# libxsmm/fpga_ai_nic

Hardware: AMD Instinct MI355X
Metric: MLP training samples/sec (1024-4096-4096-1024, BFP all-reduce + fused SGD) (higher is better)
Workload: dtype bf16; 1 GPU; model=mlp-1024-4096-4096-1024, global_batch=8192, parallelism=dp1, mb_per_gpu=8192, compress=bfp, rounding=rne, algo=mesh, rings=1, transport=none, engine=native, schedule=fixed, gemm_inflight=persistent, hip_graph=False, fused_sgd=True, fused_update_in_gemm=True, epilogue_stream=inline

## Files before the change

### csrc/bindings_ops.cpp

```cpp
#include "bindings_common.h"
#include "bfp/bfp_format.h"
#include "comm/planner.h"
#include "gemm/gemm.h"
#include "gemm/gemm_chain.h"
#include "gemm/gemm_group.h"
#include "nn/nn.h"

namespace fan {

namespace {

int dcode(const at::Tensor& t) {
  if (t.scalar_type() == at::kFloat) return kF32;
  if (t.scalar_type() == at::kBFloat16) return kBF16;
  TORCH_CHECK(false, "expected float32 or bfloat16 tensor");
}

int64_t ld_of(const at::Tensor& t) {
  TORCH_CHECK(t.dim() == 2, "expected a 2-D tensor");
  TORCH_CHECK(t.stride(1) == 1, "expected unit stride in the last dim");
  return t.stride(0);
}

void gemm(const at::Tensor& A, bool a_t, const at::Tensor& B, bool b_t, at::Tensor& C, int64_t epilogue,
          const c10::optional<at::Tensor>& bias, const c10::optional<at::Tensor>& aux, bool accumulate,
          int64_t split_k, const c10::optional<at::Tensor>& workspace, int64_t tile_bm, int64_t tile_bn,
          const c10::optional<at::Tensor>& colsum, int64_t tile_waves, const c10::optional<at::Tensor>& wire,
          int64_t wire_shard, int64_t wire_own, int64_t wire_codec, int64_t wire_period, int64_t wire_off,
          const c10::optional<at::Tensor>& upd_master, const c10::optional<at::Tensor>& upd_lp,
          const c10::optional<at::Tensor>& upd_mom, double upd_lr, double upd_grad_scale, double upd_weight_decay,
          double upd_momentum, bool upd_nesterov, bool defer_colsum, bool defer_reduce) {
  TORCH_CHECK(A.is_cuda() && B.is_cuda() && C.is_cuda(), "gemm operands must be GPU tensors");
  TORCH_CHECK(A.scalar_type() == B.scalar_type(), "A and B dtype mismatch");
  GemmArgs g{};
  g.A = A.data_ptr();
  g.B = B.data_ptr();
  g.C = C.data_ptr();
  g.lda = ld_of(A);
  g.ldb = ld_of(B);
  g.ldc = ld_of(C);
  g.M = (int)(a_t ? A.size(1) : A.size(0));
  g.K = (int)(a_t ? A.size(0) : A.size(1));
  g.N = (int)(b_t ? B.size(0) : B.size(1));
  const int64_t kb = b_t ? B.size(1) : B.size(0);
  TORCH_CHECK(kb == g.K, "gemm: inner dimensions differ (", g.K, " vs ", kb, ")");
  TORCH_CHECK(C.size(0) == g.M && C.size(1) == g.N, "gemm: bad C shape");
  g.a_kcontig = !a_t;
  g.b_kcontig = b_t;
  g.epilogue = (int)epilogue;
  g.c_bf16 = C.scalar_type() == at::kBFloat16;
  g.accumulate = accumulate;
  g.split_k = (int)std::max<int64_t>(0, split_k);
  g.tile_bm = (int)tile_bm;
  g.tile_bn = (int)tile_bn;
  g.tile_waves = (int)tile_waves;
  g.defer_reduce = defer_reduce;
  TORCH_CHECK(!defer_reduce || (epilogue == kEpiBias && C.scalar_type() == at::kFloat && !colsum && !accumulate),
              "defer_reduce: the f32 bias epilogue only (the softmax folds the slabs)");
  if (colsum) {
    TORCH_CHECK(colsum->is_cuda() && colsum->is_contiguous() && colsum->scalar_type() == at::kFloat &&
                    colsum->numel() >= g.N,
                "colsum must be a contiguous f32 GPU tensor of >= N elements");
    g.colsum = colsum->data_ptr<float>();
  }
  if (bias) {
    TORCH_CHECK(bias->is_contiguous() && bias->numel() >= g.N, "bad bias");
    g.bias = bias->data_ptr();
  }
  if (aux) {
    TORCH_CHECK(aux->scalar_type() == C.scalar_type(), "aux dtype must match C");
    g.aux = aux->data_ptr();
    g.ldaux = ld_of(*aux);
  }
  if (workspace) g.workspace = workspace->data_ptr();
  if (epilogue == kEpiWire) {
    TORCH_CHECK(wire && wire->is_cuda() && wire->is_contiguous() && wire->scalar_type() == at::kByte,
                "wire epilogue needs a contiguous uint8 GPU wire buffer");
    TORCH_CHECK(wire_shard > 0 && wire_shard % 256 == 0, "wire_shard must be a positive multiple of 256");
    TORCH_CHECK(wire_off >= 0 && wire_off % 16 == 0, "wire_off must be a non-negative multiple of 16");
    const int64_t last = wire_off + (g.colsum ? (int64_t)g.M * g.ldc + g.N - 1 : (int64_t)(g.M - 1) * g.ldc + g.N - 1);
    const int64_t need = (last / wire_shard + 1) * (int64_t)wire_shard_bytes((int)wire_codec, (size_t)wire_shard);
    TORCH_CHECK(wire->numel() >= need, "wire buffer too small: ", wire->numel(), " < ", need);
    g.wire = wire->data_ptr<uint8_t>();
    g.wire_shard = wire_shard;
    g.wire_own = (int)wire_own;
    g.wire_period = (int)wire_period;
    g.wire_codec = (int)wire_codec;
    g.wire_off = wire_off;
    if (upd_master) {
      auto plane = [&](const at::Tensor& t, at::ScalarType st, const char* what) {
        TORCH_CHECK(t.is_cuda() && t.is_contiguous() && t.scalar_type() == st && t.numel() > last &&
                        t.data_ptr() != nullptr && (reinterpret_cast<uintptr_t>(t.data_ptr()) & 15) == 0,
                    "fused update: ", what, " must be a contiguous, 16-B aligned GPU plane covering the bucket");
      };
      TORCH_CHECK(wire_own == -1, "fused update: no owner shard (single-rank engine)");
      TORCH_CHECK(wire_codec == kBfpRne, "fused update: rne codec only");
      plane(*upd_master, at::kFloat, "master");
      g.upd_master = upd_master->data_ptr<float>();
      if (upd_lp) {
        plane(*upd_lp, at::kBFloat16, "lp");
        g.upd_lp = reinterpret_cast<bf16_t*>(upd_lp->data_ptr());
      }
      if (upd_mom) {
        plane(*upd_mom, at::kFloat, "mom");
        g.upd_mom = upd_mom->data_ptr<float>();
      }
      g.upd = SgdParams{(float)upd_lr, (float)upd_grad_scale, (float)upd_weight_decay, (float)upd_momentum,
                        upd_nesterov ? 1 : 0};
      g.defer_colsum = defer_colsum && g.colsum != nullptr;
    }
  }
  if (A.scalar_type() == at::kBFloat16) {
    TORCH_CHECK(bias ? bias->scalar_type() == at::kBFloat16 : true, "bias must be bf16");
    const GemmPlan p = gemm_bf16_plan(g.M, g.N, g.K, g.split_k, g.tile_bm, g.tile_bn, g.tile_waves);
    const int64_t need = (p.split_k > 1 ? (int64_t)p.split_k * g.M * g.N : 0) +
                         (g.colsum && p.bm > 0 ? (int64_t)p.split_k * ((g.M + p.bm - 1) / p.bm) * g.N : 0);
    if (need > 0 || p.split_k > 1) {
      TORCH_CHECK(workspace && workspace->scalar_type() == at::kFloat && workspace->is_contiguous() &&
                      workspace->numel() >= need,
                  "gemm: split-K ", p.split_k, (g.colsum ? " with colsum" : ""), " needs an f32 workspace of ", need,
                  " elements");
    }
    TORCH_CHECK(gemm_bf16_supported(g), "gemm_bf16: unsupported shape M=", g.M, " N=", g.N, " K=", g.K,
                " split_k=", g.split_k);
    launch_gemm_bf16(g, fan_stream());
  } else {
    TORCH_CHECK(A.scalar_type() == at::kFloat, "gemm: A must be bf16 or f32");
    const int sk = gemm_f32_split(g.M, g.N, g.K, g.split_k);
    if (sk > 1) {
      const int64_t need = (int64_t)sk * g.M * g.N;
      TORCH_CHECK(workspace && workspace->scalar_type() == at::kFloat && workspace->is_contiguous() &&
                      workspace->numel() >= need,
                  "gemm_f32: split-K ", sk, " needs an f32 workspace of ", need, " elements");
    }
    TORCH_CHECK(gemm_f32_supported(g), "gemm_f32: unsupported shape M=", g.M, " N=", g.N, " K=", g.K);
    launch_gemm_f32(g, fan_stream());
  }
}

void gemm_wgrad_group(const std::vector<at::Tensor>& Xs, const std::vector<at::Tensor>& dYs,
                      const std::vector<at::Tensor>& Cs, const std::vector<at::Tensor>& colsums,
                      const std::vector<int64_t>& offs, at::Tensor& workspace, const c10::optional<at::Tensor>& wire,
                      int64_t wire_shard, int64_t wire_own, int64_t wire_codec, int64_t wire_period) {
  const size_t n = Xs.size();
  TORCH_CHECK(n >= 1 && n <= (size_t)kGroupMax && dYs.size() == n && Cs.size() == n && colsums.size() == n &&
                  (offs.empty() || offs.size() == n),
              "gemm_wgrad_group: 1..", kGroupMax, " problems, one X, dY, C, colsum (and wire offset) each");
  TORCH_CHECK(workspace.is_cuda() && workspace.scalar_type() == at::kFloat && workspace.is_contiguous(),
              "gemm_wgrad_group: f32 GPU workspace");
  std::vector<GemmArgs> g(n);
  int64_t ws_off = 0;
  for (size_t i = 0; i < n; ++i) {
    const at::Tensor &X = Xs[i], &dY = dYs[i], &C = Cs[i], &cs = colsums[i];
    TORCH_CHECK(X.is_cuda() && dY.is_cuda() && C.is_cuda() && cs.is_cuda(), "gemm_wgrad_group: GPU tensors");
    TORCH_CHECK(X.scalar_type() == at::kBFloat16 && dY.scalar_type() == at::kBFloat16 &&
                    C.scalar_type() == at::kFloat && cs.scalar_type() == at::kFloat && cs.is_contiguous(),
                "gemm_wgrad_group: bf16 X / dY, f32 C / colsum");
    TORCH_CHECK(X.dim() == 2 && dY.dim() == 2 && X.size(0) == dY.size(0) && C.dim() == 2 && C.size(0) == X.size(1) &&
                    C.size(1) == dY.size(1) && cs.numel() >= dY.size(1),
                "gemm_wgrad_group: shapes (X [K][M], dY [K][N], C [M][N], colsum [N])");
    GemmArgs& a = g[i];
    a.A = X.data_ptr(); a.lda = ld_of(X);
    a.B = dY.data_ptr(); a.ldb = ld_of(dY);
    a.C = C.data_ptr(); a.ldc = ld_of(C);
    a.M = (int)X.size(1); a.N = (int)dY.size(1); a.K = (int)X.size(0);
    a.a_kcontig = false; a.b_kcontig = false; a.c_bf16 = false;
    a.colsum = cs.data_ptr<float>();
    a.epilogue = wire ? kEpiWire : kEpiNone;
    a.workspace = workspace.data_ptr<float>() + ws_off;
    ws_off += (gemm_wgrad_group_ws(a) + 3) / 4 * 4;
    if (wire) {
      TORCH_CHECK(wire->is_cuda() && wire->is_contiguous() && wire->scalar_type() == at::kByte,
                  "wire epilogue needs a contiguous uint8 GPU wire buffer");
      TORCH_CHECK(wire_shard > 0 && wire_shard % 256 == 0, "wire_shard must be a positive multiple of 256");
      const int64_t off = offs.empty() ? 0 : offs[i];
      TORCH_CHECK(off >= 0 && off % 16 == 0, "wire offsets must be non-negative multiples of 16");
      const int64_t last = off + (int64_t)a.M * a.ldc + a.N - 1;
      const int64_t need = (last / wire_shard + 1) * (int64_t)wire_shard_bytes((int)wire_codec, (size_t)wire_shard);
      TORCH_CHECK(wire->numel() >= need, "wire buffer too small: ", wire->numel(), " < ", need);
      a.wire = wire->data_ptr<uint8_t>();
      a.wire_shard = wire_shard;
      a.wire_own = (int)wire_own;
      a.wire_period = (int)wire_period;
      a.wire_codec = (int)wire_codec;
      a.wire_off = off;
    }
  }
  TORCH_CHECK(workspace.numel() >= ws_off, "gemm_wgrad_group: workspace of ", ws_off, " floats needed");
  TORCH_CHECK(gemm_wgrad_group_supported(g.data(), (int)n),
              "gemm_wgrad_group: unsupported (M % 256, N % 128, K % 64, aligned operands, at most ", 64 * kNumCU,
              " workgroups)");
  launch_gemm_wgrad_group(g.data(), (int)n, fan_stream());
}

bool gemm_chain(int64_t kind, const at::Tensor& A0, const std::vector<at::Tensor>& Bs, const std::vector<at::Tensor>& Cs,
                const std::vector<c10::optional<at::Tensor>>& biases,
                const std::vector<c10::optional<at::Tensor>>& auxes, const std::vector<int64_t>& epis,
                at::Tensor& counters, bool dry_run) {
  const int n = (int)Bs.size();
  TORCH_CHECK(n >= 1 && (int)Cs.size() == n && (int)biases.size() == n && (int)auxes.size() == n &&
                  (int)epis.size() == n,
              "gemm_chain: one B, C, bias, aux and epilogue entry per stage");
  if (n > gemm_chain_max_stages()) return false;
  std::vector<GemmArgs> g(n);
  for (int i = 0; i < n; ++i) {
    const at::Tensor& A = i == 0 ? A0 : Cs[i - 1];
    const at::Tensor& B = Bs[i];
    const at::Tensor& C = Cs[i];
    for (const at::Tensor* t : {&A, &B, &C})
      if (!t->is_cuda() || t->dim() != 2 || t->stride(1) != 1) return false;
    if (A.scalar_type() != at::kBFloat16 || B.scalar_type() != at::kBFloat16) return false;
    GemmArgs& a = g[i];
    a.A = A.data_ptr();
    a.B = B.data_ptr();
    a.C = C.data_ptr();
    a.lda = A.stride(0);
    a.ldb = B.stride(0);
    a.ldc = C.stride(0);
    a.M = (int)A.size(0);
    a.K = (int)A.size(1);
    a.N = (int)(kind == kChainBwdData ? B.size(0) : B.size(1));
    if ((kind == kChainBwdData ? B.size(1) : B.size(0)) != a.K || C.size(0) != a.M || C.size(1) != a.N) return false;
    a.a_kcontig = true;
    a.b_kcontig = kind == kChainBwdData;
    a.c_bf16 = C.scalar_type() == at::kBFloat16;
    if (!a.c_bf16 && C.scalar_type() != at::kFloat) return false;
    a.split_k = 1;
    if (kind == kChainFwd) {
      if (!biases[i] || biases[i]->scalar_type() != at::kBFloat16 || biases[i]->numel() < a.N) return false;
      a.bias = biases[i]->data_ptr();
      a.epilogue = (int)epis[i];
    } else {
      if (!auxes[i] || auxes[i]->scalar_type() != at::kBFloat16 || auxes[i]->dim() != 2 ||
          auxes[i]->stride(1) != 1 || auxes[i]->size(0) != a.M || auxes[i]->size(1) != a.N)
        return false;
      a.aux = auxes[i]->data_ptr();
      a.ldaux = auxes[i]->stride(0);
      a.epilogue = (int)epis[i];
    }
  }
  if (!gemm_chain_supported(g.data(), n, (int)kind)) return false;
  TORCH_CHECK(counters.is_cuda() && counters.scalar_type() == at::kInt && counters.is_contiguous() &&
                  counters.numel() >= gemm_chain_counter_words(n, g[0].M),
              "gemm_chain: counters must be a contiguous int32 GPU tensor of gemm_chain_words(n, M) elements");
  if (dry_run) return true;
  launch_gemm_chain(g.data(), n, (int)kind, reinterpret_cast<unsigned*>(counters.data_ptr()), fan_stream());
  return true;
}

int64_t gemm_wgrad_group_ws_floats(const std::vector<std::pair<int64_t, int64_t>>& mn) {
  int64_t w = 0;
  for (const auto& p : mn) w += ((p.first / 256) * p.second + 3) / 4 * 4;
  return w;
}

pybind11::tuple gemm_plan(int64_t M, int64_t N, int64_t K, int64_t split_k, int64_t tile_bm, int64_t tile_bn,
                          int64_t tile_waves) {
  GemmPlan p = gemm_bf16_plan((int)M, (int)N, (int)K, (int)split_k, (int)tile_bm, (int)tile_bn, (int)tile_waves);
  return pybind11::make_tuple(p.bm, p.bn, p.split_k, p.waves);
}

bool gemm_supported(int64_t M, int64_t N, int64_t K, bool bf16, int64_t split_k) {
  GemmArgs g{};
  g.M = (int)M;
  g.N = (int)N;
  g.K = (int)K;
  g.lda = g.ldb = 64;
  g.ldc = N;
  g.split_k = (int)split_k;
  g.workspace = (void*)16;
  return bf16 ? gemm_bf16_supported(g) : gemm_f32_supported(g);
}

void softmax_xent(const at::Tensor& logits, const at::Tensor& labels, at::Tensor& dlogits, at::Tensor& loss_rows,
                  double grad_scale) {
  TORCH_CHECK(logits.is_cuda() && labels.is_cuda() && dlogits.is_cuda() && loss_rows.is_cuda(), "GPU tensors");
  TORCH_CHECK(labels.scalar_type() == at::kInt && labels.is_contiguous(), "labels must be int32");
  TORCH_CHECK(loss_rows.scalar_type() == at::kFloat, "loss_rows must be f32");
  const int M = (int)logits.size(0), Cc = (int)logits.size(1);
  TORCH_CHECK(dlogits.size(0) == M && dlogits.size(1) == Cc, "dlogits shape");
  launch_softmax_xent(dcode(logits), logits.data_ptr(), ld_of(logits), labels.data_ptr<int32_t>(), dcode(dlogits),
                      dlogits.data_ptr(), ld_of(dlogits), loss_rows.data_ptr<float>(), M, Cc, (float)grad_scale,
                      fan_stream());
}

void softmax_xent_slabs(const at::Tensor& ws, int64_t sk, const at::Tensor& bias, at::Tensor& logits,
                        const at::Tensor& labels, at::Tensor& dlogits, at::Tensor& loss_rows, double grad_scale) {
  TORCH_CHECK(ws.is_cuda() && bias.is_cuda() && logits.is_cuda() && labels.is_cuda() && dlogits.is_cuda() &&
                  loss_rows.is_cuda(), "GPU tensors");
  TORCH_CHECK(ws.scalar_type() == at::kFloat && ws.is_contiguous() && logits.scalar_type() == at::kFloat &&
                  bias.scalar_type() == at::kBFloat16 && bias.is_contiguous(), "f32 slabs / logits, bf16 bias");
  TORCH_CHECK(labels.scalar_type() == at::kInt && labels.is_contiguous() && loss_rows.scalar_type() == at::kFloat,
              "int32 labels, f32 loss rows");
  const int M = (int)logits.size(0), Cc = (int)logits.size(1);
  TORCH_CHECK(dlogits.size(0) == M && dlogits.size(1) == Cc && bias.numel() >= Cc, "shapes");
  TORCH_CHECK(sk >= 1 && ws.numel() >= sk * (int64_t)M * Cc, "workspace holds sk slabs of M x C");
  launch_softmax_xent_slabs(ws.data_ptr<float>(), (int)sk, reinterpret_cast<const bf16_t*>(bias.data_ptr()),
                            logits.data_ptr<float>(), ld_of(logits), labels.data_ptr<int32_t>(), dcode(dlogits),
                            dlogits.data_ptr(), ld_of(dlogits), loss_rows.data_ptr<float>(), M, Cc,
                            (float)grad_scale, fan_stream());
}

void col_sum(const at::Tensor& x, at::Tensor& out, double scale, bool accumulate, at::Tensor& workspace) {
  TORCH_CHECK(x.is_cuda() && out.is_cuda() && workspace.is_cuda(), "GPU tensors");
  const int M = (int)x.size(0), N = (int)x.size(1);
  TORCH_CHECK(out.numel() >= N && out.is_contiguous(), "out too small");
  TORCH_CHECK(workspace.scalar_type() == at::kFloat && (size_t)workspace.numel() >= col_sum_workspace_floats(M, N),
              "workspace too small");
  launch_col_sum(dcode(x), x.data_ptr(), ld_of(x), M, N, dcode(out), out.data_ptr(), (float)scale, accumulate,
                 workspace.data_ptr<float>(), fan_stream());
}

}

void register_gemm(pybind11::module_& m) {
  m.def("gemm", &gemm, "MFMA GEMM with fused epilogue", pybind11::arg("A"), pybind11::arg("a_t"), pybind11::arg("B"),
        pybind11::arg("b_t"), pybind11::arg("C"), pybind11::arg("epilogue") = 0, pybind11::arg("bias") = pybind11::none(),
        pybind11::arg("aux") = pybind11::none(), pybind11::arg("accumulate") = false, pybind11::arg("split_k") = 1,
        pybind11::arg("workspace") = pybind11::none(), pybind11::arg("tile_bm") = 0, pybind11::arg("tile_bn") = 0,
        pybind11::arg("colsum") = pybind11::none(), pybind11::arg("tile_waves") = 0,
        pybind11::arg("wire") = pybind11::none(), pybind11::arg("wire_shard") = 0, pybind11::arg("wire_own") = -1,
        pybind11::arg("wire_codec") = 1, pybind11::arg("wire_period") = 0, pybind11::arg("wire_off") = 0,
        pybind11::arg("upd_master") = pybind11::none(), pybind11::arg("upd_lp") = pybind11::none(),
        pybind11::arg("upd_mom") = pybind11::none(), pybind11::arg("upd_lr") = 0.0,
        pybind11::arg("upd_grad_scale") = 1.0, pybind11::arg("upd_weight_decay") = 0.0,
        pybind11::arg("upd_momentum") = 0.0, pybind11::arg("upd_nesterov") = false,
        pybind11::arg("defer_colsum") = false, pybind11::arg("defer_reduce") = false);
  m.def("gemm_supported", &gemm_supported);
  m.def("gemm_flush_colsum", []() { return gemm_flush_colsum(fan_stream()); },
        "launch the bias-gradient reduces queued on the current stream by defer_colsum GEMMs; returns how many");
  m.def("gemm_pending_colsum", []() { return gemm_pending_colsum(fan_stream()); },
        "bias-gradient reduces queued on the current stream");
  m.def("gemm_wgrad_group", &gemm_wgrad_group,
        "up to 8 bwd-weight GEMMs (+ fused bias gradients, f32 or BFP wire epilogue) in one dispatch",
        pybind11::arg("Xs"), pybind11::arg("dYs"), pybind11::arg("Cs"), pybind11::arg("colsums"),
        pybind11::arg("offs"), pybind11::arg("workspace"), pybind11::arg("wire") = pybind11::none(),
        pybind11::arg("wire_shard") = 0, pybind11::arg("wire_own") = -1, pybind11::arg("wire_codec") = 1,
        pybind11::arg("wire_period") = 0);
  m.def("gemm_wgrad_group_ws", &gemm_wgrad_group_ws_floats, "f32 workspace elements for a group of (M, N) problems");
  m.def("gemm_chain", &gemm_chain, "the GEMMs of one MLP pass as one persistent launch (row-panel hand-offs)",
        pybind11::arg("kind"), pybind11::arg("A0"), pybind11::arg("Bs"), pybind11::arg("Cs"), pybind11::arg("biases"),
        pybind11::arg("auxes"), pybind11::arg("epis"), pybind11::arg("counters"), pybind11::arg("dry_run") = false);
  m.def("gemm_chain_words", &gemm_chain_counter_words, "int32 words of a layer-chain counter block",
        pybind11::arg("n"), pybind11::arg("M"));
  m.def("gemm_set_prio", [](int on) { gemm_prio_flag().store(on); },
        "4-wave pipelined GEMM waves at s_setprio 2 (another stream's kernels issue in their stalls)");
  m.def("gemm_prio", []() { return gemm_prio_flag().load(); });
  m.def("gemm_set_ovl", [](int on) { gemm_ovl_flag().store(on); },
        "256x256 bf16 plans on the persistent loop with overlapped tile transitions (pl4_run OVL)");
  m.def("gemm_ovl", []() { return gemm_ovl_flag().load(); });
  m.def("gemm_set_reduce4", [](int on) { gemm_reduce4_flag().store(on); },
        "split-K wire / fused-update reduce: 4 values per lane (1) or one 16-value group per lane (0)");
  m.def("gemm_reduce4", []() { return gemm_reduce4_flag().load(); });
  m.def("gemm_f32_split", &gemm_f32_split, "f32 GEMM split-K factor (split_k <= 0: automatic)", pybind11::arg("M"),
        pybind11::arg("N"), pybind11::arg("K"), pybind11::arg("split_k") = 0);
  m.def("gemm_set_main_loop", [](int mode) { gemm_main_loop_flag().store(mode); },
        "256x256 GEMM tiles: 0 one-role, 2 pipelined (4 or 8 waves by layout / K), 3 pipelined 4-wave, "
        "5 pipelined 8-wave");
  m.def("gemm_main_loop", []() { return gemm_main_loop_flag().load(); });
  m.def("gemm_set_persist", [](int cap) { gemm_persist_flag().store(cap); },
        "grid cap of the persistent 4-wave GEMM kernel (<= 0: one workgroup per tile)");
  m.def("gemm_persist", []() { return gemm_persist_flag().load(); });
  m.def("gemm_set_stamp_buffer", [](const c10::optional<at::Tensor>& t) {
          gemm_set_stamp_buffer(t ? t->data_ptr() : nullptr);
        },
        "diagnostic builds only: int64 GPU buffer [8 wg][8 waves][64 K-tiles][5] for the GEMM loop's s_memtime stamps");
  m.def("gemm_plan", &gemm_plan, "bf16 GEMM tile/split-K plan (bm, bn, split_k, waves); bm == 0: unsupported",
        pybind11::arg("M"), pybind11::arg("N"), pybind11::arg("K"), pybind11::arg("split_k") = 0,
        pybind11::arg("tile_bm") = 0, pybind11::arg("tile_bn") = 0, pybind11::arg("tile_waves") = 0);
  m.attr("EPI_NONE") = (int)kEpiNone;
  m.attr("EPI_BIAS") = (int)kEpiBias;
  m.attr("EPI_BIAS_RELU") = (int)kEpiBiasRelu;
  m.attr("EPI_RELU_MASK") = (int)kEpiReluMask;
  m.attr("EPI_WIRE") = (int)kEpiWire;
}

void register_nn(pybind11::module_& m) {
  m.def("softmax_xent", &softmax_xent, "fused softmax + cross-entropy fwd/bwd");
  m.def("softmax_xent_slabs", &softmax_xent_slabs,
        "softmax + cross-entropy over the classifier GEMM's unreduced split-K slabs (+ bias; logits written)");
  m.def("col_sum", &col_sum, "bias-gradient column sum");
  m.def("col_sum_workspace_floats", [](int64_t M, int64_t N) { return (int64_t)col_sum_workspace_floats((int)M, (int)N); });
}

void register_planner(pybind11::module_& m) {
  m.def("ring_geometry", [](int64_t n, int world, int64_t max_slice) {
    auto g = ring_geometry(n, world, max_slice);
    return pybind11::make_tuple(g.n, g.slice_elems, g.blocks, g.n_pad);
  });
  m.def("ring_plan", [](int world, int position, int64_t blocks) {
    auto rounds = ring_plan(world, position, blocks);
    std::vector<std::vector<int32_t>> out;
    out.reserve(rounds.size());
    for (auto& r : rounds) out.push_back({r.send_slice, r.send_src, r.recv_slice, r.recv_full, r.owned});
    return out;
  });
  m.def(
      "ring_orders",
      [](int world, int max_rings, c10::optional<std::vector<std::vector<int>>> links) {
        if (!links) return ring_orders(world, max_rings);
        std::vector<char> l((size_t)world * world, 0);
        TORCH_CHECK((int)links->size() == world, "links: world rows expected");
        for (int a = 0; a < world; ++a) {
          TORCH_CHECK((int)(*links)[a].size() == world, "links: world columns expected");
          for (int b = 0; b < world; ++b) l[(size_t)a * world + b] = (*links)[a][b] != 0;
        }
        return ring_orders(world, max_rings, &l);
      },
      pybind11::arg("world"), pybind11::arg("max_rings"), pybind11::arg("links") = pybind11::none(),
      "arc-disjoint directed Hamiltonian rings over the (optional) link matrix links[a][b]: a can send to b");
}

}
```

### csrc/gemm/gemm.h

```cpp
#pragma once
#include <atomic>

#include "bfp/bfp_format.h"
#include "common/hip_common.h"

namespace fan {

enum GemmEpilogue : int {
  kEpiNone = 0,
  kEpiBias = 1,
  kEpiBiasRelu = 2,
  kEpiReluMask = 3,
  kEpiWire = 4,
  kEpiWireUpd = 5,
};
constexpr bool is_wire_epi(int e) { return e == kEpiWire || e == kEpiWireUpd; }

constexpr int kWireOwnAll = -2;

struct GemmArgs {
  const void* A;
  const void* B;
  void* C;
  const void* bias;
  const void* aux;
  int64_t lda, ldb, ldc, ldaux;
  int M, N, K;
  bool a_kcontig, b_kcontig;
  int epilogue;
  bool c_bf16;
  bool accumulate;
  int split_k;
  void* workspace;
  int tile_bm = 0;
  int tile_bn = 0;
  int tile_waves = 0;
  float* colsum = nullptr;
  uint8_t* wire = nullptr;
  int64_t wire_shard = 0;
  int wire_own = -1;
  int wire_period = 0;
  int wire_codec = 1;
  int64_t wire_off = 0;
  float* upd_master = nullptr;
  bf16_t* upd_lp = nullptr;
  float* upd_mom = nullptr;
  SgdParams upd{};
  bool defer_colsum = false;
  bool defer_reduce = false;
};

struct GemmPlan {
  int bm, bn, split_k, waves;
};

GemmPlan gemm_bf16_plan(int M, int N, int K, int split_k, int tile_bm = 0, int tile_bn = 0, int tile_waves = 0);

bool gemm_bf16_supported(const GemmArgs& a);
void launch_gemm_bf16(const GemmArgs& a, hipStream_t stream);
int gemm_flush_colsum(hipStream_t stream);
int gemm_pending_colsum(hipStream_t stream);

std::atomic<int>& gemm_main_loop_flag();
std::atomic<int>& gemm_persist_flag();
std::atomic<int>& gemm_prio_flag();
std::atomic<int>& gemm_ovl_flag();
std::atomic<int>& gemm_reduce4_flag();
void gemm_set_stamp_buffer(void* p);
void* gemm_stamp_buffer();

int gemm_f32_split(int M, int N, int K, int split_k);
bool gemm_f32_supported(const GemmArgs& a);
void launch_gemm_f32(const GemmArgs& a, hipStream_t stream);

}
```

### csrc/gemm/gemm_bf16_kernel.h

```cpp
#pragma once
#include <cstdlib>
#include <type_traits>
#include <utility>

#include "bfp/bfp_format.h"
#include "gemm/gemm.h"
#include "gemm/glds.h"

namespace fan {
namespace gemm_detail {

typedef short s16x8 __attribute__((ext_vector_type(8)));
typedef short s16x4 __attribute__((ext_vector_type(4)));
typedef __bf16 bf16x8 __attribute__((ext_vector_type(8)));
typedef float f32x4 __attribute__((ext_vector_type(4)));
typedef __attribute__((address_space(3))) void lds_void_t;
typedef __attribute__((address_space(3))) s16x4 lds_s16x4_t;

constexpr int BK = 64;
constexpr int kDefaultWaves = 8;

#ifdef FAN_GEMM_STAMPS
constexpr int kStampWG = 8, kStampKT = 64, kStampPts = 5;
#define FAN_STAMP(pt)                                                                                        \
  if (wo.stamps && blockIdx.x < kStampWG && kt < kStampKT && lane == 0)                                       \
  wo.stamps[(((size_t)blockIdx.x * 8 + wave) * kStampKT + kt) * kStampPts + (pt)] = __builtin_amdgcn_s_memtime()
#else
#define FAN_STAMP(pt)
#endif

__device__ __forceinline__ int mn_swz(int k) { return (k & 3) | (((k >> 3) & 1) << 2); }

static __device__ __attribute__((aligned(256))) uint4 g_gemm_zero16[16];

__host__ __device__ constexpr int cdiv_i(int a, int b) { return (a + b - 1) / b; }

template <int OUTER, int NT>
struct OpTile {
  static constexpr int BYTES = OUTER * BK * 2;
  static constexpr int IB = NT * 16;
  static constexpr int GLDS = BYTES / IB;
  static constexpr int PER_HALF = (64 * 256) / IB;
};

template <bool KCONTIG, int OUTER, int NT, bool EDGE = false>
__device__ __forceinline__ void stage_one(const bf16_t* __restrict__ g, int64_t ld, int o0, int k0, char* lds,
                                          int wave, int lane, int i, int o_lim = 0, int k_lim = 0) {
  using T = OpTile<OUTER, NT>;
  const int t = wave * 64 + lane;
  const bf16_t* src;
  bool out = false;
  if (KCONTIG) {
    const int row = i * (T::IB / 128) + (t >> 3);
    const int c = (t & 7) ^ ((row >> 1) & 7);
    src = g + (int64_t)(o0 + row) * ld + k0 + c * 8;
    if (EDGE) out = o0 + row >= o_lim || k0 + c * 8 >= k_lim;
  } else {
    const int half = i / T::PER_HALF;
    const int krow = (i % T::PER_HALF) * (T::IB / 256) + (t >> 4);
    const int cs = t & 15;
    const int blk = (cs >> 1) ^ mn_swz(krow);
    const int col = o0 + half * 128 + blk * 16 + (cs & 1) * 8;
    src = g + (int64_t)(k0 + krow) * ld + col;
    if (EDGE) out = k0 + krow >= k_lim || col >= o_lim;
  }
  if (EDGE && out) src = reinterpret_cast<const bf16_t*>(g_gemm_zero16);
  glds16((const void*)src, __builtin_amdgcn_readfirstlane(lds_addr_of(lds + i * T::IB + wave * 1024)));
}

template <bool KCONTIG, int OUTER, int NT, bool EDGE = false>
__device__ __forceinline__ void stage_tile(const bf16_t* __restrict__ g, int64_t ld, int o0, int k0, char* lds,
                                           int wave, int lane, int o_lim = 0, int k_lim = 0) {
#pragma unroll
  for (int i = 0; i < OpTile<OUTER, NT>::GLDS; ++i)
    stage_one<KCONTIG, OUTER, NT, EDGE>(g, ld, o0, k0, lds, wave, lane, i, o_lim, k_lim);
}

template <bool KCONTIG>
__device__ __forceinline__ s16x8 read_frag(const char* lds, int o, int ks, int lane) {
  if (KCONTIG) {
    const int row = o + (lane & 15);
    const int chunk = ks * 4 + (lane >> 4);
    return *reinterpret_cast<const s16x8*>(lds + row * 128 + ((chunk ^ ((row >> 1) & 7)) << 4));
  } else {
    const char* h = lds + (o >> 7) * (64 * 256);
    const int oo = o & 127;
    const int q = (lane & 15) >> 2, p = lane & 3;
    const int kb = ks * 32 + 8 * (lane >> 4) + q;
    const int blk = oo >> 4;
    const int off0 = kb * 256 + ((blk ^ mn_swz(kb)) << 5) + 8 * p;
    const int off1 = (kb + 4) * 256 + ((blk ^ mn_swz(kb + 4)) << 5) + 8 * p;
    s16x4 lo = __builtin_amdgcn_ds_read_tr16_b64_v4i16((lds_s16x4_t*)(h + off0));
    s16x4 hi = __builtin_amdgcn_ds_read_tr16_b64_v4i16((lds_s16x4_t*)(h + off1));
    s16x8 r;
    r[0] = lo[0]; r[1] = lo[1]; r[2] = lo[2]; r[3] = lo[3];
    r[4] = hi[0]; r[5] = hi[1]; r[6] = hi[2]; r[7] = hi[3];
    return r;
  }
}

__device__ __forceinline__ float frag_sum(const s16x8& f) {
  typedef __bf16 bf16x2 __attribute__((ext_vector_type(2)));
  typedef short s16x2 __attribute__((ext_vector_type(2)));
  const bf16x2 one = {(__bf16)1.0f, (__bf16)1.0f};
  float s = 0.f;
#pragma unroll
  for (int e = 0; e < 4; ++e) {
    const s16x2 p = {f[2 * e], f[2 * e + 1]};
    s = __builtin_amdgcn_fdot2_f32_bf16(__builtin_bit_cast(bf16x2, p), one, s, false);
  }
  return s;
}

__device__ __forceinline__ int xcd_remap(int bid, int nwg) {
  const int xcd = bid % kNumXCD;
  const int q = nwg / kNumXCD, r = nwg % kNumXCD;
  const int base = xcd < r ? xcd * (q + 1) : r * (q + 1) + (xcd - r) * q;
  return base + bid / kNumXCD;
}

template <typename TC>
struct Out;
template <>
struct Out<float> {
  __device__ static __forceinline__ void load4(const float* p, float v[4]) {
    const float4 x = *reinterpret_cast<const float4*>(p);
    v[0] = x.x; v[1] = x.y; v[2] = x.z; v[3] = x.w;
  }
  __device__ static __forceinline__ void store4(float* p, const float v[4]) {
    *reinterpret_cast<float4*>(p) = make_float4(v[0], v[1], v[2], v[3]);
  }
};
template <>
struct Out<bf16_t> {
  __device__ static __forceinline__ void load4(const bf16_t* p, float v[4]) {
    const uint2 u = *reinterpret_cast<const uint2*>(p);
    v[0] = __uint_as_float(u.x << 16); v[1] = __uint_as_float(u.x & 0xFFFF0000u);
    v[2] = __uint_as_float(u.y << 16); v[3] = __uint_as_float(u.y & 0xFFFF0000u);
  }
  __device__ static __forceinline__ void store4(bf16_t* p, const float v[4]) {
    *reinterpret_cast<uint2*>(p) = make_uint2(pack_bf16x2(v[0], v[1]), pack_bf16x2(v[2], v[3]));
  }
};

template <int EPI, typename TC, bool ACCUM>
__device__ __forceinline__ void epi4(float v[4], TC* __restrict__ C, int64_t ldc, const bf16_t* __restrict__ bias,
                                     const TC* __restrict__ aux, int64_t ldaux, int row, int col) {
  if (EPI == kEpiBias || EPI == kEpiBiasRelu) {
    const uint2 u = *reinterpret_cast<const uint2*>(bias + col);
    v[0] += __uint_as_float(u.x << 16); v[1] += __uint_as_float(u.x & 0xFFFF0000u);
    v[2] += __uint_as_float(u.y << 16); v[3] += __uint_as_float(u.y & 0xFFFF0000u);
  }
  if (EPI == kEpiBiasRelu) {
#pragma unroll
    for (int u = 0; u < 4; ++u) v[u] = fmaxf(v[u], 0.f);
  }
  if (EPI == kEpiReluMask) {
    float m[4];
    Out<TC>::load4(aux + (int64_t)row * ldaux + col, m);
#pragma unroll
    for (int u = 0; u < 4; ++u) v[u] = m[u] > 0.f ? v[u] : 0.f;
  }
  TC* p = C + (int64_t)row * ldc + col;
  if (ACCUM) {
    float o[4];
    Out<TC>::load4(p, o);
#pragma unroll
    for (int u = 0; u < 4; ++u) v[u] += o[u];
  }
  Out<TC>::store4(p, v);
}

typedef uint32_t u32x4_t __attribute__((ext_vector_type(4)));
__device__ __forceinline__ void store_wt16(void* p, const uint4& o) {
  const u32x4_t v = {o.x, o.y, o.z, o.w};
  asm volatile("global_store_dwordx4 %0, %1, off sc1\n\ts_nop 1" ::"v"(p), "v"(v) : "memory");
}

template <int EPI, bool ACCUM, bool WT = false>
__device__ __forceinline__ void epi8_bf16(float v[8], bf16_t* __restrict__ C, int64_t ldc,
                                          const bf16_t* __restrict__ bias, const uint4* mask, int row, int col) {
  auto lo = [](uint32_t u) { return __uint_as_float(u << 16); };
  auto hi = [](uint32_t u) { return __uint_as_float(u & 0xFFFF0000u); };
  if (EPI == kEpiBias || EPI == kEpiBiasRelu) {
    const uint4 u = *reinterpret_cast<const uint4*>(bias + col);
    v[0] += lo(u.x); v[1] += hi(u.x); v[2] += lo(u.y); v[3] += hi(u.y);
    v[4] += lo(u.z); v[5] += hi(u.z); v[6] += lo(u.w); v[7] += hi(u.w);
  }
  if (EPI == kEpiBiasRelu) {
#pragma unroll
    for (int u = 0; u < 8; ++u) v[u] = fmaxf(v[u], 0.f);
  }
  if (EPI == kEpiReluMask) {
    const uint4 m = *mask;
    const float mv[8] = {lo(m.x), hi(m.x), lo(m.y), hi(m.y), lo(m.z), hi(m.z), lo(m.w), hi(m.w)};
#pragma unroll
    for (int u = 0; u < 8; ++u) v[u] = mv[u] > 0.f ? v[u] : 0.f;
  }
  bf16_t* p = C + (int64_t)row * ldc + col;
  if (ACCUM) {
    const uint4 o = *reinterpret_cast<const uint4*>(p);
    v[0] += lo(o.x); v[1] += hi(o.x); v[2] += lo(o.y); v[3] += hi(o.y);
    v[4] += lo(o.z); v[5] += hi(o.z); v[6] += lo(o.w); v[7] += hi(o.w);
  }
  const uint4 o = make_uint4(pack_bf16x2(v[0], v[1]), pack_bf16x2(v[2], v[3]), pack_bf16x2(v[4], v[5]),
                             pack_bf16x2(v[6], v[7]));
  if constexpr (WT) store_wt16(p, o);
  else *reinterpret_cast<uint4*>(p) = o;
}

struct WireOut {
  uint8_t* p;
  int64_t shard;
  int own;
  int period;
  int codec;
  float inv_shard;
  int bias_off;
  float* um;
  bf16_t* ulp;
  float* umom;
  SgdParams up;
#ifdef FAN_GEMM_STAMPS
  unsigned long long* stamps;
#endif
  uint32_t off;
  int prio;
};

__device__ __forceinline__ int wire_shard_of(uint32_t f, const WireOut& wo) {
  int sh = (int)((float)f * wo.inv_shard);
  const uint32_t sz = (uint32_t)wo.shard;
  if ((uint32_t)sh * sz > f) --sh;
  else if ((uint32_t)(sh + 1) * sz <= f) ++sh;
  return sh;
}

__device__ __forceinline__ uint8_t* wire_shard_base(int sh, const WireOut& wo) {
  return wo.p + (int64_t)sh * (wo.shard + wo.shard / 16);
}

__device__ __forceinline__ int32_t wire_encode(float x, uint32_t E, int codec) {
  return codec == kBfpTrunc ? bfp_encode_trunc(__float_as_uint(x), E) : bfp_encode_rne(x, E);
}

__device__ __forceinline__ float wire_roundtrip_rne(float x, uint32_t E) {
  return bfp_decode_rne(bfp_encode_rne(x, E), E);
}

__device__ __forceinline__ float sgd_apply(float g, float& w, float& m, bool has_mom, const SgdParams& p) {
  float gj = g * p.grad_scale;
  if (p.weight_decay != 0.0f) gj = fmaf(p.weight_decay, w, gj);
  if (has_mom) {
    m = fmaf(p.momentum, m, gj);
    gj = p.nesterov ? fmaf(p.momentum, m, gj) : m;
  }
  w = fmaf(-p.lr, gj, w);
  return w;
}

template <bool PRE = false>
__device__ __forceinline__ void local_update16(const float v[16], uint32_t E, uint32_t f, const WireOut& wo,
                                               float (&w)[16]) {
  float m[16];
  if constexpr (!PRE) {
#pragma unroll
    for (int u = 0; u < 16; u += 4) {
      const float4 a = *reinterpret_cast<const float4*>(wo.um + f + u);
      w[u] = a.x; w[u + 1] = a.y; w[u + 2] = a.z; w[u + 3] = a.w;
    }
  }
  const bool hm = wo.umom != nullptr;
  if (hm) {
#pragma unroll
    for (int u = 0; u < 16; u += 4) {
      const float4 a = *reinterpret_cast<const float4*>(wo.umom + f + u);
      m[u] = a.x; m[u + 1] = a.y; m[u + 2] = a.z; m[u + 3] = a.w;
    }
  }
#pragma unroll
  for (int u = 0; u < 16; ++u) sgd_apply(wire_roundtrip_rne(v[u], E), w[u], m[u], hm, wo.up);
#pragma unroll
  for (int u = 0; u < 16; u += 4) {
    *reinterpret_cast<float4*>(wo.um + f + u) = make_float4(w[u], w[u + 1], w[u + 2], w[u + 3]);
    if (hm) *reinterpret_cast<float4*>(wo.umom + f + u) = make_float4(m[u], m[u + 1], m[u + 2], m[u + 3]);
  }
  if (wo.ulp) {
    uint4* d = reinterpret_cast<uint4*>(wo.ulp + f);
    d[0] = make_uint4(pack_bf16x2(w[0], w[1]), pack_bf16x2(w[2], w[3]), pack_bf16x2(w[4], w[5]),
                      pack_bf16x2(w[6], w[7]));
    d[1] = make_uint4(pack_bf16x2(w[8], w[9]), pack_bf16x2(w[10], w[11]), pack_bf16x2(w[12], w[13]),
                      pack_bf16x2(w[14], w[15]));
  }
}

template <bool UPD = false, bool PRE = false>
__device__ __forceinline__ int wire_store16(const float v[16], uint32_t f, const WireOut& wo, float (&wm)[16]) {
  uint32_t mx = 0;
#pragma unroll
  for (int u = 0; u < 16; ++u) mx = max(mx, __float_as_uint(v[u]) & 0x7FFFFFFFu);
  const uint32_t E = mx >> 23;
  if constexpr (UPD) {
    local_update16<PRE>(v, E, f, wo, wm);
    return -1;
  }
  const int sh = wire_shard_of(f, wo);
  const uint32_t pos = f - (uint32_t)sh * (uint32_t)wo.shard;
  uint32_t w[4] = {0u, 0u, 0u, 0u};
#pragma unroll
  for (int u = 0; u < 16; ++u) w[u >> 2] |= ((uint32_t)wire_encode(v[u], E, wo.codec) & 0xFFu) << (8 * (u & 3));
  uint8_t* base = wire_shard_base(sh, wo);
  *reinterpret_cast<uint4*>(base + pos) = make_uint4(w[0], w[1], w[2], w[3]);
  base[wo.shard + pos / 16] = (uint8_t)E;
  return sh;
}

template <bool UPD = false>
__device__ __forceinline__ int wire_store16(const float v[16], uint32_t f, const WireOut& wo) {
  float wm[16];
  return wire_store16<UPD, false>(v, f, wo, wm);
}

template <bool UPD = false, bool PRE = false>
__device__ __forceinline__ void wire_epi16(const float v[16], float* __restrict__ C, int64_t ldc, const WireOut& wo,
                                           int row, int col, float (&w)[16]) {
  const uint32_t loc = (uint32_t)row * (uint32_t)ldc + (uint32_t)col;
  const int sh = wire_store16<UPD, PRE>(v, wo.off + loc, wo, w);
  if (sh >= 0 && (wo.own == kWireOwnAll || (wo.period > 0 ? sh % wo.period : sh) == wo.own)) {
#pragma unroll
    for (int u = 0; u < 16; u += 4)
      *reinterpret_cast<float4*>(C + loc + u) = make_float4(v[u], v[u + 1], v[u + 2], v[u + 3]);
  }
}

template <bool UPD = false>
__device__ __forceinline__ void wire_epi16(const float v[16], float* __restrict__ C, int64_t ldc, const WireOut& wo,
                                           int row, int col) {
  float w[16];
  wire_epi16<UPD, false>(v, C, ldc, wo, row, col, w);
}

template <int NJ, int WTN, int EPI, bool SPLIT>
__device__ __forceinline__ void colsum_finish(float (&cs)[NJ], int lane, int col0, float* __restrict__ out,
                                              const WireOut& wo, int N) {
#pragma unroll
  for (int j = 0; j < NJ; ++j) {
    float v = cs[j];
    v += __shfl_xor(v, 16);
    v += __shfl_xor(v, 32);
    const int col = col0 + j * 16 + (lane & 15);
    if (lane < 16 && col < N) out[col] = v;
    if constexpr (is_wire_epi(EPI) && !SPLIT) {
      if (wo.bias_off > 0 && col0 + j * 16 < N) {
        uint32_t mx = __float_as_uint(v) & 0x7FFFFFFFu;
#pragma unroll
        for (int o = 1; o < 16; o <<= 1) mx = max(mx, (uint32_t)__shfl_xor((int)mx, o));
        const uint32_t E = mx >> 23;
        const uint32_t f = (uint32_t)wo.bias_off + (uint32_t)col;
        if constexpr (EPI == kEpiWireUpd) {
          if (lane < 16) {
            float w = wo.um[f], m = wo.umom ? wo.umom[f] : 0.f;
            sgd_apply(wire_roundtrip_rne(v, E), w, m, wo.umom != nullptr, wo.up);
            wo.um[f] = w;
            if (wo.umom) wo.umom[f] = m;
            if (wo.ulp) wo.ulp[f] = f32_to_bf16(w);
          }
          continue;
        }
        const int sh = wire_shard_of(f, wo);
        const uint32_t pos = f - (uint32_t)sh * (uint32_t)wo.shard;
        uint8_t* base = wire_shard_base(sh, wo);
        if (lane < 16) base[pos] = (uint8_t)(wire_encode(v, E, wo.codec) & 0xFF);
        if (lane == 0) base[wo.shard + pos / 16] = (uint8_t)E;
      }
    }
  }
}

template <int MI, int NJ, int WTN, int EPI, typename TC, bool ACCUM, bool SPLIT, int SW = WTN, bool WT = false>
__device__ __forceinline__ void store_tile(const f32x4 (&acc)[MI][NJ], char* smem, int wave, int lane, int row0,
                                           int col0, TC* __restrict__ C, int64_t ldc, const bf16_t* __restrict__ bias,
                                           const TC* __restrict__ aux, int64_t ldaux, int M, int N, int ksplit,
                                           float* __restrict__ ws, const WireOut& wo, bool mn_edge = false) {
  static_assert(SW == WTN || (SW == 64 && WTN % 64 == 0 && sizeof(TC) == 2 && !SPLIT && !is_wire_epi(EPI)),
                "64-column staging: bf16 8-column path only");
  static_assert(!WT || (sizeof(TC) == 2 && !SPLIT && !is_wire_epi(EPI)), "write-through stores: the bf16 8-column path");
  constexpr int EW = SW + 4;
  float* stg = reinterpret_cast<float*>(smem) + wave * (16 * EW);
  const int col_l = lane & 15, row_l = (lane >> 4) * 4;
  constexpr int C4 = WTN / 4;
  constexpr int RPI = 64 / C4;
  if constexpr (sizeof(TC) == 2 && !SPLIT && !is_wire_epi(EPI)) {
    {
      constexpr int C8 = SW / 8;
      constexpr int RP8 = 64 / C8;
      constexpr int NP8 = 16 / RP8;
      constexpr int HV = WTN / SW;
      static_assert(WTN % 8 == 0 && RP8 <= 16 && 16 % RP8 == 0, "8-column chunks of whole 16-row blocks");
      constexpr bool kPf8 = EPI == kEpiReluMask;
      constexpr int kPfd = 2;
      uint4 aq8[kPf8 ? MI : 1][kPf8 ? HV * NP8 : 1];
      auto aux_load8 = [&](int i) __attribute__((always_inline)) {
#pragma unroll
        for (int hv = 0; hv < HV; ++hv)
#pragma unroll
          for (int pass = 0; pass < NP8; ++pass) {
            const int row = row0 + i * 16 + pass * RP8 + lane / C8;
            const int col = col0 + hv * SW + (lane % C8) * 8;
            if (!mn_edge || (row < M && col < N))
              aq8[i][hv * NP8 + pass] = *reinterpret_cast<const uint4*>(aux + (int64_t)row * ldaux + col);
          }
      };
      if constexpr (kPf8) {
#pragma unroll
        for (int i = 0; i < kPfd && i < MI; ++i) aux_load8(i);
      }
#pragma unroll
      for (int i = 0; i < MI; ++i) {
        if constexpr (kPf8) {
          if (i + kPfd < MI) aux_load8(i + kPfd);
        }
#pragma unroll
        for (int hv = 0; hv < HV; ++hv) {
#pragma unroll
        for (int j = 0; j < SW / 16; ++j)
#pragma unroll
          for (int r = 0; r < 4; ++r) stg[(row_l + r) * EW + j * 16 + col_l] = acc[i][hv * (SW / 16) + j][r];
        __builtin_amdgcn_s_waitcnt(0xC07F);
#pragma unroll
        for (int pass = 0; pass < NP8; ++pass) {
          const int rr = pass * RP8 + lane / C8;
          const int cc = (lane % C8) * 8;
          const float4 q0 = *reinterpret_cast<const float4*>(stg + rr * EW + cc);
          const float4 q1 = *reinterpret_cast<const float4*>(stg + rr * EW + cc + 4);
          float v[8] = {q0.x, q0.y, q0.z, q0.w, q1.x, q1.y, q1.z, q1.w};
          const int row = row0 + i * 16 + rr;
          const int col = col0 + hv * SW + cc;
          if (mn_edge && (row >= M || col >= N)) continue;
          const uint4* mk = nullptr;
          if constexpr (kPf8) mk = &aq8[i][hv * NP8 + pass];
          epi8_bf16<EPI, ACCUM, WT>(v, reinterpret_cast<bf16_t*>(C), ldc, bias, mk, row, col);
        }
        __builtin_amdgcn_s_waitcnt(0xC07F);
        }
      }
      return;
    }
  }
  constexpr bool kPfAux = EPI == kEpiReluMask && !SPLIT && sizeof(TC) == 2;
  constexpr int kPf = 2;
  constexpr int NP = 16 / RPI;
  using AuxV = typename std::conditional<sizeof(TC) == 2, uint2, uint4>::type;
  AuxV aq[kPfAux ? MI : 1][kPfAux ? NP : 1];
  auto aux_load = [&](int i) __attribute__((always_inline)) {
#pragma unroll
    for (int pass = 0; pass < NP; ++pass) {
      const int row = row0 + i * 16 + pass * RPI + lane / C4;
      const int col = col0 + (lane % C4) * 4;
      if (!mn_edge || (row < M && col < N))
        aq[i][pass] = *reinterpret_cast<const AuxV*>(aux + (int64_t)row * ldaux + col);
    }
  };
  if constexpr (kPfAux) {
#pragma unroll
    for (int i = 0; i < kPf && i < MI; ++i) aux_load(i);
  }
  constexpr bool kPfUpd = EPI == kEpiWireUpd && !SPLIT;
  constexpr int UG16 = WTN / 16, URPG = 64 / UG16, UPASS = URPG >= 16 ? 1 : 16 / URPG;
#ifndef FAN_GEMM_UPD_PF
#define FAN_GEMM_UPD_PF 2
#endif
  constexpr int kUpf = FAN_GEMM_UPD_PF, US = kPfUpd ? kUpf + 1 : 1;
  float um_pf[US][kPfUpd ? UPASS : 1][16];
  auto upd_load = [&](int i, int slot) __attribute__((always_inline)) {
    if constexpr (kPfUpd) {
#pragma unroll
      for (int pass = 0; pass < UPASS; ++pass) {
        const int rr = pass * URPG + lane / UG16;
        const int row = row0 + i * 16 + rr, col = col0 + (lane % UG16) * 16;
        if ((URPG <= 16 || rr < 16) && (!mn_edge || (row < M && col < N))) {
          const float* q = wo.um + wo.off + (uint32_t)row * (uint32_t)ldc + (uint32_t)col;
#pragma unroll
          for (int u = 0; u < 16; u += 4) {
            const float4 a = *reinterpret_cast<const float4*>(q + u);
            um_pf[slot][pass][u] = a.x; um_pf[slot][pass][u + 1] = a.y;
            um_pf[slot][pass][u + 2] = a.z; um_pf[slot][pass][u + 3] = a.w;
          }
        }
      }
    }
  };
  if constexpr (kPfUpd) {
#pragma unroll
    for (int d = 0; d < kUpf && d < MI; ++d) upd_load(d, d % US);
  }
#pragma unroll
  for (int i = 0; i < MI; ++i) {
    if constexpr (kPfAux) {
      if (i + kPf < MI) aux_load(i + kPf);
    }
    if constexpr (kPfUpd) {
      if (i + kUpf < MI) upd_load(i + kUpf, (i + kUpf) % US);
    }
#pragma unroll
    for (int j = 0; j < NJ; ++j)
#pragma unroll
      for (int r = 0; r < 4; ++r) stg[(row_l + r) * EW + j * 16 + col_l] = acc[i][j][r];
    __builtin_amdgcn_s_waitcnt(0xC07F);
    if constexpr (is_wire_epi(EPI) && !SPLIT) {
      constexpr int G16 = WTN / 16;
      constexpr int RPG = 64 / G16;
      constexpr int PASSES = RPG >= 16 ? 1 : 16 / RPG;
#pragma unroll
      for (int pass = 0; pass < PASSES; ++pass) {
        const int rr = pass * RPG + lane / G16;
        if (RPG <= 16 || rr < 16) {
          const int cc = (lane % G16) * 16;
          float v[16];
#pragma unroll
          for (int u = 0; u < 16; u += 4) {
            const float4 q = *reinterpret_cast<const float4*>(stg + rr * EW + cc + u);
            v[u] = q.x; v[u + 1] = q.y; v[u + 2] = q.z; v[u + 3] = q.w;
          }
          if (!mn_edge || (row0 + i * 16 + rr < M && col0 + cc < N))
            wire_epi16<EPI == kEpiWireUpd, kPfUpd>(v, reinterpret_cast<float*>(C), ldc, wo, row0 + i * 16 + rr,
                                                   col0 + cc, um_pf[kPfUpd ? i % US : 0][kPfUpd ? pass : 0]);
        }
      }
      __builtin_amdgcn_s_waitcnt(0xC07F);
      continue;
    }
#pragma unroll
    for (int pass = 0; pass < 16 / RPI; ++pass) {
      const int rr = pass * RPI + lane / C4;
      const int cc = (lane % C4) * 4;
      const float4 q = *reinterpret_cast<const float4*>(stg + rr * EW + cc);
      float v[4] = {q.x, q.y, q.z, q.w};
      const int row = row0 + i * 16 + rr;
      const int col = col0 + cc;
      if (mn_edge && (row >= M || col >= N)) continue;
      if (SPLIT) {
        float* slab = ws + (int64_t)ksplit * M * N;
        *reinterpret_cast<float4*>(slab + (int64_t)row * N + col) = q;
      } else if constexpr (kPfAux) {
        float m[4];
        if constexpr (sizeof(TC) == 2) {
          const uint2 u = aq[i][pass];
          m[0] = __uint_as_float(u.x << 16); m[1] = __uint_as_float(u.x & 0xFFFF0000u);
          m[2] = __uint_as_float(u.y << 16); m[3] = __uint_as_float(u.y & 0xFFFF0000u);
        } else {
          const uint4 u = aq[i][pass];
          m[0] = __uint_as_float(u.x); m[1] = __uint_as_float(u.y);
          m[2] = __uint_as_float(u.z); m[3] = __uint_as_float(u.w);
        }
#pragma unroll
        for (int u = 0; u < 4; ++u) v[u] = m[u] > 0.f ? v[u] : 0.f;
        epi4<kEpiNone, TC, ACCUM>(v, C, ldc, bias, aux, ldaux, row, col);
      } else {
        epi4<EPI, TC, ACCUM>(v, C, ldc, bias, aux, ldaux, row, col);
      }
    }
    __builtin_amdgcn_s_waitcnt(0xC07F);
  }
}

template <int BM, int BN, int WM, int WN, bool AK, bool BKC, int EPI, typename TC, bool ACCUM, bool SPLIT,
          bool DMA1 = false, bool RAGGED = false>
__global__ void __launch_bounds__(WM * WN * 64, WM * WN / 4)
    gemm_bf16_kernel(const bf16_t* __restrict__ A, int64_t lda, const bf16_t* __restrict__ B, int64_t ldb,
                     TC* __restrict__ C, int64_t ldc, const bf16_t* __restrict__ bias, const TC* __restrict__ aux,
                     int64_t ldaux, int M, int N, int K, int split_k, float* __restrict__ ws,
                     float* __restrict__ colsum, WireOut wo) {
  constexpr int NT = WM * WN * 64;
  constexpr int A_BYTES = OpTile<BM, NT>::BYTES, B_BYTES = OpTile<BN, NT>::BYTES;
  constexpr int STAGE = A_BYTES + B_BYTES;
  constexpr int S = (3 * STAGE <= 160 * 1024) ? 3 : 2;
  constexpr int G = OpTile<BM, NT>::GLDS + OpTile<BN, NT>::GLDS;
  constexpr int WTM = BM / WM, WTN = BN / WN;
  constexpr int MI = WTM / 16, NJ = WTN / 16;
  static_assert(WM * WN == 8 || WM * WN == 4, "4 or 8 waves");
  extern __shared__ __attribute__((aligned(16))) char smem[];

  const int tiles_n = cdiv_i(N, BN);
  const int tiles_m = cdiv_i(M, BM);
  const int tiles = tiles_m * tiles_n;
  const int nwg = tiles * split_k;
  const int wg = xcd_remap(blockIdx.x, nwg);
  const int tile = wg % tiles;
  const int ksplit = wg / tiles;
  const int GM = tiles_m >= 4 ? 4 : tiles_m;
  const int grp = tile / (GM * tiles_n);
  const int gm = (tiles_m - grp * GM) < GM ? (tiles_m - grp * GM) : GM;
  const int in_grp = tile % (GM * tiles_n);
  const int m0 = (grp * GM + in_grp % gm) * BM;
  const int n0 = (in_grp / gm) * BN;
  const int nkt = cdiv_i(K, BK);
  const int kt_per = cdiv_i(nkt, split_k);
  const int kt0 = ksplit * kt_per;
  const int nk = max(0, min(nkt, kt0 + kt_per) - kt0);
  const int kbeg = kt0 * BK;
  const bool mn_edge = RAGGED && (m0 + BM > M || n0 + BN > N);
  const bool edge = RAGGED && (mn_edge || (kt0 + nk) * BK > K);

  const int lane = threadIdx.x & 63;
  const int wave = __builtin_amdgcn_readfirstlane(threadIdx.x >> 6);
  const int wm = wave / WN, wn = wave % WN;
  const bool do_colsum = !BKC && colsum != nullptr && m0 == 0 && wm == 0;
  float cs[NJ];
#pragma unroll
  for (int j = 0; j < NJ; ++j) cs[j] = 0.f;

  f32x4 acc[MI][NJ];
#pragma unroll
  for (int i = 0; i < MI; ++i)
#pragma unroll
    for (int j = 0; j < NJ; ++j) acc[i][j] = f32x4{0.f, 0.f, 0.f, 0.f};

  auto issue_stage = [&](int kt_stage, int buf) {
    char* st = smem + buf * STAGE;
    if (edge) {
      stage_tile<AK, BM, NT, true>(A, lda, m0, kbeg + kt_stage * BK, st, wave, lane, M, K);
      stage_tile<BKC, BN, NT, true>(B, ldb, n0, kbeg + kt_stage * BK, st + A_BYTES, wave, lane, N, K);
    } else {
      stage_tile<AK, BM, NT>(A, lda, m0, kbeg + kt_stage * BK, st, wave, lane);
      stage_tile<BKC, BN, NT>(B, ldb, n0, kbeg + kt_stage * BK, st + A_BYTES, wave, lane);
    }
  };

  constexpr int REG_BUDGET = NT == 256 ? 480 : 232;
  constexpr int ACC_R = MI * NJ * 4, FRAG_R = (MI + NJ) * 4;
  constexpr bool DBL = ACC_R + 2 * FRAG_R <= REG_BUDGET;
#pragma unroll
  for (int s = 0; s < S - 1; ++s) {
    if (s < nk) issue_stage(s, s);
  }

  for (int kt = 0; kt < nk; ++kt) {
    FAN_STAMP(0);
    if (S == 3 && kt + 1 < nk) {
      asm volatile("s_waitcnt vmcnt(%0)" ::"n"(G) : "memory");
    } else {
      asm volatile("s_waitcnt vmcnt(0)" ::: "memory");
    }
    FAN_STAMP(1);
    __builtin_amdgcn_s_barrier();
    FAN_STAMP(2);
    const bool pf = kt + S - 1 < nk;
    char* pst = smem + ((kt + S - 1) % S) * STAGE;
    const int pk = kbeg + (kt + S - 1) * BK;
    if constexpr (DMA1 && S == 2 && NT == 512) {
      if (pf && wave < 4) {
        if (edge) {
          stage_tile<AK, BM, 256, true>(A, lda, m0, pk, pst, wave, lane, M, K);
          stage_tile<BKC, BN, 256, true>(B, ldb, n0, pk, pst + A_BYTES, wave, lane, N, K);
        } else {
          stage_tile<AK, BM, 256>(A, lda, m0, pk, pst, wave, lane);
          stage_tile<BKC, BN, 256>(B, ldb, n0, pk, pst + A_BYTES, wave, lane);
        }
      }
    } else if (pf) {
      if (edge) {
        stage_tile<AK, BM, NT, true>(A, lda, m0, pk, pst, wave, lane, M, K);
        stage_tile<BKC, BN, NT, true>(B, ldb, n0, pk, pst + A_BYTES, wave, lane, N, K);
      } else {
        stage_tile<AK, BM, NT>(A, lda, m0, pk, pst, wave, lane);
        stage_tile<BKC, BN, NT>(B, ldb, n0, pk, pst + A_BYTES, wave, lane);
      }
    }
    FAN_STAMP(3);
    const char* sa = smem + (kt % S) * STAGE;
    const char* sb = sa + A_BYTES;
    if constexpr (DBL) {
      s16x8 af[2][MI], bfr[2][NJ];
#pragma unroll
      for (int ks = 0; ks < 2; ++ks) {
#pragma unroll
        for (int i = 0; i < MI; ++i) af[ks][i] = read_frag<AK>(sa, wm * WTM + i * 16, ks, lane);
#pragma unroll
        for (int j = 0; j < NJ; ++j) bfr[ks][j] = read_frag<BKC>(sb, wn * WTN + j * 16, ks, lane);
        if (do_colsum) {
#pragma unroll
          for (int j = 0; j < NJ; ++j) cs[j] += frag_sum(bfr[ks][j]);
        }
      }
      FAN_STAMP(4);
#pragma unroll
      for (int ks = 0; ks < 2; ++ks) {
        __builtin_amdgcn_s_setprio(1);
#pragma unroll
        for (int i = 0; i < MI; ++i)
#pragma unroll
          for (int j = 0; j < NJ; ++j)
            acc[i][j] = __builtin_amdgcn_mfma_f32_16x16x32_bf16(__builtin_bit_cast(bf16x8, af[ks][i]),
                                                                __builtin_bit_cast(bf16x8, bfr[ks][j]), acc[i][j],
                                                                0, 0, 0);
        __builtin_amdgcn_s_setprio(0);
      }
    } else {
#pragma unroll
      for (int ks = 0; ks < 2; ++ks) {
        s16x8 af[MI], bfr[NJ];
#pragma unroll
        for (int i = 0; i < MI; ++i) af[i] = read_frag<AK>(sa, wm * WTM + i * 16, ks, lane);
#pragma unroll
        for (int j = 0; j < NJ; ++j) bfr[j] = read_frag<BKC>(sb, wn * WTN + j * 16, ks, lane);
        if (do_colsum) {
#pragma unroll
          for (int j = 0; j < NJ; ++j) cs[j] += frag_sum(bfr[j]);
        }
        __builtin_amdgcn_s_setprio(1);
#pragma unroll
        for (int i = 0; i < MI; ++i)
#pragma unroll
          for (int j = 0; j < NJ; ++j)
            acc[i][j] = __builtin_amdgcn_mfma_f32_16x16x32_bf16(__builtin_bit_cast(bf16x8, af[i]),
                                                                __builtin_bit_cast(bf16x8, bfr[j]), acc[i][j], 0,
                                                                0, 0);
        __builtin_amdgcn_s_setprio(0);
      }
    }
  }

  if (do_colsum)
    colsum_finish<NJ, WTN, EPI, SPLIT>(cs, lane, n0 + wn * WTN, SPLIT ? ws + (int64_t)split_k * M * N + (int64_t)ksplit * N
                                                                      : colsum, wo, N);
  __syncthreads();
  store_tile<MI, NJ, WTN, EPI, TC, ACCUM, SPLIT>(acc, smem, wave, lane, m0 + wm * WTM, n0 + wn * WTN, C, ldc, bias,
                                                 aux, ldaux, M, N, ksplit, ws, wo, mn_edge);
}

__device__ __forceinline__ void glds16_s(const void* sbase, uint32_t voff, uint32_t lds_addr) {
  asm volatile("s_mov_b32 m0, %2\n\ts_nop 0\n\tglobal_load_lds_dwordx4 %0, %1" ::"v"(voff), "s"(sbase), "s"(lds_addr)
               : "memory");
}

template <uint32_t OFF, bool SC1 = false>
__device__ __forceinline__ void glds16_si(const void* sbase, uint32_t voff, uint32_t lds_base) {
  if constexpr (SC1)
    asm volatile("s_add_u32 m0, %2, %3\n\ts_nop 0\n\tglobal_load_lds_dwordx4 %0, %1 sc1" ::"v"(voff), "s"(sbase),
                 "s"(lds_base), "i"(OFF)
                 : "memory", "scc");
  else
    asm volatile("s_add_u32 m0, %2, %3\n\ts_nop 0\n\tglobal_load_lds_dwordx4 %0, %1" ::"v"(voff), "s"(sbase),
                 "s"(lds_base), "i"(OFF)
                 : "memory", "scc");
}

template <int VM, int LGKM>
__device__ __forceinline__ void waitcnt_known() {
  static_assert(VM >= 0 && VM <= 63 && LGKM >= 0 && LGKM <= 15, "s_waitcnt field ranges");
#ifdef FAN_GEMM_ASM_WAITS
  asm volatile("s_waitcnt vmcnt(%0) lgkmcnt(%1)" ::"n"(VM), "n"(LGKM) : "memory");
#else
  __builtin_amdgcn_s_waitcnt((VM & 15) | (7 << 4) | (LGKM << 8) | ((VM >> 4) << 14));
  asm volatile("" ::: "memory");
#endif
}

template <bool KCONTIG, int OUTER, int NT>
__device__ __forceinline__ uint32_t piece_off(int64_t ld, int o0, int wave, int lane, int i) {
  using T = OpTile<OUTER, NT>;
  const int t = wave * 64 + lane;
  if (KCONTIG) {
    const int row = i * (T::IB / 128) + (t >> 3);
    const int c = (t & 7) ^ ((row >> 1) & 7);
    return (uint32_t)(((int64_t)(o0 + row) * ld + c * 8) * 2);
  } else {
    const int half = i / T::PER_HALF;
    const int krow = (i % T::PER_HALF) * (T::IB / 256) + (t >> 4);
    const int cs = t & 15;
    const int blk = (cs >> 1) ^ mn_swz(krow);
    return (uint32_t)(((int64_t)krow * ld + o0 + half * 128 + blk * 16 + (cs & 1) * 8) * 2);
  }
}

template <bool AK, bool BKC, int EPI, typename TC, bool ACCUM, bool SPLIT, bool COLSUM = false>
__global__ void __launch_bounds__(512, 2)
    gemm_pl_kernel(const bf16_t* __restrict__ A, int64_t lda, const bf16_t* __restrict__ B, int64_t ldb,
                   TC* __restrict__ C, int64_t ldc, const bf16_t* __restrict__ bias, const TC* __restrict__ aux,
                   int64_t ldaux, int M, int N, int K, int split_k, float* __restrict__ ws,
                   float* __restrict__ colsum, WireOut wo) {
  constexpr int BM = 256, BN = 256, NT = 512;
  constexpr int A_BYTES = OpTile<BM, NT>::BYTES;
  constexpr int STAGE = A_BYTES + OpTile<BN, NT>::BYTES;
  constexpr int GA = OpTile<BM, NT>::GLDS, G = GA + OpTile<BN, NT>::GLDS;
  constexpr int WTM = 128, WTN = 64, MI = 8, NJ = 4;
  static_assert(G == 8, "8 glds pieces per wave and K-tile");
  extern __shared__ __attribute__((aligned(16))) char smem[];

  const int tiles_n = N / BN, tiles_m = M / BM, tiles = tiles_m * tiles_n;
  const int wg = xcd_remap(blockIdx.x, tiles * split_k);
  const int tile = wg % tiles, ksplit = wg / tiles;
  const int GM = tiles_m >= 4 ? 4 : tiles_m;
  const int grp = tile / (GM * tiles_n);
  const int gm = (tiles_m - grp * GM) < GM ? (tiles_m - grp * GM) : GM;
  const int in_grp = tile % (GM * tiles_n);
  const int m0 = (grp * GM + in_grp % gm) * BM;
  const int n0 = (in_grp / gm) * BN;
  const int k_per = K / split_k;
  const int kbeg = ksplit * k_per;
  const int nk = k_per / BK;

  const int lane = threadIdx.x & 63;
  const int wave = __builtin_amdgcn_readfirstlane(threadIdx.x >> 6);
  const int wm = wave / 4, wn = wave % 4;
  const int im = SPLIT ? 0 : m0 / BM;
  const int cs0 = SPLIT ? (m0 == 0 ? 0 : nk) : im * nk / tiles_m;
  const int cs1 = SPLIT ? nk : (im + 1) * nk / tiles_m;
  const bool do_colsum = COLSUM && wm == 0;
  float cs[NJ];
#pragma unroll
  for (int j = 0; j < NJ; ++j) cs[j] = 0.f;

  f32x4 acc[MI][NJ];
#pragma unroll
  for (int i = 0; i < MI; ++i)
#pragma unroll
    for (int j = 0; j < NJ; ++j) acc[i][j] = f32x4{0.f, 0.f, 0.f, 0.f};
  s16x8 fa[MI], fb[2][NJ];

  uint32_t off[G];
#pragma unroll
  for (int p = 0; p < GA; ++p) off[p] = piece_off<AK, BM, NT>(lda, m0, wave, lane, p);
#pragma unroll
  for (int p = GA; p < G; ++p) off[p] = piece_off<BKC, BN, NT>(ldb, n0, wave, lane, p - GA);
  const int64_t a_step = AK ? (int64_t)BK * 2 : (int64_t)BK * lda * 2;
  const int64_t b_step = BKC ? (int64_t)BK * 2 : (int64_t)BK * ldb * 2;
  const char* a_k0 = reinterpret_cast<const char*>(A) + (AK ? (int64_t)kbeg * 2 : (int64_t)kbeg * lda * 2);
  const char* b_k0 = reinterpret_cast<const char*>(B) + (BKC ? (int64_t)kbeg * 2 : (int64_t)kbeg * ldb * 2);
  const uint32_t lds0 = lds_addr_of(smem);

  auto piece = [&](int kt, int p) {
    const uint32_t st = lds0 + (kt & 1) * STAGE + wave * 1024;
    if (p < GA) glds16_s(a_k0 + kt * a_step, off[p], st + p * OpTile<BM, NT>::IB);
    else glds16_s(b_k0 + kt * b_step, off[p], st + A_BYTES + (p - GA) * OpTile<BN, NT>::IB);
  };
  auto read_a = [&](const char* st, int ks, int i) { fa[i] = read_frag<AK>(st, wm * WTM + i * 16, ks, lane); };
  auto read_b = [&](const char* st, int ks, int set, int j) {
    fb[set][j] = read_frag<BKC>(st + A_BYTES, wn * WTN + j * 16, ks, lane);
  };
  auto block = [&](auto cur_c, auto read_c, auto dma_c, const char* rd_st, int rd_ks, int dma_kt, bool csk) {
    constexpr int cur = decltype(cur_c)::value;
    constexpr bool READ = decltype(read_c)::value, DMA = decltype(dma_c)::value;
    if (COLSUM && csk) {
#pragma unroll
      for (int j = 0; j < NJ; ++j) cs[j] += frag_sum(fb[cur][j]);
    }
#pragma unroll
    for (int i = 0; i < MI; ++i) {
#pragma unroll
      for (int j = 0; j < NJ; ++j) {
        if (READ && i < 2 && (j & 1) == 0) read_b(rd_st, rd_ks, cur ^ 1, i * 2 + (j >> 1));
        if (DMA && j == 2) piece(dma_kt, i);
        acc[i][j] = __builtin_amdgcn_mfma_f32_16x16x32_bf16(__builtin_bit_cast(bf16x8, fa[i]),
                                                            __builtin_bit_cast(bf16x8, fb[cur][j]), acc[i][j], 0, 0, 0);
      }
      if (READ) read_a(rd_st, rd_ks, i);
    }
    if constexpr (READ) {
#pragma unroll
      for (int i = 0; i < MI; ++i) {
        if (i < 2) {
          __builtin_amdgcn_sched_group_barrier(0x100, 1, 0);
          __builtin_amdgcn_sched_group_barrier(0x008, 2, 0);
          __builtin_amdgcn_sched_group_barrier(0x100, 1, 0);
          __builtin_amdgcn_sched_group_barrier(0x008, 2, 0);
        } else {
          __builtin_amdgcn_sched_group_barrier(0x008, 4, 0);
        }
        __builtin_amdgcn_sched_group_barrier(0x100, 1, 0);
      }
    }
  };
  using I0 = std::integral_constant<int, 0>;
  using I1 = std::integral_constant<int, 1>;
  using T_ = std::true_type;
  using F_ = std::false_type;

#pragma unroll
  for (int p = 0; p < G; ++p) piece(0, p);
  if (nk > 1) {
#pragma unroll
    for (int p = 0; p < G; ++p) piece(1, p);
    asm volatile("s_waitcnt vmcnt(%0)" ::"n"(G) : "memory");
  } else {
    asm volatile("s_waitcnt vmcnt(0)" ::: "memory");
  }
  __builtin_amdgcn_s_barrier();
#pragma unroll
  for (int j = 0; j < NJ; ++j) read_b(smem, 0, 0, j);
#pragma unroll
  for (int i = 0; i < MI; ++i) read_a(smem, 0, i);

  auto ktile = [&](int kt, auto more_c, auto more2_c) {
    const char* st = smem + (kt & 1) * STAGE;
    const bool csk = do_colsum && kt >= cs0 && kt < cs1;
    FAN_STAMP(0);
    __builtin_amdgcn_s_setprio(1);
    block(I0{}, T_{}, F_{}, st, 1, 0, csk);
    __builtin_amdgcn_s_setprio(0);
    FAN_STAMP(1);
    asm volatile("s_waitcnt vmcnt(0) lgkmcnt(0)" ::: "memory");
    FAN_STAMP(2);
    __builtin_amdgcn_s_barrier();
    FAN_STAMP(3);
    __builtin_amdgcn_s_setprio(1);
    block(I1{}, more_c, more2_c, smem + ((kt + 1) & 1) * STAGE, 0, kt + 2, csk);
    __builtin_amdgcn_s_setprio(0);
    FAN_STAMP(4);
  };
  int kt = 0;
  for (; kt + 2 < nk; ++kt) ktile(kt, T_{}, T_{});
  if (kt + 1 < nk) ktile(kt++, T_{}, F_{});
  if (kt < nk) ktile(kt, F_{}, F_{});

  if (COLSUM && do_colsum && (!SPLIT || m0 == 0))
    colsum_finish<NJ, WTN, kEpiNone, true>(
        cs, lane, n0 + wn * WTN, ws + (SPLIT ? (int64_t)split_k * M * N + (int64_t)ksplit * N : (int64_t)im * N), wo,
        N);
  asm volatile("s_waitcnt vmcnt(0)" ::: "memory");
  __syncthreads();
  store_tile<MI, NJ, WTN, EPI, TC, ACCUM, SPLIT>(acc, smem, wave, lane, m0 + wm * WTM, n0 + wn * WTN, C, ldc, bias,
                                                 aux, ldaux, M, N, ksplit, ws, wo);
}


template <typename F, int... I>
__device__ __forceinline__ void static_for_impl(F&& f, std::integer_sequence<int, I...>) {
  (f(std::integral_constant<int, I>{}), ...);
}
template <int N, typename F>
__device__ __forceinline__ void static_for(F&& f) {
  static_for_impl(f, std::make_integer_sequence<int, N>{});
}

__device__ __forceinline__ void mfma_acc(f32x4& acc, const s16x8& a, const s16x8& b) {
#ifdef FAN_GEMM_NOMFMA
  asm volatile("" : "+a"(acc) : "v"(a), "v"(b));
#else
  asm volatile("v_mfma_f32_16x16x32_bf16 %0, %1, %2, %0" : "+a"(acc) : "v"(a), "v"(b));
#endif
}

constexpr int kChainMaxStages = 8;
constexpr int kChainLdsCtl = 2 * (256 + 256) * BK * 2 + 4 * 16 * (64 + 4) * 4;
constexpr int kChainLds = kChainLdsCtl + 64;
constexpr uint32_t kChainSpinLimit = 1u << 22;

struct ChainStageArgs {
  const bf16_t* A;
  const bf16_t* B;
  void* C;
  const bf16_t* bias;
  const void* aux;
  int64_t lda, ldb, ldc, ldaux;
  int M, N, K;
  int tn;
  int first;
  int dep;
  int signal;
  int cfg;
};

struct ChainArgs {
  ChainStageArgs st[kChainMaxStages];
  int nstages;
  int total;
  int ppg;
  int panels;
  unsigned* ctr;
  int prio;
  int flags;
};
constexpr int kChainNoAcquire = 1;
constexpr int kChainRowsFastest = 2;

__host__ __device__ constexpr int chain_ctr_words(int nstages, int panels) { return (10 + nstages * panels) * 16; }
__device__ __forceinline__ int chain_ready_word(const ChainArgs& ca, int s, int panel) {
  return (10 + s * ca.panels + panel) * 16;
}
__device__ __forceinline__ int chain_stage_of(const ChainArgs& ca, int t) {
  int s = 0;
  while (s + 1 < ca.nstages && t >= ca.st[s + 1].first) ++s;
  return s;
}

struct ChainState {
  int ticket;
  int ready;
  int pending;
};

struct ChainRun {
  unsigned* ctr;
  int group, ppg, wpg;
  int first, end, tn;
  int dep;
  int dep_word0;
  int sig_word0;
  int nx_end, nx_tn;
  int flags;
};
__device__ __forceinline__ void chain_rc(const ChainRun& cr, int tn, int k, int& r, int& c) {
  if (cr.flags & kChainRowsFastest) {
    r = k % cr.ppg;
    c = k / cr.ppg;
  } else {
    r = k / tn;
    c = k % tn;
  }
}

__device__ __forceinline__ void chain_add(unsigned* ctr, int word) {
  __hip_atomic_fetch_add(ctr + word, 1u, __ATOMIC_RELAXED, __HIP_MEMORY_SCOPE_AGENT);
}
__device__ __forceinline__ unsigned chain_poll(const unsigned* ctr, int word) {
  return __hip_atomic_load(ctr + word, __ATOMIC_RELAXED, __HIP_MEMORY_SCOPE_AGENT);
}
__device__ __forceinline__ void chain_acquire(int flags = 0) {
  if (!(flags & kChainNoAcquire)) asm volatile("buffer_inv sc1" ::: "memory");
}
__device__ __forceinline__ void chain_tile_rc(const ChainArgs& ca, int tn, int k, int& r, int& c) {
  if (ca.flags & kChainRowsFastest) {
    r = k % ca.ppg;
    c = k / ca.ppg;
  } else {
    r = k / tn;
    c = k % tn;
  }
}

__device__ __forceinline__ void chain_dep_of(const ChainArgs& ca, int t, int& word, unsigned& target) {
  word = -1;
  target = 0;
  if (t >= ca.total) return;
  const int s = chain_stage_of(ca, t);
  const ChainStageArgs& S = ca.st[s];
  if (S.dep <= 0) return;
  int r, c;
  chain_tile_rc(ca, S.tn, t - S.first, r, c);
  word = chain_ready_word(ca, s - 1, (int)(blockIdx.x & 7) * ca.ppg + r);
  target = (unsigned)S.dep;
}

template <bool AK, bool BKC, int EPI, typename TC, bool ACCUM, bool SPLIT, bool COLSUM = false, int BN_ = 256,
          int BM_ = 256, bool OVL = false, bool CHAIN = false, bool WT = false, bool ASC1 = false>
__device__ __forceinline__ void pl4_run(const bf16_t* __restrict__ A, int64_t lda, const bf16_t* __restrict__ B,
                                        int64_t ldb, TC* __restrict__ C, int64_t ldc, const bf16_t* __restrict__ bias,
                                        const TC* __restrict__ aux, int64_t ldaux, int M, int N, int K, int split_k,
                                        float* __restrict__ ws, float* __restrict__ colsum, const WireOut& wo, int v0,
                                        int vstep, ChainRun cr = ChainRun{}, ChainState* chs = nullptr) {
  constexpr int BM = BM_, BN = BN_, NT = 256;
  constexpr int A_BYTES = OpTile<BM, NT>::BYTES;
  constexpr int STAGE = A_BYTES + OpTile<BN, NT>::BYTES;
  constexpr int GA = OpTile<BM, NT>::GLDS, G = GA + OpTile<BN, NT>::GLDS;
  constexpr int WTM = BM / 2, WTN = BN / 2, MI = WTM / 16, NJ = WTN / 16;
  constexpr int Q = MI * NJ, R = MI + NJ;
#ifndef FAN_GEMM_RSP_Q4
#define FAN_GEMM_RSP_Q4 3
#endif
  constexpr int RSP = (Q * FAN_GEMM_RSP_Q4 / 4) / R, DSP = Q / G;
  static_assert(BN == 256 || BN == 128, "256x256 or 256x128 tiles");
  static_assert(BM == 256 || (BM == 224 && BN == 128 && AK && !COLSUM) || (BM == 128 && BN == 128),
                "256-row tiles; 224-row tiles (K-contiguous A, BN 128); 128x128 tiles");
  static_assert(OpTile<BM, NT>::BYTES % OpTile<BM, NT>::IB == 0, "whole glds pieces");
  constexpr int STAGES = BN == 128 ? 3 : 2;
  static_assert(RSP >= 1 && DSP >= 1 && G * DSP <= Q, "schedule");
  static_assert(!OVL || (BM == 256 && BN == 256 && !COLSUM && !SPLIT && !ACCUM && sizeof(TC) == 2 &&
                         !is_wire_epi(EPI)),
                "overlapped transitions: 256x256 bf16 tiles without split-K or bias gradient");
  constexpr int kSW = OVL ? 64 : WTN;
  constexpr int kS = MI * (WTN / kSW) * (16 / (64 / (kSW / 8)));
  constexpr int DSP2 = Q / (2 * G);
  static_assert(!OVL || (G + kS <= 63 && DSP2 >= 1), "vmcnt range / schedule");
  extern __shared__ __attribute__((aligned(16))) char smem[];

  const int tiles_n = N / BN, tiles_m = M / BM, tiles = tiles_m * tiles_n;
  const int lane = threadIdx.x & 63;
  const int wave = __builtin_amdgcn_readfirstlane(threadIdx.x >> 6);
  const int wm = wave / 2, wn = wave % 2;
  const uint32_t lds0 = lds_addr_of(smem);
  if (wo.prio > 0) __builtin_amdgcn_s_setprio(2);
  static_assert(!CHAIN || (!SPLIT && !COLSUM && !ACCUM && BM == 256), "layer chain: unsplit 256-row tiles");
  const int GM = tiles_m >= 4 ? 4 : tiles_m;
  auto tile_origin = [&](int v, int& m, int& n) __attribute__((always_inline)) {
    if constexpr (CHAIN) {
      int r, c;
      chain_rc(cr, cr.tn, v - cr.first, r, c);
      m = (cr.group * cr.ppg + r) * BM;
      n = c * BN;
    } else {
      const int t1 = xcd_remap(v, tiles * split_k) % tiles;
      const int g1 = t1 / (GM * tiles_n);
      const int gm1 = (tiles_m - g1 * GM) < GM ? (tiles_m - g1 * GM) : GM;
      const int i1 = t1 % (GM * tiles_n);
      m = (g1 * GM + i1 % gm1) * BM;
      n = (i1 / gm1) * BN;
    }
  };
  int ch_next = 0, ch_rdy = 0;
  bool ch_cont = false;
  auto tile_body = [&](int v, bool first, int vn) __attribute__((always_inline)) {
  const int ksplit = CHAIN ? 0 : xcd_remap(v, tiles * split_k) / tiles;
  int m0, n0;
  tile_origin(v, m0, n0);
  const int k_per = K / split_k;
  const int kbeg = ksplit * k_per;
  const int nk = k_per / BK;

  const int im = SPLIT ? 0 : m0 / BM;
  const int cs0 = SPLIT ? (m0 == 0 ? 0 : nk) : im * nk / tiles_m;
  const int cs1 = SPLIT ? nk : (im + 1) * nk / tiles_m;
  const bool do_colsum = COLSUM && wm == 0;
  float cs[NJ];
#pragma unroll
  for (int j = 0; j < NJ; ++j) cs[j] = 0.f;

  f32x4 acc[MI][NJ];
#pragma unroll
  for (int i = 0; i < MI; ++i)
#pragma unroll
    for (int j = 0; j < NJ; ++j) acc[i][j] = f32x4{0.f, 0.f, 0.f, 0.f};
  s16x8 fa[2][MI], fb[2][NJ];

  uint32_t off[G];
#pragma unroll
  for (int p = 0; p < GA; ++p) off[p] = piece_off<AK, BM, NT>(lda, m0, wave, lane, p);
#pragma unroll
  for (int p = GA; p < G; ++p) off[p] = piece_off<BKC, BN, NT>(ldb, n0, wave, lane, p - GA);
  const int64_t a_step = AK ? (int64_t)BK * 2 : (int64_t)BK * lda * 2;
  const int64_t b_step = BKC ? (int64_t)BK * 2 : (int64_t)BK * ldb * 2;
  const char* a_k0 = reinterpret_cast<const char*>(A) + (AK ? (int64_t)kbeg * 2 : (int64_t)kbeg * lda * 2);
  const char* b_k0 = reinterpret_cast<const char*>(B) + (BKC ? (int64_t)kbeg * 2 : (int64_t)kbeg * ldb * 2);

  auto piece = [&](int kt, auto pc) __attribute__((always_inline)) {
    constexpr int p = decltype(pc)::value;
    const uint32_t st = lds0 + (STAGES == 2 ? kt & 1 : kt % 3) * STAGE + wave * 1024;
    if constexpr (p < GA) glds16_si<p * OpTile<BM, NT>::IB, ASC1>(a_k0 + kt * a_step, off[p], st);
    else glds16_si<A_BYTES + (p - GA) * OpTile<BN, NT>::IB>(b_k0 + kt * b_step, off[p], st);
  };
  auto read_next = [&](const char* st, int ks, int set, int r) __attribute__((always_inline)) {
    if (r < MI) fa[set][r] = read_frag<AK>(st, wm * WTM + r * 16, ks, lane);
    else fb[set][r - MI] = read_frag<BKC>(st + A_BYTES, wn * WTN + (r - MI) * 16, ks, lane);
  };
  auto block = [&](auto cur_c, auto read_c, auto dma_c, const char* rd_st, int rd_ks, int dma_kt,
                   bool csk, auto next_c, bool next_on = false) __attribute__((always_inline)) {
    constexpr int cur = decltype(cur_c)::value;
    constexpr bool READ = decltype(read_c)::value, DMA = decltype(dma_c)::value, NEXT = decltype(next_c)::value;
    if (COLSUM && csk)
      static_for<NJ>([&](auto jc) __attribute__((always_inline)) { cs[jc.value] += frag_sum(fb[cur][jc.value]); });
    static_for<MI * NJ>([&](auto qc) __attribute__((always_inline)) {
      constexpr int q = decltype(qc)::value;
      if constexpr (READ && q % RSP == 0 && q / RSP < R) read_next(rd_st, rd_ks, cur ^ 1, q / RSP);
#ifndef FAN_GEMM_NODMA
      if constexpr (DMA && q % DSP == DSP / 2 && q / DSP < G) piece(dma_kt, std::integral_constant<int, q / DSP>{});
      if constexpr (NEXT && q % DSP2 == 0 && q / DSP2 < 2 * G) {
        if (next_on) piece(q / DSP2 / G, std::integral_constant<int, q / DSP2 % G>{});
      }
#endif
      mfma_acc(acc[q / NJ][q % NJ], fa[cur][q / NJ], fb[cur][q % NJ]);
    });
  };
  using I0 = std::integral_constant<int, 0>;
  using I1 = std::integral_constant<int, 1>;
  using T_ = std::true_type;
  using F_ = std::false_type;

  if (!OVL || first) static_for<G>([&](auto pc) __attribute__((always_inline)) { piece(0, pc); });
  if (nk > 1) {
    if (!OVL || first) {
      static_for<G>([&](auto pc) __attribute__((always_inline)) { piece(1, pc); });
      asm volatile("s_waitcnt vmcnt(%0)" ::"n"(G) : "memory");
    } else {
      asm volatile("s_waitcnt vmcnt(%0)" ::"n"(G + kS) : "memory");
    }
  } else {
    asm volatile("s_waitcnt vmcnt(0)" ::: "memory");
  }
  __builtin_amdgcn_s_barrier();
#pragma unroll
  for (int r = 0; r < R; ++r) read_next(smem, 0, 0, r);

  unsigned ch_poll = 0;
  int* const ch_ctl = reinterpret_cast<int*>(smem + kChainLdsCtl);
  auto chain_hook = [&](int kt) __attribute__((always_inline)) {
    if constexpr (CHAIN) {
      if (kt == 1) {
        if (wave == 0 && lane == 0) {
          if (chs->pending >= 0) chain_add(cr.ctr, chs->pending);
          ch_ctl[0] = cr.wpg + (int)__hip_atomic_fetch_add(cr.ctr + cr.group * 16, 1u, __ATOMIC_RELAXED,
                                                            __HIP_MEMORY_SCOPE_AGENT);
        }
        chs->pending = -1;
      } else if (kt == nk - 3) {
        if (wave == 0 && lane == 0) {
          const int t = ch_ctl[0];
          int r, c, word = -1, tgt = 0;
          if (t < cr.end) {
            if (cr.dep > 0) {
              chain_rc(cr, cr.tn, t - cr.first, r, c);
              word = cr.dep_word0 + r * 16;
              tgt = cr.dep;
            }
          } else if (t < cr.nx_end && cr.sig_word0 >= 0) {
            chain_rc(cr, cr.nx_tn, t - cr.end, r, c);
            word = cr.sig_word0 + r * 16;
            tgt = cr.tn;
          } else {
            word = -2;
          }
          ch_ctl[2] = word;
          ch_ctl[3] = tgt;
          if (word >= 0) ch_poll = chain_poll(cr.ctr, word);
        }
      } else if (kt == nk - 2) {
        if (wave == 0 && lane == 0) {
          const int word = ch_ctl[2];
          ch_ctl[1] = word == -1 || (word >= 0 && ch_poll >= (unsigned)ch_ctl[3]);
        }
      }
    }
  };
  auto chain_decide = [&]() __attribute__((always_inline)) {
    if constexpr (CHAIN) {
      ch_next = __builtin_amdgcn_readfirstlane(ch_ctl[0]);
      ch_rdy = __builtin_amdgcn_readfirstlane(ch_ctl[1]);
      ch_cont = OVL && ch_rdy && ch_next < cr.end;
      if (ch_cont && cr.dep > 0) chain_acquire(cr.flags);
    }
  };
  auto ktile = [&](int kt, auto more_c, auto more2_c) __attribute__((always_inline)) {
    const char* st = smem + (STAGES == 2 ? kt & 1 : kt % 3) * STAGE;
    const bool csk = do_colsum && kt >= cs0 && kt < cs1;
    FAN_STAMP(0);
    if constexpr (STAGES == 2) {
      constexpr bool kLast = OVL && !decltype(more_c)::value && !decltype(more2_c)::value;
      auto next_offsets = [&](int vnn) __attribute__((always_inline)) {
        int m1, n1;
        tile_origin(vnn, m1, n1);
#pragma unroll
        for (int p = 0; p < GA; ++p) off[p] = piece_off<AK, BM, NT>(lda, m1, wave, lane, p);
#pragma unroll
        for (int p = GA; p < G; ++p) off[p] = piece_off<BKC, BN, NT>(ldb, n1, wave, lane, p - GA);
      };
      if constexpr (kLast && !CHAIN) {
        if (vn >= 0) next_offsets(vn);
      }
      block(I0{}, T_{}, F_{}, st, 1, 0, csk, F_{});
      FAN_STAMP(1);
      if (OVL && kt == 0 && !first) waitcnt_known<kS, 0>();
      else waitcnt_known<0, 0>();
      FAN_STAMP(2);
      __builtin_amdgcn_s_barrier();
      FAN_STAMP(3);
      if constexpr (kLast) {
        int vnn = vn;
        if constexpr (CHAIN) {
          chain_decide();
          vnn = ch_cont ? ch_next : -1;
          if (vnn >= 0) next_offsets(vnn);
        }
        block(I1{}, F_{}, F_{}, smem, 0, 0, csk, T_{}, vnn >= 0);
      } else {
        if constexpr (!decltype(more_c)::value && !decltype(more2_c)::value) chain_decide();
        else chain_hook(kt);
        block(I1{}, more_c, more2_c, smem + ((kt + 1) & 1) * STAGE, 0, kt + 2, csk, F_{});
        if constexpr (decltype(more_c)::value) waitcnt_known<63, 0>();
      }
    } else {
      block(I0{}, T_{}, more2_c, st, 1, kt + 2, csk, F_{});
      FAN_STAMP(1);
      if constexpr (decltype(more2_c)::value) waitcnt_known<G, 0>();
      else waitcnt_known<0, 0>();
      FAN_STAMP(2);
      __builtin_amdgcn_s_barrier();
      FAN_STAMP(3);
      if constexpr (!decltype(more_c)::value && !decltype(more2_c)::value) chain_decide();
      else chain_hook(kt);
      block(I1{}, more_c, F_{}, smem + ((kt + 1) % 3) * STAGE, 0, 0, csk, F_{});
      if constexpr (decltype(more_c)::value) waitcnt_known<63, 0>();
    }
    FAN_STAMP(4);
  };
  int kt = 0;
  for (; kt + 2 < nk; ++kt) ktile(kt, T_{}, T_{});
  if (kt + 1 < nk) ktile(kt++, T_{}, F_{});
  if (kt < nk) ktile(kt, F_{}, F_{});

  asm volatile("s_nop 7\n\ts_nop 7\n\ts_nop 7" ::: "memory");
#pragma unroll
  for (int i = 0; i < MI; ++i)
#pragma unroll
    for (int j = 0; j < NJ; ++j) asm volatile("" : "+a"(acc[i][j]));
  if (COLSUM && do_colsum && (!SPLIT || m0 == 0))
    colsum_finish<NJ, WTN, kEpiNone, true>(
        cs, lane, n0 + wn * WTN, ws + (SPLIT ? (int64_t)split_k * M * N + (int64_t)ksplit * N : (int64_t)im * N), wo,
        N);
  if constexpr (OVL) {
    store_tile<MI, NJ, WTN, EPI, TC, ACCUM, SPLIT, kSW, WT>(acc, smem + 2 * STAGE, wave, lane, m0 + wm * WTM,
                                                            n0 + wn * WTN, C, ldc, bias, aux, ldaux, M, N, ksplit, ws,
                                                            wo);
  } else {
    asm volatile("s_waitcnt vmcnt(0)" ::: "memory");
    __syncthreads();
    store_tile<MI, NJ, WTN, EPI, TC, ACCUM, SPLIT, WTN, WT>(acc, smem, wave, lane, m0 + wm * WTM, n0 + wn * WTN, C,
                                                            ldc, bias, aux, ldaux, M, N, ksplit, ws, wo);
  }
  };
  if constexpr (CHAIN) {
    int v = chs->ticket;
    for (bool first = true;; first = false) {
      tile_body(v, first, -1);
      if (cr.sig_word0 >= 0) {
        int r, c;
        chain_rc(cr, cr.tn, v - cr.first, r, c);
        chs->pending = cr.sig_word0 + r * 16;
      }
      chs->ticket = ch_next;
      chs->ready = ch_rdy;
      if constexpr (!OVL) __syncthreads();
      if (!ch_cont) break;
      v = ch_next;
    }
  } else if constexpr (COLSUM) {
    if (v0 < tiles * split_k) tile_body(v0, true, -1);
  } else {
    for (int v = v0; v < tiles * split_k; v += vstep) {
      tile_body(v, v == v0, v + vstep < tiles * split_k ? v + vstep : -1);
      if constexpr (!OVL) __syncthreads();
    }
  }
}

template <bool AK, bool BKC, int EPI, typename TC, bool ACCUM, bool SPLIT, bool COLSUM = false, int BN_ = 256,
          int BM_ = 256, bool OVL = false>
__global__ void __launch_bounds__(256, 1)
    gemm_pl4_kernel(const bf16_t* __restrict__ A, int64_t lda, const bf16_t* __restrict__ B, int64_t ldb,
                    TC* __restrict__ C, int64_t ldc, const bf16_t* __restrict__ bias, const TC* __restrict__ aux,
                    int64_t ldaux, int M, int N, int K, int split_k, float* __restrict__ ws,
                    float* __restrict__ colsum, WireOut wo) {
  pl4_run<AK, BKC, EPI, TC, ACCUM, SPLIT, COLSUM, BN_, BM_, OVL>(A, lda, B, ldb, C, ldc, bias, aux, ldaux, M,
                                                                           N, K, split_k, ws, colsum, wo,
                                                                           (int)blockIdx.x, (int)gridDim.x);
}

template <typename TC>
struct PlProblem {
  const bf16_t* A;
  int64_t lda;
  const bf16_t* B;
  int64_t ldb;
  TC* C;
  int64_t ldc;
  const bf16_t* bias;
  const TC* aux;
  int64_t ldaux;
  int M, N, K, split_k;
  float* ws;
  float* colsum;
  WireOut wo;
};

template <bool AK, bool BKC, int EPI, typename TC_, bool ACCUM, bool SPLIT, bool COLSUM, int BN_, int BM_ = 256>
struct PlCfg {
  using TC = TC_;
  static constexpr int kLds = (BN_ == 128 ? 3 : 2) * (BM_ + BN_) * BK * 2;
  static constexpr int kBM = BM_, kBN = BN_;
  __device__ static __forceinline__ void run(const PlProblem<TC>& p, int v0, int vstep) {
    pl4_run<AK, BKC, EPI, TC, ACCUM, SPLIT, COLSUM, BN_, BM_>(p.A, p.lda, p.B, p.ldb, p.C, p.ldc, p.bias, p.aux,
                                                             p.ldaux, p.M, p.N, p.K, p.split_k, p.ws, p.colsum, p.wo,
                                                             v0, vstep);
  }
};

constexpr int kMaxGroup = 8;
template <typename TC>
struct PlGroup {
  PlProblem<TC> p[kMaxGroup];
  int first[kMaxGroup + 1];
  int n;
};

template <class P>
__global__ void __launch_bounds__(256, 1) gemm_groupn_kernel(PlGroup<typename P::TC> g) {
  const int b = (int)blockIdx.x;
  int i = 0;
  while (i + 1 < g.n && b >= g.first[i + 1]) ++i;
  P::run(g.p[i], b - g.first[i], g.first[i + 1] - g.first[i]);
}

template <int EPI, typename TC, bool ACCUM, int SK = 0>
__global__ void __launch_bounds__(256)
    splitk_reduce_kernel(const float* __restrict__ ws, int split_k, TC* __restrict__ C, int64_t ldc,
                         const bf16_t* __restrict__ bias, const TC* __restrict__ aux, int64_t ldaux, int M, int N) {
  const int64_t total4 = (int64_t)M * N / 4;
  const int sk = SK > 0 ? SK : split_k;
  for (int64_t i = blockIdx.x * (int64_t)blockDim.x + threadIdx.x; i < total4; i += (int64_t)gridDim.x * blockDim.x) {
    const int64_t e = i * 4;
    const int row = (int)(e / N), col = (int)(e % N);
    float4 s = reinterpret_cast<const float4*>(ws)[i];
#pragma unroll
    for (int k = 1; k < (SK > 0 ? SK : sk); ++k) {
      const float4 t = reinterpret_cast<const float4*>(ws + (int64_t)k * M * N)[i];
      s.x += t.x; s.y += t.y; s.z += t.z; s.w += t.w;
    }
    float v[4] = {s.x, s.y, s.z, s.w};
    epi4<EPI, TC, ACCUM>(v, C, ldc, bias, aux, ldaux, row, col);
  }
}

template <bool UPD, int SK = 0>
__global__ void __launch_bounds__(256)
    splitk_reduce_wire_kernel(const float* __restrict__ ws, int split_k, float* __restrict__ C, int64_t ldc, int M,
                              int N, float* __restrict__ colsum, WireOut wo) {
  if constexpr (SK > 0) split_k = SK;
  const int gpr = N / 16;
  const int64_t groups = (int64_t)M * gpr;
  const int64_t total = groups + (colsum ? gpr : 0);
  const int64_t slab = (int64_t)M * N;
  for (int64_t g = blockIdx.x * (int64_t)blockDim.x + threadIdx.x; g < total; g += (int64_t)gridDim.x * blockDim.x) {
    const bool bias = g >= groups;
    const int row = bias ? -1 : (int)(g / gpr);
    const int col = (int)((bias ? g - groups : g % gpr) * 16);
    const float* p = bias ? ws + (int64_t)split_k * slab + col : ws + (int64_t)row * N + col;
    const int64_t stride = bias ? N : slab;
    float v[16];
#pragma unroll
    for (int u = 0; u < 16; u += 4) {
      const float4 q = *reinterpret_cast<const float4*>(p + u);
      v[u] = q.x; v[u + 1] = q.y; v[u + 2] = q.z; v[u + 3] = q.w;
    }
#pragma unroll
    for (int k = 1; k < (SK > 0 ? SK : split_k); ++k) {
#pragma unroll
      for (int u = 0; u < 16; u += 4) {
        const float4 q = *reinterpret_cast<const float4*>(p + k * stride + u);
        v[u] += q.x; v[u + 1] += q.y; v[u + 2] += q.z; v[u + 3] += q.w;
      }
    }
    if (!bias) {
      wire_epi16<UPD>(v, C, ldc, wo, row, col);
    } else {
#pragma unroll
      for (int u = 0; u < 16; ++u) colsum[col + u] = v[u];
      if (wo.bias_off > 0) wire_store16<UPD>(v, (uint32_t)wo.bias_off + (uint32_t)col, wo);
    }
  }
}

struct ColsumGroup {
  const float* part[kMaxGroup];
  float* colsum[kMaxGroup];
  WireOut wo[kMaxGroup];
  int parts[kMaxGroup];
  int N[kMaxGroup];
  int first[kMaxGroup + 1];
  int n;
};
template <bool WIRE, bool UPD>
__device__ __forceinline__ void colsum_reduce_block(const float* __restrict__ part, int parts,
                                                    float* __restrict__ colsum, int N, const WireOut& wo, int blk);

__device__ __forceinline__ void local_update4(float v[4], uint32_t E, uint32_t f, const WireOut& wo) {
  float4 a = *reinterpret_cast<const float4*>(wo.um + f);
  float w[4] = {a.x, a.y, a.z, a.w}, m[4] = {0.f, 0.f, 0.f, 0.f};
  const bool hm = wo.umom != nullptr;
  if (hm) {
    const float4 b = *reinterpret_cast<const float4*>(wo.umom + f);
    m[0] = b.x; m[1] = b.y; m[2] = b.z; m[3] = b.w;
  }
#pragma unroll
  for (int u = 0; u < 4; ++u) sgd_apply(wire_roundtrip_rne(v[u], E), w[u], m[u], hm, wo.up);
  *reinterpret_cast<float4*>(wo.um + f) = make_float4(w[0], w[1], w[2], w[3]);
  if (hm) *reinterpret_cast<float4*>(wo.umom + f) = make_float4(m[0], m[1], m[2], m[3]);
  if (wo.ulp) *reinterpret_cast<uint2*>(wo.ulp + f) = make_uint2(pack_bf16x2(w[0], w[1]), pack_bf16x2(w[2], w[3]));
}

template <bool UPD, int SK = 0, bool QCS = false>
__global__ void __launch_bounds__(256)
    splitk_reduce_wire4_kernel(const float* __restrict__ ws, int split_k, float* __restrict__ C, int64_t ldc, int M,
                               int N, float* __restrict__ colsum, WireOut wo, ColsumGroup qcs) {
  int bid = (int)blockIdx.x, nb = (int)gridDim.x;
  if constexpr (QCS) {
    const int nq = qcs.first[qcs.n];
    if (bid < nq) {
      int i = 0;
      while (i + 1 < qcs.n && bid >= qcs.first[i + 1]) ++i;
      colsum_reduce_block<true, true>(qcs.part[i], qcs.parts[i], qcs.colsum[i], qcs.N[i], qcs.wo[i],
                                      bid - qcs.first[i]);
      return;
    }
    bid -= nq;
    nb -= nq;
  }
  if constexpr (SK > 0) split_k = SK;
  const int64_t slab = (int64_t)M * N, quads = slab / 4;
  const int64_t t0 = bid * (int64_t)blockDim.x + threadIdx.x, step = (int64_t)nb * blockDim.x;
  for (int64_t q = t0; q < quads; q += step) {
    const int64_t e = q * 4;
    const int row = (int)(e / N), col = (int)(e % N);
    float4 a = *reinterpret_cast<const float4*>(ws + e);
#pragma unroll
    for (int k = 1; k < (SK > 0 ? SK : split_k); ++k) {
      const float4 b = *reinterpret_cast<const float4*>(ws + k * slab + e);
      a.x += b.x; a.y += b.y; a.z += b.z; a.w += b.w;
    }
    float v[4] = {a.x, a.y, a.z, a.w};
    uint32_t mx = 0;
#pragma unroll
    for (int u = 0; u < 4; ++u) mx = max(mx, __float_as_uint(v[u]) & 0x7FFFFFFFu);
    mx = max(mx, (uint32_t)__shfl_xor((int)mx, 1));
    mx = max(mx, (uint32_t)__shfl_xor((int)mx, 2));
    const uint32_t E = mx >> 23;
    const uint32_t loc = (uint32_t)row * (uint32_t)ldc + (uint32_t)col;
    if constexpr (UPD) {
      local_update4(v, E, wo.off + loc, wo);
    } else {
      const int sub = (col & 15) >> 2;
      const uint32_t fg = wo.off + loc - 4u * (uint32_t)sub;
      const int sh = wire_shard_of(fg, wo);
      const uint32_t pos = fg - (uint32_t)sh * (uint32_t)wo.shard;
      uint32_t w = 0;
#pragma unroll
      for (int u = 0; u < 4; ++u) w |= ((uint32_t)wire_encode(v[u], E, wo.codec) & 0xFFu) << (8 * u);
      uint8_t* base = wire_shard_base(sh, wo);
      *reinterpret_cast<uint32_t*>(base + pos + 4 * sub) = w;
      if (sub == 0) base[wo.shard + pos / 16] = (uint8_t)E;
      if (wo.own == kWireOwnAll || (wo.period > 0 ? sh % wo.period : sh) == wo.own)
        *reinterpret_cast<float4*>(C + loc) = a;
    }
  }
  if (colsum) {
    for (int64_t g = t0; g < N / 16; g += step) {
      const int col = (int)g * 16;
      const float* p = ws + (int64_t)split_k * slab + col;
      float v[16];
#pragma unroll
      for (int u = 0; u < 16; u += 4) {
        const float4 b = *reinterpret_cast<const float4*>(p + u);
        v[u] = b.x; v[u + 1] = b.y; v[u + 2] = b.z; v[u + 3] = b.w;
      }
      for (int k = 1; k < split_k; ++k) {
#pragma unroll
        for (int u = 0; u < 16; u += 4) {
          const float4 b = *reinterpret_cast<const float4*>(p + (int64_t)k * N + u);
          v[u] += b.x; v[u + 1] += b.y; v[u + 2] += b.z; v[u + 3] += b.w;
        }
      }
#pragma unroll
      for (int u = 0; u < 16; ++u) colsum[col + u] = v[u];
      if (wo.bias_off > 0) wire_store16<UPD>(v, (uint32_t)wo.bias_off + (uint32_t)col, wo);
    }
  }
}

template <bool WIRE, bool UPD>
__device__ __forceinline__ void colsum_reduce_block(const float* __restrict__ part, int parts,
                                                    float* __restrict__ colsum, int N, const WireOut& wo, int blk) {
  __shared__ float4 red[16][16];
  __shared__ float fin[64];
  const int t = threadIdx.x, cg = t & 15, pc = t >> 4;
  const int col = blk * 64 + cg * 4;
  float4 acc = make_float4(0.f, 0.f, 0.f, 0.f);
  if (col < N) {
    for (int p = pc; p < parts; p += 16) {
      const float4 q = *reinterpret_cast<const float4*>(part + (int64_t)p * N + col);
      acc.x += q.x; acc.y += q.y; acc.z += q.z; acc.w += q.w;
    }
  }
  red[pc][cg] = acc;
  __syncthreads();
  if (t < 16) {
    float4 s = red[0][t];
    for (int c = 1; c < 16; ++c) {
      const float4 q = red[c][t];
      s.x += q.x; s.y += q.y; s.z += q.z; s.w += q.w;
    }
    fin[t * 4] = s.x; fin[t * 4 + 1] = s.y; fin[t * 4 + 2] = s.z; fin[t * 4 + 3] = s.w;
    if (col < N) *reinterpret_cast<float4*>(colsum + col) = s;
  }
  if constexpr (WIRE) {
    __syncthreads();
    const int c16 = blk * 64 + t * 16;
    if (t < 4 && c16 < N && wo.bias_off > 0) {
      float v[16];
#pragma unroll
      for (int u = 0; u < 16; ++u) v[u] = fin[t * 16 + u];
      wire_store16<UPD>(v, (uint32_t)wo.bias_off + (uint32_t)c16, wo);
    }
  }
}

template <bool WIRE, bool UPD = false>
__global__ void __launch_bounds__(256)
    colsum_reduce_kernel(const float* __restrict__ part, int parts, float* __restrict__ colsum, int N, WireOut wo) {
  colsum_reduce_block<WIRE, UPD>(part, parts, colsum, N, wo, (int)blockIdx.x);
}

template <bool WIRE, bool UPD = false>
__global__ void __launch_bounds__(256) colsum_reduce_group_kernel(ColsumGroup g) {
  const int b = (int)blockIdx.x;
  int i = 0;
  while (i + 1 < g.n && b >= g.first[i + 1]) ++i;
  colsum_reduce_block<WIRE, UPD>(g.part[i], g.parts[i], g.colsum[i], g.N[i], g.wo[i], b - g.first[i]);
}

}
}
```

### csrc/gemm/gemm_bf16_plan.hip

```cpp
#include "gemm/gemm_bf16_launch.h"

#include <algorithm>
#include <cstdio>
#include <map>
#include <mutex>
#include <vector>

namespace fan {

static std::atomic<void*> g_stamp_buffer{nullptr};
void* gemm_stamp_buffer() { return g_stamp_buffer.load(std::memory_order_relaxed); }
void gemm_set_stamp_buffer(void* p) {
#ifdef FAN_GEMM_STAMPS
  g_stamp_buffer.store(p);
#else
  (void)p;
  FAN_CHECK(false, "built without FAN_GEMM_STAMPS");
#endif
}

using gemm_detail::BK;
using gemm_detail::kDefaultWaves;
using gemm_detail::launch_tile;

namespace gemm_detail {
extern template void launch_tile<false, false>(const GemmArgs&, int, int, int, int, hipStream_t);
extern template void launch_tile<false, true>(const GemmArgs&, int, int, int, int, hipStream_t);
extern template void launch_tile<true, false>(const GemmArgs&, int, int, int, int, hipStream_t);
extern template void launch_tile<true, true>(const GemmArgs&, int, int, int, int, hipStream_t);
}

namespace gemm_detail {
namespace {
std::mutex g_pend_mu;
std::map<hipStream_t, std::vector<PendingColsum>>& pend_map() {
  static std::map<hipStream_t, std::vector<PendingColsum>> m;
  return m;
}
}

void push_pending_colsum(hipStream_t s, const PendingColsum& p) {
  std::lock_guard<std::mutex> g(g_pend_mu);
  pend_map()[s].push_back(p);
}

ColsumGroup take_pending_colsum(hipStream_t s) {
  ColsumGroup g{};
  std::lock_guard<std::mutex> lk(g_pend_mu);
  auto it = pend_map().find(s);
  if (it == pend_map().end() || it->second.empty()) return g;
  auto& v = it->second;
  const int n = (int)std::min<size_t>(v.size(), kMaxGroup);
  int blocks = 0;
  for (int i = 0; i < n; ++i) {
    g.part[i] = v[i].part;
    g.parts[i] = v[i].parts;
    g.colsum[i] = v[i].colsum;
    g.N[i] = v[i].N;
    g.wo[i] = v[i].wo;
    g.first[i] = blocks;
    blocks += cdiv_i(v[i].N, 64);
  }
  g.first[n] = blocks;
  g.n = n;
  v.erase(v.begin(), v.begin() + n);
  return g;
}
}

int gemm_flush_colsum(hipStream_t s) {
  int ran = 0;
  for (;;) {
    const gemm_detail::ColsumGroup g = gemm_detail::take_pending_colsum(s);
    if (g.n == 0) return ran;
    hipLaunchKernelGGL((gemm_detail::colsum_reduce_group_kernel<true, true>), g.first[g.n], 256, 0, s, g);
    ran += g.n;
  }
}

int gemm_pending_colsum(hipStream_t s) {
  std::lock_guard<std::mutex> g(gemm_detail::g_pend_mu);
  auto it = gemm_detail::pend_map().find(s);
  return it == gemm_detail::pend_map().end() ? 0 : (int)it->second.size();
}

std::atomic<int>& gemm_prio_flag() {
  static std::atomic<int> flag{[] {
    const char* e = getenv("FAN_GEMM_PRIO");
    return e && e[0] == '0' ? 0 : 1;
  }()};
  return flag;
}

std::atomic<int>& gemm_ovl_flag() {
  static std::atomic<int> flag{[] {
    const char* e = getenv("FAN_GEMM_OVL");
    return e && e[0] == '0' ? 0 : 1;
  }()};
  return flag;
}

std::atomic<int>& gemm_reduce4_flag() {
  static std::atomic<int> flag{[] {
    const char* e = getenv("FAN_GEMM_REDUCE4");
    return e && e[0] == '0' ? 0 : 1;
  }()};
  return flag;
}

std::atomic<int>& gemm_main_loop_flag() {
  static std::atomic<int> flag{[] {
    const char* pl = getenv("FAN_GEMM_PL");
    const int m = pl && pl[0] >= '0' && pl[0] <= '5' ? pl[0] - '0' : 2;
    return m == 1 || m == 4 ? 2 : m;
  }()};
  return flag;
}

std::atomic<int>& gemm_persist_flag() {
  static std::atomic<int> flag{[] {
    const char* e = getenv("FAN_GEMM_PERSIST");
    return e ? atoi(e) : kNumCU;
  }()};
  return flag;
}

struct TunedPlan {
  int M, N, K, bm, bn, sk;
};
static constexpr TunedPlan kTuned[] = {
    {4096, 3072, 768, 256, 256, 1},
    {3072, 768, 4096, 256, 256, 4},
    {768, 3072, 4096, 256, 256, 4},
    {768, 768, 4096, 128, 128, 4},
    {768, 2304, 4096, 128, 256, 4},
};

struct EnvPlans {
  std::vector<TunedPlan> plans;
  bool bad = false;
};
static const EnvPlans& env_plans() {
  static const EnvPlans ep = [] {
    EnvPlans r;
    const char* e = getenv("FAN_GEMM_PLAN");
    for (const char* q = e; q && *q;) {
      TunedPlan t{};
      int used = 0;
      if (sscanf(q, "%dx%dx%d=%d,%d,%d%n", &t.M, &t.N, &t.K, &t.bm, &t.bn, &t.sk, &used) != 6 ||
          (t.bm != 128 && t.bm != 256 && t.bm != 224) || (t.bn != 128 && t.bn != 256) ||
          (t.bm == 224 && t.bn != 128) || t.sk < 1) {
        r.bad = true;
        break;
      }
      r.plans.push_back(t);
      q += used;
      if (*q == ';') ++q;
    }
    return r;
  }();
  FAN_CHECK(!ep.bad, "FAN_GEMM_PLAN: expected MxNxK=bm,bn,sk[;...] with bm, bn in {128, 256} (or 224x128)");
  return ep;
}

static GemmPlan plan_ragged(int M, int N, int K, int split_k, int tile_bm, int tile_bn) {
  GemmPlan p{0, 0, 1, kDefaultWaves};
  const int cand[4][2] = {{256, 256}, {128, 256}, {256, 128}, {128, 128}};
  auto pad_ok = [](int x, int b) { return (int64_t)((x + b - 1) / b) * b * 100 <= (int64_t)x * 115; };
  int best = 3;
  for (int c = 0; c < 4; ++c) {
    const int bm = cand[c][0], bn = cand[c][1];
    if (tile_bm > 0) {
      if (bm == tile_bm && bn == tile_bn) best = c;
      continue;
    }
    const int tiles = ((M + bm - 1) / bm) * ((N + bn - 1) / bn);
    if (tiles >= kNumCU && pad_ok(M, bm) && pad_ok(N, bn)) {
      best = c;
      break;
    }
  }
  p.bm = cand[best][0];
  p.bn = cand[best][1];
  const int tiles = ((M + p.bm - 1) / p.bm) * ((N + p.bn - 1) / p.bn);
  const int nkt = (K + BK - 1) / BK;
  int sk = 1;
  if (split_k > 0) {
    sk = split_k;
    if (sk > nkt) return GemmPlan{0, 0, 1, kDefaultWaves};
  } else if (tiles * 2 <= kNumCU) {
    while (tiles * sk < kNumCU && sk < 8 && nkt / (sk * 2) >= 8) sk *= 2;
  }
  p.split_k = sk;
  return p;
}

GemmPlan gemm_bf16_plan(int M, int N, int K, int split_k, int tile_bm, int tile_bn, int tile_waves) {
  GemmPlan p{0, 0, 1, 8};
  if (M <= 0 || N <= 0 || K <= 0 || M % 8 || N % 8 || K % 8) return p;
  if (tile_bm == 224) {
    const int sk = split_k > 0 ? split_k : 1;
    if (tile_bn != 128 || M % 224 || N % 128 || K % (BK * sk)) return p;
    return GemmPlan{224, 128, sk, kDefaultWaves};
  }
  if (tile_bm != 0 && ((tile_bm != 128 && tile_bm != 256) || (tile_bn != 128 && tile_bn != 256))) return p;
  if (tile_bm == 0 && split_k <= 0) {
    for (const TunedPlan& t : env_plans().plans)
      if (t.bm == 224 && t.M == M && t.N == N && t.K == K) return gemm_bf16_plan(M, N, K, t.sk, 224, 128, 0);
  }
  if (M % 128 || N % 128 || K % BK ||
      (tile_bm > 0 && (M % tile_bm || N % tile_bn)) || (split_k > 1 && K % (BK * split_k)))
    return plan_ragged(M, N, K, split_k, tile_bm, tile_bn);
  if (tile_bm == 0 && split_k <= 0) {
    for (const TunedPlan& t : env_plans().plans) {
      if (t.M == M && t.N == N && t.K == K && M % t.bm == 0 && N % t.bn == 0 && K % (BK * t.sk) == 0) {
        p.bm = t.bm;
        p.bn = t.bn;
        p.split_k = t.sk;
        p.waves = kDefaultWaves;
        return p;
      }
    }
    for (const TunedPlan& t : kTuned) {
      if (t.M == M && t.N == N && t.K == K && K % (BK * t.sk) == 0) {
        p.bm = t.bm;
        p.bn = t.bn;
        p.split_k = t.sk;
        p.waves = kDefaultWaves;
        return p;
      }
    }
  }
  const int cand[4][2] = {{256, 256}, {256, 128}, {128, 256}, {128, 128}};
  int best = -1;
  for (int c = 0; c < 4 && best < 0; ++c) {
    const int bm = cand[c][0], bn = cand[c][1];
    if (M % bm || N % bn) continue;
    if (tile_bm > 0 && (bm != tile_bm || bn != tile_bn)) continue;
    if (tile_bm > 0 || (M / bm) * (N / bn) >= kNumCU) best = c;
  }
  if (best < 0) {
    for (int c = 3; c >= 0 && best < 0; --c) {
      const int bm = cand[c][0], bn = cand[c][1];
      if (M % bm || N % bn) continue;
      if (tile_bm > 0 && (bm != tile_bm || bn != tile_bn)) continue;
      best = c;
    }
  }
  if (best < 0) return p;
  int sk = 1;
  if (tile_bm == 0 && split_k <= 0 && best == 3 && M % 256 == 0 && N % 256 == 0) {
    const int t256 = (M / 256) * (N / 256);
    int s = 1;
    while (t256 * s < kNumCU && K % (BK * s * 2) == 0 && K / (s * 2) >= 1024) s *= 2;
    if (t256 * s >= kNumCU) {
      best = 0;
      sk = s;
    }
  }
  const int tiles = (M / cand[best][0]) * (N / cand[best][1]);
  if (sk > 1) {
  } else if (split_k > 0) {
    sk = split_k;
    if (K % (BK * sk)) return p;
  } else if (tiles * 2 <= kNumCU) {
    while (tiles * sk < kNumCU && sk < 8 && K % (BK * sk * 2) == 0 && K / (sk * 2) >= 512) sk *= 2;
  }
  p.bm = cand[best][0];
  p.bn = cand[best][1];
  p.split_k = sk;
#ifdef FAN_GEMM_4WAVE
  p.waves = tile_waves == 4 || tile_waves == 8 ? tile_waves : kDefaultWaves;
#else
  p.waves = kDefaultWaves;
  (void)tile_waves;
#endif
  return p;
}

bool gemm_bf16_supported(const GemmArgs& a) {
  const GemmPlan p = gemm_bf16_plan(a.M, a.N, a.K, a.split_k, a.tile_bm, a.tile_bn, a.tile_waves);
  if (p.bm == 0) return false;
  if (a.lda % 8 || a.ldb % 8 || a.ldc % 4 || (a.aux && a.ldaux % 4)) return false;
  if (((uintptr_t)a.A | (uintptr_t)a.B) & 15) return false;
  if (((uintptr_t)a.C) & (a.c_bf16 ? 7 : 15)) return false;
  if (a.accumulate && a.c_bf16) return false;
  if (p.split_k > 1 && a.workspace == nullptr) return false;
  if (a.colsum && a.b_kcontig) return false;
  if (p.bm == 224 && (!a.a_kcontig || a.colsum)) return false;
  if (a.epilogue == kEpiWire) {
    if (a.a_kcontig || a.b_kcontig || a.c_bf16 || a.accumulate || !a.wire || a.N % 16) return false;
    if (a.wire_shard <= 0 || a.wire_shard % 256 || a.ldc % 16) return false;
    if (a.wire_codec != kBfpTrunc && a.wire_codec != kBfpRne) return false;
    if (a.wire_off < 0 || a.wire_off % 16 || a.wire_off + (int64_t)a.M * a.ldc + a.N >= (int64_t(1) << 31))
      return false;
  }
  return true;
}

void launch_gemm_bf16(const GemmArgs& a, hipStream_t s) {
  FAN_CHECK(gemm_bf16_supported(a), "gemm_bf16: unsupported shape/layout (need M, N, K % 8 == 0)");
  const GemmPlan p = gemm_bf16_plan(a.M, a.N, a.K, a.split_k, a.tile_bm, a.tile_bn, a.tile_waves);
  if (a.c_bf16 && !a.wire) {
    const bool mask = a.epilogue == kEpiReluMask;
    const bool bias = a.epilogue == kEpiBias || a.epilogue == kEpiBiasRelu;
    FAN_CHECK(((uintptr_t)a.C & 15) == 0 && a.ldc % 8 == 0 && (!bias || ((uintptr_t)a.bias & 15) == 0) &&
                  (!mask || (((uintptr_t)a.aux & 15) == 0 && a.ldaux % 8 == 0)),
              "gemm_bf16: bf16 output, bias and activation must be 16-B aligned with ldc, ldaux % 8 == 0");
  }
  if (a.a_kcontig && a.b_kcontig) launch_tile<true, true>(a, p.bm, p.bn, p.waves, p.split_k, s);
  else if (a.a_kcontig && !a.b_kcontig) launch_tile<true, false>(a, p.bm, p.bn, p.waves, p.split_k, s);
  else if (!a.a_kcontig && a.b_kcontig) launch_tile<false, true>(a, p.bm, p.bn, p.waves, p.split_k, s);
  else launch_tile<false, false>(a, p.bm, p.bn, p.waves, p.split_k, s);
  FAN_HIP_CHECK(hipGetLastError());
}

}
```

### csrc/gemm/gemm_group.h

```cpp
#pragma once
#include "gemm/gemm.h"

namespace fan {

constexpr int kGroupMax = 8;
bool gemm_wgrad_group_supported(const GemmArgs* a, int n);
int64_t gemm_wgrad_group_ws(const GemmArgs& a);
void launch_gemm_wgrad_group(const GemmArgs* a, int n, hipStream_t stream);

}
```

### csrc/gemm/gemm_group.hip

```cpp
#include "gemm/gemm_bf16_kernel.h"
#include "gemm/gemm_group.h"

namespace fan {

using namespace gemm_detail;

namespace {

template <typename TC>
PlProblem<TC> problem_of(const GemmArgs& a, const WireOut& wo) {
  return PlProblem<TC>{(const bf16_t*)a.A, a.lda, (const bf16_t*)a.B, a.ldb, (TC*)a.C, a.ldc, (const bf16_t*)a.bias,
                       (const TC*)a.aux, a.ldaux, a.M, a.N, a.K, 1, (float*)a.workspace, a.colsum, wo};
}

WireOut wire_of(const GemmArgs& a) {
  WireOut wo{};
  wo.prio = gemm_prio_flag().load(std::memory_order_relaxed);
  if (a.wire) {
    wo.p = a.wire;
    wo.shard = a.wire_shard;
    wo.own = a.wire_own;
    wo.period = a.wire_period;
    wo.codec = a.wire_codec;
    wo.inv_shard = a.wire_shard > 0 ? 1.0f / (float)a.wire_shard : 0.f;
    wo.bias_off = a.colsum ? (int)(a.wire_off + (int64_t)a.M * a.ldc) : 0;
    wo.off = (uint32_t)a.wire_off;
  }
  return wo;
}

template <int EPI>
void launch_wgrad_group(const GemmArgs* a, int n, hipStream_t s) {
  using P = PlCfg<false, false, EPI, float, false, false, true, 128, 256>;
  PlGroup<float> g{};
  ColsumGroup cg{};
  g.n = cg.n = n;
  int wg = 0, cb = 0;
  for (int i = 0; i < n; ++i) {
    const WireOut wo = wire_of(a[i]);
    g.p[i] = problem_of<float>(a[i], wo);
    g.first[i] = wg;
    const int tiles = (a[i].M / 256) * (a[i].N / 128);
    wg += (tiles + kNumXCD - 1) / kNumXCD * kNumXCD;
    cg.part[i] = (const float*)a[i].workspace;
    cg.parts[i] = a[i].M / 256;
    cg.colsum[i] = a[i].colsum;
    cg.wo[i] = wo;
    cg.N[i] = a[i].N;
    cg.first[i] = cb;
    cb += (a[i].N + 63) / 64;
  }
  g.first[n] = wg;
  cg.first[n] = cb;
  auto k = gemm_groupn_kernel<P>;
  FAN_HIP_CHECK(hipFuncSetAttribute((const void*)k, hipFuncAttributeMaxDynamicSharedMemorySize, P::kLds));
  hipLaunchKernelGGL(k, wg, 256, P::kLds, s, g);
  FAN_HIP_CHECK(hipGetLastError());
  hipLaunchKernelGGL((colsum_reduce_group_kernel<is_wire_epi(EPI)>), cb, 256, 0, s, cg);
  FAN_HIP_CHECK(hipGetLastError());
}

}

int64_t gemm_wgrad_group_ws(const GemmArgs& a) { return (int64_t)(a.M / 256) * a.N; }

bool gemm_wgrad_group_supported(const GemmArgs* a, int n) {
  static_assert(kGroupMax == kMaxGroup, "group capacity");
  if (n < 1 || n > kGroupMax) return false;
  int64_t wg = 0;
  for (int i = 0; i < n; ++i) {
    const GemmArgs& g = a[i];
    if (g.a_kcontig || g.b_kcontig || g.c_bf16 || g.accumulate || !g.colsum || !g.workspace) return false;
    if (g.epilogue != a[0].epilogue || (g.epilogue != kEpiNone && g.epilogue != kEpiWire)) return false;
    if (g.M <= 0 || g.N <= 0 || g.M % 256 || g.N % 128 || g.K <= 0 || g.K % 64 || g.ldc < g.N) return false;
    if (g.lda % 8 || g.ldb % 8 || g.ldc % 4 || ((uintptr_t)g.C & 15) || ((uintptr_t)g.colsum & 15)) return false;
    if (g.epilogue == kEpiWire) {
      if (!g.wire || g.wire_shard <= 0 || g.wire_shard % 256 || g.wire_off < 0 || g.wire_off % 16 || g.upd_master)
        return false;
      if (g.wire_off + (int64_t)g.M * g.ldc + g.N >= (1ll << 31)) return false;
    }
    wg += ((int64_t)(g.M / 256) * (g.N / 128) + kNumXCD - 1) / kNumXCD * kNumXCD;
  }
  return wg <= 64 * kNumCU;
}

void launch_gemm_wgrad_group(const GemmArgs* a, int n, hipStream_t s) {
  FAN_CHECK(gemm_wgrad_group_supported(a, n), "gemm_wgrad_group: unsupported shapes / layouts / epilogues");
  if (a[0].epilogue == kEpiWire) launch_wgrad_group<kEpiWire>(a, n, s);
  else launch_wgrad_group<kEpiNone>(a, n, s);
}

}
```

### fpga_ai_nic_amd/models/mlp.py

```python
from __future__ import annotations


import math
from dataclasses import dataclass

import torch

from ..ops import gemm as G
from ..ops import nn as NN


@dataclass
class LayerBucket:
    cin: int
    cout: int
    n: int
    n_pad: int
    master: torch.Tensor
    grad: torch.Tensor
    lp: torch.Tensor | None
    mom: torch.Tensor | None

    @property
    def w_master(self):
        return self.master[: self.cin * self.cout].view(self.cin, self.cout)

    @property
    def b_master(self):
        return self.master[self.cin * self.cout: self.n]

    @property
    def w(self):
        src = self.lp if self.lp is not None else self.master
        return src[: self.cin * self.cout].view(self.cin, self.cout)

    @property
    def b(self):
        src = self.lp if self.lp is not None else self.master
        return src[self.cin * self.cout: self.n]

    @property
    def gw(self):
        return self.grad[: self.cin * self.cout].view(self.cin, self.cout)

    @property
    def gb(self):
        return self.grad[self.cin * self.cout: self.n]


class MLP:

    def __init__(self, sizes, *, dtype=torch.bfloat16, device="cpu", pad_fn=None, seed: int = 1,
                 momentum: bool = False, init_scale: float | None = None, bias: bool = True,
                 relu: str = "hidden"):
        if len(sizes) < 2:
            raise ValueError("need at least one layer")
        if relu not in ("hidden", "all", "none"):
            raise ValueError(f"relu must be hidden|all|none, got {relu!r}")
        self.bias, self.relu = bias, relu
        self.sizes = list(sizes)
        self.L = len(sizes) - 1
        self.dtype = dtype
        self.device = torch.device(device)
        pad_fn = pad_fn or (lambda n: (n + 255) // 256 * 256)
        gen = torch.Generator().manual_seed(seed)
        self.layers: list[LayerBucket] = []
        for i in range(self.L):
            cin, cout = sizes[i], sizes[i + 1]
            n = cin * cout + cout
            n_pad = pad_fn(n)
            master = torch.zeros(n_pad, dtype=torch.float32)
            bound = init_scale if init_scale is not None else 1.0 / math.sqrt(cin)
            master[: cin * cout] = (torch.rand(cin * cout, generator=gen) * 2 - 1) * bound
            b0 = (torch.rand(cout, generator=gen) * 2 - 1) * bound
            master[cin * cout: n] = b0 if bias else 0.0
            master = master.to(self.device)
            lp = master.to(torch.bfloat16) if dtype == torch.bfloat16 else None
            grad = torch.zeros(n_pad, dtype=torch.float32, device=self.device)
            mom = torch.zeros(n_pad, dtype=torch.float32, device=self.device) if momentum else None
            self.layers.append(LayerBucket(cin, cout, n, n_pad, master, grad, lp, mom))
        self._act_mb = None
        self._zero_b: dict[int, torch.Tensor] = {}

    def _relu_at(self, i: int) -> bool:
        return self.relu == "all" or (self.relu == "hidden" and i + 1 < self.L)

    def _bias_of(self, l: LayerBucket):
        if self.bias:
            return l.b
        z = self._zero_b.get(l.cout)
        if z is None:
            z = self._zero_b[l.cout] = torch.zeros(l.cout, dtype=l.b.dtype, device=self.device)
        return z

    def num_params(self) -> int:
        return sum(l.n for l in self.layers)

    def flops_per_sample(self) -> int:
        f = 0
        for i, l in enumerate(self.layers):
            f += (6 if i > 0 else 4) * l.cin * l.cout
        return f

    def sync_lp(self):
        for l in self.layers:
            if l.lp is not None:
                l.lp.copy_(l.master.to(torch.bfloat16))

    def state_dict(self):
        out = {}
        for i, l in enumerate(self.layers):
            out[f"fc{i}.weight"] = l.w_master.detach().clone()
            out[f"fc{i}.bias"] = l.b_master.detach().clone()
        return out

    def load_state_dict(self, sd):
        for i, l in enumerate(self.layers):
            l.w_master.copy_(sd[f"fc{i}.weight"].to(l.master.dtype))
            l.b_master.copy_(sd[f"fc{i}.bias"].to(l.master.dtype))
        self.sync_lp()

    def repad(self, i: int, n_pad: int):
        l = self.layers[i]
        if n_pad <= l.n_pad:
            return

        def grow(t):
            if t is None:
                return None
            u = torch.zeros(n_pad, dtype=t.dtype, device=t.device)
            u[: l.n_pad] = t
            return u

        l.master, l.grad, l.lp, l.mom = grow(l.master), grow(l.grad), grow(l.lp), grow(l.mom)
        l.n_pad = n_pad

    def alloc_activations(self, mb: int):
        if self._act_mb == mb:
            return
        adt = self.dtype
        dev = self.device
        self.act = [torch.empty(mb, c, dtype=adt, device=dev) for c in self.sizes[:-1]]
        self.logits = torch.empty(mb, self.sizes[-1], dtype=torch.float32, device=dev)
        self.dz = [None] + [torch.empty(mb, c, dtype=adt, device=dev) for c in self.sizes[1:]]
        self.loss_rows = torch.empty(mb, dtype=torch.float32, device=dev)
        self._act_mb = mb

    def forward_layer(self, i: int, fold_logits: bool = False):
        l = self.layers[i]
        out = self.act[i + 1] if i + 1 < self.L else self.logits
        self._slabs = None
        if fold_logits and i + 1 == self.L and out.is_cuda and self.dtype == torch.bfloat16 and not self._relu_at(i):
            self._slabs = {}
        G.linear_fwd(self.act[i], l.w, self._bias_of(l), out, relu=self._relu_at(i), defer_reduce=self._slabs)

    def forward_chain(self) -> bool:
        if not (self.device.type == "cuda" and self.dtype == torch.bfloat16 and self.L >= 2):
            return False
        outs = [self.act[i + 1] for i in range(self.L - 1)] + [self.logits]
        epis = [G.EPI_BIAS_RELU if self._relu_at(i) else G.EPI_BIAS for i in range(self.L)]
        return G.linear_chain(G.CHAIN_FWD, self.act[0], [l.w for l in self.layers], outs,
                              biases=[self._bias_of(l) for l in self.layers], epis=epis, key=("fwd", id(self)))

    def backward_data_chain(self) -> bool:
        if not (self.device.type == "cuda" and self.dtype == torch.bfloat16 and self.L >= 3):
            return False
        if not all(self._relu_at(i - 1) for i in range(1, self.L)):
            return False
        idx = list(range(self.L - 1, 0, -1))
        return G.linear_chain(G.CHAIN_BWD_DATA, self.dz[self.L], [self.layers[i].w for i in idx],
                              [self.dz[i] for i in idx], auxes=[self.act[i] for i in idx], key=("bwd", id(self)))

    def loss_backward(self, labels, grad_scale: float):
        slabs, self._slabs = getattr(self, "_slabs", None), None
        if slabs:
            NN.softmax_xent_slabs(slabs, self._bias_of(self.layers[-1]), self.logits, labels, self.dz[self.L],
                                  self.loss_rows, grad_scale)
        else:
            NN.softmax_xent(self.logits, labels, self.dz[self.L], self.loss_rows, grad_scale)
        if self._relu_at(self.L - 1):
            self.dz[self.L].mul_(self.logits > 0)

    def backward_weight(self, i: int, wire=None, update=None, defer_colsum=False):
        l = self.layers[i]
        if wire is not None:
            G.linear_bwd_weight(self.act[i], self.dz[i + 1], l.gw, bias_grad=l.gb if self.bias else None, wire=wire,
                                update=update, defer_colsum=defer_colsum)
        elif not self.bias:
            G.linear_bwd_weight(self.act[i], self.dz[i + 1], l.gw)
        elif l.gw.is_cuda and self.dtype == torch.bfloat16:
            G.linear_bwd_weight(self.act[i], self.dz[i + 1], l.gw, bias_grad=l.gb)
        else:
            G.linear_bwd_weight(self.act[i], self.dz[i + 1], l.gw)
            NN.col_sum(self.dz[i + 1], l.gb)

    def backward_data(self, i: int):
        if i == 0:
            return
        l = self.layers[i]
        G.linear_bwd_data(self.dz[i + 1], l.w, self.dz[i], relu_input=self.act[i] if self._relu_at(i - 1) else None)

    def forward(self, x):
        self.alloc_activations(x.shape[0])
        self.act[0].copy_(x)
        for i in range(self.L):
            self.forward_layer(i)
        return self.logits
```

### fpga_ai_nic_amd/ops/gemm.py

```python
from __future__ import annotations

import torch

from .. import _ext

EPI_NONE, EPI_BIAS, EPI_BIAS_RELU, EPI_RELU_MASK, EPI_WIRE = 0, 1, 2, 3, 4

_ws: dict = {}


def _workspace(device, numel):
    key = (device, torch.cuda.current_stream(device).cuda_stream if device.type == "cuda" else 0)
    t = _ws.get(key)
    if t is None or t.numel() < numel:
        t = torch.empty(max(numel, 1 << 20), dtype=torch.float32, device=device)
        _ws[key] = t
    return t


def _bf16_ws_floats(M: int, N: int, sk: int, bm: int, colsum) -> int:
    return (sk * M * N if sk > 1 else 0) + (sk * (-(-M // bm)) * N if colsum is not None else 0)


def choose_split_k(M: int, N: int, K: int, target_wg: int = 256) -> int:
    tiles = (M // 128) * (N // 128)
    if tiles == 0:
        return 1
    best = 1
    for s in (2, 3, 4, 6, 8):
        if tiles * best >= target_wg:
            break
        if K % (64 * s) == 0 and K // s >= 256:
            best = s
    return best


def gemm(A, a_t: bool, B, b_t: bool, C, epilogue: int = EPI_NONE, bias=None, aux=None, accumulate=False,
         split_k: int | None = None, tile: tuple | None = None, colsum=None, wire=None, update=None,
         defer_colsum: bool = False, defer_reduce: dict | None = None):
    if wire is not None:
        if not C.is_cuda or A.dtype != torch.bfloat16 or not a_t or b_t:
            raise ValueError("wire epilogue: bf16 GPU bwd-weight layout only")
        _bf16(_ext.require(), A, a_t, B, b_t, C, EPI_WIRE, None, None, False, split_k, tile, colsum, wire, update,
              defer_colsum=defer_colsum)
        return C
    if update is not None:
        raise ValueError("update needs the wire epilogue")
    if C.is_cuda:
        Cx = _ext.require()
        if colsum is not None and (A.dtype != torch.bfloat16 or b_t):
            from . import nn as _nn

            gemm(A, a_t, B, b_t, C, epilogue, bias, aux, accumulate, split_k, tile)
            _nn.col_sum(B.t() if b_t else B, colsum)
            return C
        if A.dtype == torch.bfloat16:
            if C.dtype == torch.bfloat16 and not _aligned16(C, bias, aux if epilogue == EPI_RELU_MASK else None):
                Ct = torch.empty(C.shape, dtype=C.dtype, device=C.device)
                if accumulate:
                    Ct.copy_(C)
                _bf16(Cx, A, a_t, B, b_t, Ct, epilogue, None if bias is None else bias.clone(),
                      aux if aux is None or epilogue != EPI_RELU_MASK else aux.contiguous().clone(), accumulate,
                      split_k, tile, colsum, None)
                C.copy_(Ct)
                return C
            _bf16(Cx, A, a_t, B, b_t, C, epilogue, bias, aux, accumulate, split_k, tile, colsum, None,
                  defer_reduce=defer_reduce)
            return C
        M = A.shape[1] if a_t else A.shape[0]
        K = A.shape[0] if a_t else A.shape[1]
        N = B.shape[0] if b_t else B.shape[1]
        ws = None
        tbm, tbn, tw = (tuple(tile) + (0,))[:3] if tile is not None else (0, 0, 0)
        sk = Cx.gemm_f32_split(M, N, K, 0 if split_k is None else int(split_k))
        if sk > 1:
            ws = _workspace(C.device, sk * M * N)
        Cx.gemm(A, a_t, B, b_t, C, epilogue, bias, aux, accumulate, sk, ws, tbm, tbn, colsum, tw)
        return C
    a = (A.t() if a_t else A).float()
    b = (B.t() if b_t else B).float()
    r = a @ b
    if epilogue in (EPI_BIAS, EPI_BIAS_RELU):
        r = r + bias.float()
    if epilogue == EPI_BIAS_RELU:
        r = torch.relu(r)
    if epilogue == EPI_RELU_MASK:
        r = r * (aux.float() > 0)
    if accumulate:
        r = r + C.float()
    C.copy_(r.to(C.dtype))
    if colsum is not None:
        colsum.copy_(b.sum(0).to(colsum.dtype))
    return C


def wgrad_group_supported(problems) -> bool:
    if not 1 <= len(problems) <= 8:
        return False
    for p in problems:
        X, dY = p[0], p[1]
        K, M, N = X.shape[0], X.shape[1], dY.shape[1]
        if M % 256 or N % 128 or K % 64 or dY.shape[0] != K or X.dtype != torch.bfloat16 or not X.is_cuda:
            return False
    return True


def gemm_wgrad_group(problems, wire=None):
    Cx = _ext.require()
    Xs = [p[0] for p in problems]
    dYs = [p[1] for p in problems]
    Cs = [p[2] for p in problems]
    css = [p[3] for p in problems]
    offs = [int(p[4]) if len(p) > 4 else 0 for p in problems]
    ws = _workspace(Cs[0].device, Cx.gemm_wgrad_group_ws([(x.shape[1], y.shape[1]) for x, y in zip(Xs, dYs)]))
    if wire is None:
        Cx.gemm_wgrad_group(Xs, dYs, Cs, css, offs, ws)
    else:
        buf, shard, own, codec = wire[:4]
        period = wire[4] if len(wire) > 4 else 0
        Cx.gemm_wgrad_group(Xs, dYs, Cs, css, offs, ws, buf, int(shard), int(own), int(codec), int(period))


def _aligned16(C, bias, aux) -> bool:
    ok = C.data_ptr() % 16 == 0 and C.stride(0) % 8 == 0
    if bias is not None:
        ok = ok and bias.data_ptr() % 16 == 0
    if aux is not None:
        ok = ok and aux.data_ptr() % 16 == 0 and aux.stride(0) % 8 == 0
    return ok


def _shares_storage(C, *ts) -> bool:
    c = C.untyped_storage().data_ptr()
    return any(t is not None and t.untyped_storage().data_ptr() == c for t in ts)


class LocalUpdate:

    __slots__ = ("master", "lp", "mom", "lr", "grad_scale", "weight_decay", "momentum", "nesterov")

    def __init__(self, master, lp=None, mom=None, *, lr, grad_scale=1.0, weight_decay=0.0, momentum=0.0,
                 nesterov=False):
        self.master, self.lp, self.mom = master, lp, mom
        self.lr, self.grad_scale, self.weight_decay = float(lr), float(grad_scale), float(weight_decay)
        self.momentum, self.nesterov = float(momentum), bool(nesterov)

    def kwargs(self):
        return dict(upd_master=self.master, upd_lp=self.lp, upd_mom=self.mom, upd_lr=self.lr,
                    upd_grad_scale=self.grad_scale, upd_weight_decay=self.weight_decay, upd_momentum=self.momentum,
                    upd_nesterov=self.nesterov)


_defer_ws: dict = {}


def _colsum_ws(Cx, device, colsum, numel):
    key = (device, torch.cuda.current_stream(device).cuda_stream, colsum.data_ptr())
    t = _defer_ws.get(key)
    if t is None or t.numel() < numel:
        if t is not None:
            Cx.gemm_flush_colsum()
        t = torch.empty(numel, dtype=torch.float32, device=device)
        _defer_ws[key] = t
    return t


def _slab_ws(device, numel):
    key = ("slabs", device, torch.cuda.current_stream(device).cuda_stream)
    t = _defer_ws.get(key)
    if t is None or t.numel() < numel:
        t = torch.empty(numel, dtype=torch.float32, device=device)
        _defer_ws[key] = t
    return t


def flush_colsum() -> int:
    if not torch.cuda.is_available():
        return 0
    return int(_ext.require().gemm_flush_colsum())


def pending_colsum() -> int:
    return int(_ext.require().gemm_pending_colsum()) if torch.cuda.is_available() else 0


def _bf16(Cx, A, a_t, B, b_t, C, epilogue, bias, aux, accumulate, split_k, tile, colsum, wire, update=None,
          defer_colsum=False, defer_reduce=None):
    M = A.shape[1] if a_t else A.shape[0]
    K = A.shape[0] if a_t else A.shape[1]
    N = B.shape[0] if b_t else B.shape[1]
    tbm, tbn, tw = (tuple(tile) + (0,))[:3] if tile is not None else (0, 0, 0)
    sk0 = 0 if split_k is None else int(split_k)
    static = Cx.gemm_plan(M, N, K, sk0, tbm, tbn, tw)
    if static[0] == 0:
        raise ValueError(f"gemm: unsupported bf16 shape M={M} N={N} K={K} split_k={split_k} tile={tile}")
    if wire is not None:
        buf, shard, own, codec = wire[:4]
        period = int(wire[4]) if len(wire) > 4 else 0
        woff = int(wire[5]) if len(wire) > 5 else 0

    def run(plan, waves=0, upd=None, final=False):
        bm, bn, sk = plan
        need = _bf16_ws_floats(M, N, sk, bm, colsum)
        defer = bool(defer_colsum and upd is not None and colsum is not None and sk == 1)
        dred = bool(final and defer_reduce is not None and sk > 1 and epilogue == EPI_BIAS and colsum is None
                    and C.dtype == torch.float32 and not accumulate)
        if dred:
            ws = _slab_ws(C.device, need)
        else:
            ws = (_colsum_ws(Cx, C.device, colsum, need) if defer else _workspace(C.device, need)) if need else None
        if wire is not None:
            Cx.gemm(A, a_t, B, b_t, C, EPI_WIRE, None, None, False, sk, ws, bm, bn, colsum, waves, buf, int(shard),
                    int(own), int(codec), period, woff, **(upd.kwargs() if upd is not None else {}),
                    defer_colsum=defer)
        else:
            Cx.gemm(A, a_t, B, b_t, C, epilogue, bias, aux, accumulate, sk, ws, bm, bn, colsum, waves,
                    defer_reduce=dred)
            if dred:
                defer_reduce.update(ws=ws, sk=sk)

    from . import gemm_tune

    T = gemm_tune.tuner()
    if (tile is not None or split_k is not None or not T.enabled or accumulate
            or _shares_storage(C, A, B, aux, bias)):
        run(tuple(static[:3]), tw, update, final=True)
        return
    k = T.key(M, N, K, a_t, b_t, epilogue, colsum is not None, 0 if wire is None else 1, C.device)
    plan = T.lookup(k)
    if torch.cuda.is_current_stream_capturing():
        run(plan if plan is not None else tuple(static[:3]), 0, update, final=True)
        return
    if plan is None and not T.worth_tuning(M, N, static, C.device):
        plan = T.keep_static(k, static)
    if plan is None:
        plan = T.tune(k, static, T.candidates(Cx, M, N, K, a_kcontig=not a_t, colsum=colsum is not None), run)
        if update is not None:
            run(plan, 0, update)
    else:
        run(plan, 0, update, final=True)


CHAIN_FWD, CHAIN_BWD_DATA = 0, 1
_chain_ctr: dict = {}


def chain_enabled() -> bool:
    import os

    return os.environ.get("FAN_GEMM_CHAIN", "0") == "1"


def _chain_counters(key, device, n: int, M: int):
    Cx = _ext.require()
    words = int(Cx.gemm_chain_words(n, M))
    sk = (key, device, torch.cuda.current_stream(device).cuda_stream)
    t = _chain_ctr.get(sk)
    if t is None or t.numel() < words:
        if torch.cuda.is_current_stream_capturing():
            return None
        t = torch.zeros(words, dtype=torch.int32, device=device)
        _chain_ctr[sk] = t
    return t


def chain_error(key=None) -> int:
    worst = 0
    for (k, _, _), t in _chain_ctr.items():
        if key is None or k == key:
            worst = max(worst, int(t[9 * 16].item()))
    return worst


def linear_chain(kind: int, a0, ws, outs, biases=None, auxes=None, epis=None, key="chain", dry_run=False) -> bool:
    if not (chain_enabled() and a0.is_cuda and a0.dtype == torch.bfloat16 and 1 <= len(ws) <= 8):
        return False
    n = len(ws)
    biases = list(biases) if biases is not None else [None] * n
    auxes = list(auxes) if auxes is not None else [None] * n
    epis = list(epis) if epis is not None else [EPI_RELU_MASK if kind == CHAIN_BWD_DATA else EPI_BIAS_RELU] * n
    ctr = _chain_counters(key, a0.device, n, a0.shape[0])
    if ctr is None:
        return False
    return bool(_ext.require().gemm_chain(kind, a0, list(ws), list(outs), biases, auxes, [int(e) for e in epis], ctr,
                                          dry_run))


def linear_fwd(x, w, b, out, relu: bool, defer_reduce: dict | None = None):
    return gemm(x, False, w, False, out, EPI_BIAS_RELU if relu else EPI_BIAS, bias=b,
                defer_reduce=None if relu else defer_reduce)


def linear_bwd_data(dz, w, out, relu_input=None):
    if relu_input is not None:
        return gemm(dz, False, w, True, out, EPI_RELU_MASK, aux=relu_input)
    return gemm(dz, False, w, True, out, EPI_NONE)


def linear_bwd_weight(x, dz, out, accumulate=False, bias_grad=None, wire=None, update=None, defer_colsum=False):
    if wire is not None:
        return gemm(x, True, dz, False, out, EPI_WIRE, colsum=bias_grad, wire=wire, update=update,
                    defer_colsum=defer_colsum)
    return gemm(x, True, dz, False, out, EPI_NONE, accumulate=accumulate, colsum=bias_grad)
```

### fpga_ai_nic_amd/parallel/dp.py

```python
from __future__ import annotations

import os
import time

import torch

from ..models.mlp import MLP
from ..ops import gemm as G
from ..ops import wire
from ..utils import tracing
from .allreduce import CompressedAllReduce, Handle, _round_up
from .transport import Transport


class RcclAllReduce(CompressedAllReduce):

    def __init__(self, transport: Transport, **kw):
        kw.pop("codec", None)
        kw.pop("algo", None)
        super().__init__(transport, codec="raw_f32", algo="mesh", **kw)
        self.algo = "rccl"

    def layout(self, n):
        from .allreduce import BucketLayout

        n_pad = _round_up(max(n, 1), 256 * self.world)
        return BucketLayout(n=n, n_pad=n_pad, algo="rccl", world=self.world, shard=n_pad)

    def wire_bytes(self, L):
        N = self.world
        return 0 if N == 1 else int(2 * (N - 1) / N * L.n_pad * 4)

    def _run(self, L, grad, finish, owner_fp32, allow_compat=True):
        g = grad.view(-1)[: L.n_pad]
        self.transport.all_reduce_(g)
        return [lambda: finish(wire.as_bytes(g), L.n_pad, 1, 0, L.n_pad)]


def make_engine(transport: Transport | None, kind: str = "bfp", *, rounding: str = "rne", algo: str = "mesh",
                rings: int = 1, max_slice_elems: int = 1 << 22, compat_owner_fp32: bool = False,
                timeout_s: float = 600.0, force_comm: bool = False, impl: str = "python", comm=None,
                side_stream: bool = False, ring_sub: int = 0, shard_update: bool | None = None):
    if kind == "local" or transport is None:
        return None
    if kind == "rccl":
        return RcclAllReduce(transport, timeout_s=timeout_s, force_comm=force_comm)
    codec = {"bfp": f"bfp_{rounding}", "raw": "raw_f32", "raw_bf16": "raw_bf16"}[kind]
    if impl == "native":
        from .native_engine import NativeAllReduce

        return NativeAllReduce(transport, codec=codec, algo=algo, rings=rings, max_slice_elems=max_slice_elems,
                               compat_owner_fp32=compat_owner_fp32, timeout_s=timeout_s, force_comm=force_comm,
                               comm=comm, side_stream=side_stream, ring_sub=ring_sub, shard_update=shard_update)
    return CompressedAllReduce(transport, codec=codec, algo=algo, rings=rings, max_slice_elems=max_slice_elems,
                               compat_owner_fp32=compat_owner_fp32, timeout_s=timeout_s, force_comm=force_comm)


class DataParallelTrainer:
    def __init__(self, model: MLP, engine: CompressedAllReduce | None, *, lr: float = 0.1,
                 weight_decay: float = 0.0, momentum: float = 0.0, nesterov: bool = False,
                 loss_scale: float = 1.0, average: bool = True, profile: bool = False, prepack: bool = True,
                 commit_at_end: bool | None = None, fused_update: bool | None = None,
                 gemm_inflight: str | None = None):
        self.m = model
        self.engine = engine
        self.world = engine.world if engine is not None else 1
        self.lr, self.wd, self.momentum, self.nesterov = lr, weight_decay, momentum, nesterov
        self.loss_scale = loss_scale
        self.grad_scale = (1.0 / self.world) if average else 1.0
        self.pending: list[Handle | None] = [None] * model.L
        self.last_handle: Handle | None = None
        self.cuda = model.device.type == "cuda"
        self.profile = profile
        self.times = {"fwd": 0.0, "loss": 0.0, "bwd": 0.0, "bwd_first": 0.0, "steps": 0}
        self.step_count = 0
        self.commit_at_end = (bool(getattr(engine, "epilogue_on_producer", False)) if commit_at_end is None
                              else commit_at_end)
        self.prepack = (prepack and engine is not None and getattr(engine, "prepack", False) and self.cuda
                        and model.dtype == torch.bfloat16)
        fu = os.environ.get("FAN_FUSED_UPDATE", "1") != "0" if fused_update is None else bool(fused_update)
        self.fused_update = (fu and self.prepack and bool(getattr(engine, "inline", False))
                             and getattr(engine, "codec", "") == "bfp_rne")
        self.fused_updates = 0
        self.defer_colsum = os.environ.get("FAN_DEFER_COLSUM", "1") != "0"
        self.fold_logits = os.environ.get("FAN_FOLD_LOGITS", "1") != "0"
        self.chain_fwd = G.chain_enabled()
        self.chain_bwd = G.chain_enabled()
        gi = os.environ.get("FAN_GEMM_INFLIGHT", "persistent") if gemm_inflight is None else gemm_inflight
        if gi not in ("persistent", "grid"):
            raise ValueError(f"gemm_inflight must be persistent|grid, got {gi!r}")
        self.gemm_inflight = gi if (self.cuda and engine is not None and not getattr(engine, "inline", True)) \
            else "persistent"
        self._persist_saved = None
        self.shard = bool(getattr(engine, "shard_update", False)) and self.cuda and model.dtype == torch.bfloat16
        self.lp_next = [l.lp.clone() if self.shard else None for l in model.layers]
        self.last_on_producer = (self.cuda and engine is not None and not getattr(engine, "inline", True)
                                 and hasattr(engine, "C") and os.environ.get("FAN_LAST_ON_PRODUCER", "1") != "0")

    def _sgd_local(self, l):
        wire.sgd(wire.as_bytes(l.grad), l.n_pad, 1, l.master, codec="raw_f32", lp=l.lp, mom=l.mom, lr=self.lr,
                 grad_scale=self.grad_scale, weight_decay=self.wd, momentum=self.momentum, nesterov=self.nesterov,
                 n_valid=l.n)

    def step(self, x: torch.Tensor, labels: torch.Tensor):
        self.forward_pass(x)
        self.backward_pass(labels)
        self.times["steps"] += 1
        self.step_count += 1
        return self.m.loss_rows

    def forward_pass(self, x: torch.Tensor):
        m = self.m
        m.alloc_activations(x.shape[0])
        m.act[0] = x
        t0 = time.perf_counter()
        with tracing.range("fwd"):
            if self.cuda and self.chain_fwd:
                for i in range(m.L):
                    self._wait_layer(i)
                chained = m.forward_chain()
            else:
                chained = False
            if not chained:
                for i in range(m.L):
                    self._wait_layer(i)
                    m.forward_layer(i, fold_logits=self.fold_logits and self.cuda)
            self.last_handle = None
        if self.profile:
            self._sync()
            self.times["fwd"] += time.perf_counter() - t0

    def _wait_layer(self, i: int):
        h = self.pending[i]
        if h is None:
            return
        for x in (h if isinstance(h, list) else [h]):
            if self.cuda:
                x.wait()
            else:
                x.synchronize()
        self.pending[i] = None

    def _wait_updates(self):
        for i in range(self.m.L):
            self._wait_layer(i)
        self.last_handle = None

    def backward_pass(self, labels: torch.Tensor):
        m = self.m
        prof = self.profile
        self._wait_updates()
        t0 = time.perf_counter()
        with tracing.range("loss"):
            m.loss_backward(labels, grad_scale=self.loss_scale / m.act[0].shape[0])
        if prof:
            self._sync()
            t1 = time.perf_counter()
            self.times["loss"] += t1 - t0
            t0 = t1
        tgts = [(self.engine.prepack_target(l.grad, l.n, None if m.bias else l.cin * l.cout)
                 if self.prepack and l.cout % 16 == 0 else None) for l in m.layers]
        chained = (self.fused_update and self.chain_bwd and all(t is not None for t in tgts)
                   and m.backward_data_chain())
        try:
            for i in reversed(range(m.L)):
                l = m.layers[i]
                with tracing.range(f"bwd{i}"):
                    tgt = tgts[i]
                    if tgt is not None and self.fused_update:
                        if not chained:
                            m.backward_data(i)
                        upd = G.LocalUpdate(l.master, l.lp, l.mom, lr=self.lr, grad_scale=self.grad_scale,
                                            weight_decay=self.wd, momentum=self.momentum, nesterov=self.nesterov)
                        m.backward_weight(i, wire=tgt, update=upd, defer_colsum=self.defer_colsum)
                        self.fused_updates += 1
                    else:
                        m.backward_weight(i, wire=tgt)
                        h = None
                        if self.engine is not None:
                            kw = {"prepacked": (tgt[0], l.n_pad)} if tgt is not None else {}
                            lp_out = self.lp_next[i] if self.shard else l.lp
                            if i == 0 and self.last_on_producer:
                                kw["on_producer"] = True
                            h = self.engine.allreduce_sgd(l.grad, l.master, lp_out, l.mom, n_valid=l.n, lr=self.lr,
                                                          grad_scale=self.grad_scale, weight_decay=self.wd,
                                                          momentum=self.momentum, nesterov=self.nesterov, defer=True,
                                                          name=f"fc{i}", **kw)
                            self._gemm_grid(True)
                        m.backward_data(i)
                        if h is not None:
                            self.pending[i] = h if self.commit_at_end else h.commit_after_current()
                            self.last_handle = self.pending[i]
                        else:
                            self._sgd_local(l)
                if prof and i == m.L - 1:
                    self._sync()
                    t1 = time.perf_counter()
                    self.times["bwd_first"] += t1 - t0
                    self.times["bwd"] += t1 - t0
                    t0 = t1
        finally:
            if self.fused_updates and self.defer_colsum and self.cuda:
                G.flush_colsum()
            self._gemm_grid(False)
        if self.shard:
            for i, l in enumerate(m.layers):
                l.lp, self.lp_next[i] = self.lp_next[i], l.lp
        if self.commit_at_end:
            for i in reversed(range(m.L)):
                h = self.pending[i]
                for x in (h if isinstance(h, list) else [] if h is None else [h]):
                    x.commit_after_current()
        if prof:
            self._sync()
            self.times["bwd"] += time.perf_counter() - t0

    def _gemm_grid(self, on: bool):
        if self.gemm_inflight != "grid":
            return
        from .. import _ext

        C = _ext.require()
        if on and self._persist_saved is None:
            self._persist_saved = C.gemm_persist()
            C.gemm_set_persist(0)
        elif not on and self._persist_saved is not None:
            C.gemm_set_persist(self._persist_saved)
            self._persist_saved = None

    def _sync(self):
        if self.cuda:
            torch.cuda.synchronize()

    def finish_async(self):
        self._wait_updates()

    def gather_state(self):
        if not self.shard:
            return
        self.finish()
        for l in self.m.layers:
            self.engine.gather_owned(l.master, l.n)
            if l.mom is not None:
                self.engine.gather_owned(l.mom, l.n)

    def finish(self, timeout: float | None = None):
        self._gemm_grid(False)
        for i, h in enumerate(self.pending):
            if h is not None:
                for x in (h if isinstance(h, list) else [h]):
                    x.synchronize(timeout)
                self.pending[i] = None
        self.last_handle = None
        self._sync()
```

Baseline: 8.329 million samples/s.

## Group postponed split-K weight-gradient GEMMs into one dispatch with grouped slab reduce

Weight-gradient GEMMs whose static plan is split-K with 256x256 tiles are postponed until the end of backward. They are then launched together as a single grouped split-K dispatch, followed by one grouped slab-reduce kernel that applies the wire epilogue and fused SGD. The aim is to fill the CUs with tiles from several small-tile-count problems at once and to cut the number of launches and reductions. In exchange the weight updates run later, lose overlap with backward-data work, and need a larger workspace.

```diff
diff --git a/csrc/bindings_ops.cpp b/csrc/bindings_ops.cpp
--- a/csrc/bindings_ops.cpp
+++ b/csrc/bindings_ops.cpp
@@ -20,6 +20,45 @@
   TORCH_CHECK(t.dim() == 2, "expected a 2-D tensor");
   TORCH_CHECK(t.stride(1) == 1, "expected unit stride in the last dim");
   return t.stride(0);
+}
+
+void set_wire(GemmArgs& g, const c10::optional<at::Tensor>& wire, int64_t wire_shard, int64_t wire_own,
+              int64_t wire_codec, int64_t wire_period, int64_t wire_off, const c10::optional<at::Tensor>& upd_master,
+              const c10::optional<at::Tensor>& upd_lp, const c10::optional<at::Tensor>& upd_mom,
+              const SgdParams& upd) {
+  TORCH_CHECK(wire && wire->is_cuda() && wire->is_contiguous() && wire->scalar_type() == at::kByte,
+              "wire epilogue needs a contiguous uint8 GPU wire buffer");
+  TORCH_CHECK(wire_shard > 0 && wire_shard % 256 == 0, "wire_shard must be a positive multiple of 256");
+  TORCH_CHECK(wire_off >= 0 && wire_off % 16 == 0, "wire_off must be a non-negative multiple of 16");
+  const int64_t last = wire_off + (g.colsum ? (int64_t)g.M * g.ldc + g.N - 1 : (int64_t)(g.M - 1) * g.ldc + g.N - 1);
+  const int64_t need = (last / wire_shard + 1) * (int64_t)wire_shard_bytes((int)wire_codec, (size_t)wire_shard);
+  TORCH_CHECK(wire->numel() >= need, "wire buffer too small: ", wire->numel(), " < ", need);
+  g.wire = wire->data_ptr<uint8_t>();
+  g.wire_shard = wire_shard;
+  g.wire_own = (int)wire_own;
+  g.wire_period = (int)wire_period;
+  g.wire_codec = (int)wire_codec;
+  g.wire_off = wire_off;
+  if (upd_master) {
+    auto plane = [&](const at::Tensor& t, at::ScalarType st, const char* what) {
+      TORCH_CHECK(t.is_cuda() && t.is_contiguous() && t.scalar_type() == st && t.numel() > last &&
+                      t.data_ptr() != nullptr && (reinterpret_cast<uintptr_t>(t.data_ptr()) & 15) == 0,
+                  "fused update: ", what, " must be a contiguous, 16-B aligned GPU plane covering the bucket");
+    };
+    TORCH_CHECK(wire_own == -1, "fused update: no owner shard (single-rank engine)");
+    TORCH_CHECK(wire_codec == kBfpRne, "fused update: rne codec only");
+    plane(*upd_master, at::kFloat, "master");
+    g.upd_master = upd_master->data_ptr<float>();
+    if (upd_lp) {
+      plane(*upd_lp, at::kBFloat16, "lp");
+      g.upd_lp = reinterpret_cast<bf16_t*>(upd_lp->data_ptr());
+    }
+    if (upd_mom) {
+      plane(*upd_mom, at::kFloat, "mom");
+      g.upd_mom = upd_mom->data_ptr<float>();
+    }
+    g.upd = upd;
+  }
 }
 
 void gemm(const at::Tensor& A, bool a_t, const at::Tensor& B, bool b_t, at::Tensor& C, int64_t epilogue,
@@ -74,41 +113,10 @@
   }
   if (workspace) g.workspace = workspace->data_ptr();
   if (epilogue == kEpiWire) {
-    TORCH_CHECK(wire && wire->is_cuda() && wire->is_contiguous() && wire->scalar_type() == at::kByte,
-                "wire epilogue needs a contiguous uint8 GPU wire buffer");
-    TORCH_CHECK(wire_shard > 0 && wire_shard % 256 == 0, "wire_shard must be a positive multiple of 256");
-    TORCH_CHECK(wire_off >= 0 && wire_off % 16 == 0, "wire_off must be a non-negative multiple of 16");
-    const int64_t last = wire_off + (g.colsum ? (int64_t)g.M * g.ldc + g.N - 1 : (int64_t)(g.M - 1) * g.ldc + g.N - 1);
-    const int64_t need = (last / wire_shard + 1) * (int64_t)wire_shard_bytes((int)wire_codec, (size_t)wire_shard);
-    TORCH_CHECK(wire->numel() >= need, "wire buffer too small: ", wire->numel(), " < ", need);
-    g.wire = wire->data_ptr<uint8_t>();
-    g.wire_shard = wire_shard;
-    g.wire_own = (int)wire_own;
-    g.wire_period = (int)wire_period;
-    g.wire_codec = (int)wire_codec;
-    g.wire_off = wire_off;
-    if (upd_master) {
-      auto plane = [&](const at::Tensor& t, at::ScalarType st, const char* what) {
-        TORCH_CHECK(t.is_cuda() && t.is_contiguous() && t.scalar_type() == st && t.numel() > last &&
-                        t.data_ptr() != nullptr && (reinterpret_cast<uintptr_t>(t.data_ptr()) & 15) == 0,
-                    "fused update: ", what, " must be a contiguous, 16-B aligned GPU plane covering the bucket");
-      };
-      TORCH_CHECK(wire_own == -1, "fused update: no owner shard (single-rank engine)");
-      TORCH_CHECK(wire_codec == kBfpRne, "fused update: rne codec only");
-      plane(*upd_master, at::kFloat, "master");
-      g.upd_master = upd_master->data_ptr<float>();
-      if (upd_lp) {
-        plane(*upd_lp, at::kBFloat16, "lp");
-        g.upd_lp = reinterpret_cast<bf16_t*>(upd_lp->data_ptr());
-      }
-      if (upd_mom) {
-        plane(*upd_mom, at::kFloat, "mom");
-        g.upd_mom = upd_mom->data_ptr<float>();
-      }
-      g.upd = SgdParams{(float)upd_lr, (float)upd_grad_scale, (float)upd_weight_decay, (float)upd_momentum,
-                        upd_nesterov ? 1 : 0};
-      g.defer_colsum = defer_colsum && g.colsum != nullptr;
-    }
+    set_wire(g, wire, wire_shard, wire_own, wire_codec, wire_period, wire_off, upd_master, upd_lp, upd_mom,
+             SgdParams{(float)upd_lr, (float)upd_grad_scale, (float)upd_weight_decay, (float)upd_momentum,
+                       upd_nesterov ? 1 : 0});
+    g.defer_colsum = defer_colsum && g.upd_master != nullptr && g.colsum != nullptr;
   }
   if (A.scalar_type() == at::kBFloat16) {
     TORCH_CHECK(bias ? bias->scalar_type() == at::kBFloat16 : true, "bias must be bf16");
@@ -193,6 +201,83 @@
   launch_gemm_wgrad_group(g.data(), (int)n, fan_stream());
 }
 
+void gemm_wgrad_splitk_group(const std::vector<at::Tensor>& Xs, const std::vector<at::Tensor>& dYs,
+                             const std::vector<at::Tensor>& Cs, const std::vector<at::Tensor>& colsums, int64_t split,
+                             at::Tensor& workspace, const std::vector<at::Tensor>& wires,
+                             const std::vector<int64_t>& wire_shards, const std::vector<int64_t>& wire_owns,
+                             const std::vector<int64_t>& wire_periods, const std::vector<int64_t>& wire_offs,
+                             int64_t wire_codec, const std::vector<c10::optional<at::Tensor>>& upd_masters,
+                             const std::vector<c10::optional<at::Tensor>>& upd_lps,
+                             const std::vector<c10::optional<at::Tensor>>& upd_moms, double upd_lr,
+                             double upd_grad_scale, double upd_weight_decay, double upd_momentum, bool upd_nesterov) {
+  const size_t n = Xs.size();
+  TORCH_CHECK(n >= 1 && n <= (size_t)kGroupMax, "gemm_wgrad_splitk_group: 1..", kGroupMax, " problems");
+  TORCH_CHECK(dYs.size() == n && Cs.size() == n && colsums.size() == n && wires.size() == n &&
+                  wire_shards.size() == n && wire_owns.size() == n && wire_periods.size() == n &&
+                  wire_offs.size() == n && upd_masters.size() == n && upd_lps.size() == n && upd_moms.size() == n,
+              "gemm_wgrad_splitk_group: one X, dY, C, colsum, wire target and update entry per problem");
+  TORCH_CHECK(split == 2 || split == 4, "gemm_wgrad_splitk_group: split 2 or 4");
+  TORCH_CHECK(workspace.is_cuda() && workspace.scalar_type() == at::kFloat && workspace.is_contiguous(),
+              "gemm_wgrad_splitk_group: f32 GPU workspace");
+  const SgdParams sgd{(float)upd_lr, (float)upd_grad_scale, (float)upd_weight_decay, (float)upd_momentum,
+                      upd_nesterov ? 1 : 0};
+  std::vector<GemmArgs> g(n);
+  int64_t ws_off = 0;
+  for (size_t i = 0; i < n; ++i) {
+    const at::Tensor &X = Xs[i], &dY = dYs[i], &C = Cs[i], &cs = colsums[i];
+    TORCH_CHECK(X.is_cuda() && dY.is_cuda() && C.is_cuda() && cs.is_cuda(), "gemm_wgrad_splitk_group: GPU tensors");
+    TORCH_CHECK(X.scalar_type() == at::kBFloat16 && dY.scalar_type() == at::kBFloat16 &&
+                    C.scalar_type() == at::kFloat && cs.scalar_type() == at::kFloat && cs.is_contiguous(),
+                "gemm_wgrad_splitk_group: bf16 X / dY, f32 C / colsum");
+    TORCH_CHECK(X.dim() == 2 && dY.dim() == 2 && X.size(0) == dY.size(0) && C.dim() == 2 && C.size(0) == X.size(1) &&
+                    C.size(1) == dY.size(1) && cs.numel() >= dY.size(1),
+                "gemm_wgrad_splitk_group: shapes (X [K][M], dY [K][N], C [M][N], colsum [N])");
+    GemmArgs& a = g[i];
+    a.A = X.data_ptr(); a.lda = ld_of(X);
+    a.B = dY.data_ptr(); a.ldb = ld_of(dY);
+    a.C = C.data_ptr(); a.ldc = ld_of(C);
+    a.M = (int)X.size(1); a.N = (int)dY.size(1); a.K = (int)X.size(0);
+    a.a_kcontig = false; a.b_kcontig = false; a.c_bf16 = false;
+    a.colsum = cs.data_ptr<float>();
+    a.epilogue = kEpiWire;
+    a.split_k = (int)split;
+    a.tile_bm = a.tile_bn = 256;
+    a.workspace = workspace.data_ptr<float>() + ws_off;
+    ws_off += gemm_wgrad_splitk_group_ws(a, (int)split);
+    set_wire(a, wires[i], wire_shards[i], wire_owns[i], wire_codec, wire_periods[i], wire_offs[i], upd_masters[i],
+             upd_lps[i], upd_moms[i], sgd);
+  }
+  TORCH_CHECK(workspace.numel() >= ws_off, "gemm_wgrad_splitk_group: workspace of ", ws_off, " floats needed");
+  TORCH_CHECK(gemm_wgrad_splitk_group_supported(g.data(), (int)n, (int)split),
+              "gemm_wgrad_splitk_group: unsupported (M, N % 256, K % (64 * split), aligned operands, the fused update on "
+              "every problem or none)");
+  launch_gemm_wgrad_splitk_group(g.data(), (int)n, (int)split, fan_stream());
+}
+
+bool gemm_wgrad_splitk_group_shapes_ok(const std::vector<std::tuple<int64_t, int64_t, int64_t>>& mnk, int64_t split) {
+  std::vector<GemmArgs> g(mnk.size());
+  for (size_t i = 0; i < mnk.size(); ++i) {
+    GemmArgs& a = g[i];
+    a.M = (int)std::get<0>(mnk[i]);
+    a.N = (int)std::get<1>(mnk[i]);
+    a.K = (int)std::get<2>(mnk[i]);
+    a.lda = a.M;
+    a.ldb = a.ldc = a.N;
+    a.epilogue = kEpiWire;
+    a.A = a.B = a.C = a.workspace = (void*)16;
+    a.colsum = (float*)16;
+    a.wire = (uint8_t*)16;
+    a.wire_shard = 256;
+  }
+  return gemm_wgrad_splitk_group_supported(g.data(), (int)g.size(), (int)split);
+}
+
+int64_t gemm_wgrad_splitk_group_ws_floats(const std::vector<std::pair<int64_t, int64_t>>& mn, int64_t split) {
+  int64_t w = 0;
+  for (const auto& p : mn) w += split * (p.first * p.second + p.second);
+  return w;
+}
+
 bool gemm_chain(int64_t kind, const at::Tensor& A0, const std::vector<at::Tensor>& Bs, const std::vector<at::Tensor>& Cs,
                 const std::vector<c10::optional<at::Tensor>>& biases,
                 const std::vector<c10::optional<at::Tensor>>& auxes, const std::vector<int64_t>& epis,
@@ -338,6 +423,25 @@
         pybind11::arg("wire_shard") = 0, pybind11::arg("wire_own") = -1, pybind11::arg("wire_codec") = 1,
         pybind11::arg("wire_period") = 0);
   m.def("gemm_wgrad_group_ws", &gemm_wgrad_group_ws_floats, "f32 workspace elements for a group of (M, N) problems");
+  m.def("gemm_wgrad_splitk_group", &gemm_wgrad_splitk_group,
+        "up to 8 bwd-weight GEMMs (256x256 tiles, wire epilogue or fused update) at one split-K count in one "
+        "dispatch + one slab reduce",
+        pybind11::arg("Xs"), pybind11::arg("dYs"), pybind11::arg("Cs"), pybind11::arg("colsums"),
+        pybind11::arg("split"), pybind11::arg("workspace"), pybind11::arg("wires"), pybind11::arg("wire_shards"),
+        pybind11::arg("wire_owns"), pybind11::arg("wire_periods"), pybind11::arg("wire_offs"),
+        pybind11::arg("wire_codec"), pybind11::arg("upd_masters"), pybind11::arg("upd_lps"),
+        pybind11::arg("upd_moms"), pybind11::arg("upd_lr") = 0.0, pybind11::arg("upd_grad_scale") = 1.0,
+        pybind11::arg("upd_weight_decay") = 0.0, pybind11::arg("upd_momentum") = 0.0,
+        pybind11::arg("upd_nesterov") = false);
+  m.def("gemm_wgrad_splitk_group_supported", &gemm_wgrad_splitk_group_shapes_ok,
+        "shape limits of gemm_wgrad_splitk_group for (M, N, K) problems at a common split", pybind11::arg("mnk"),
+        pybind11::arg("split"));
+  m.def("gemm_wgrad_splitk_group_ws", &gemm_wgrad_splitk_group_ws_floats,
+        "f32 workspace elements for a split-K group of (M, N) problems", pybind11::arg("mn"), pybind11::arg("split"));
+  m.def("gemm_plan_overridden", [](int64_t M, int64_t N, int64_t K) {
+          return gemm_bf16_plan_overridden((int)M, (int)N, (int)K);
+        },
+        "the automatic plan of this shape comes from FAN_GEMM_PLAN or the measured table");
   m.def("gemm_chain", &gemm_chain, "the GEMMs of one MLP pass as one persistent launch (row-panel hand-offs)",
         pybind11::arg("kind"), pybind11::arg("A0"), pybind11::arg("Bs"), pybind11::arg("Cs"), pybind11::arg("biases"),
         pybind11::arg("auxes"), pybind11::arg("epis"), pybind11::arg("counters"), pybind11::arg("dry_run") = false);
diff --git a/csrc/gemm/gemm.h b/csrc/gemm/gemm.h
--- a/csrc/gemm/gemm.h
+++ b/csrc/gemm/gemm.h
@@ -55,6 +55,7 @@
 };
 
 GemmPlan gemm_bf16_plan(int M, int N, int K, int split_k, int tile_bm = 0, int tile_bn = 0, int tile_waves = 0);
+bool gemm_bf16_plan_overridden(int M, int N, int K);
 
 bool gemm_bf16_supported(const GemmArgs& a);
 void launch_gemm_bf16(const GemmArgs& a, hipStream_t stream);
diff --git a/csrc/gemm/gemm_bf16_kernel.h b/csrc/gemm/gemm_bf16_kernel.h
--- a/csrc/gemm/gemm_bf16_kernel.h
+++ b/csrc/gemm/gemm_bf16_kernel.h
@@ -1476,23 +1476,11 @@
   if (wo.ulp) *reinterpret_cast<uint2*>(wo.ulp + f) = make_uint2(pack_bf16x2(w[0], w[1]), pack_bf16x2(w[2], w[3]));
 }
 
-template <bool UPD, int SK = 0, bool QCS = false>
-__global__ void __launch_bounds__(256)
-    splitk_reduce_wire4_kernel(const float* __restrict__ ws, int split_k, float* __restrict__ C, int64_t ldc, int M,
-                               int N, float* __restrict__ colsum, WireOut wo, ColsumGroup qcs) {
-  int bid = (int)blockIdx.x, nb = (int)gridDim.x;
-  if constexpr (QCS) {
-    const int nq = qcs.first[qcs.n];
-    if (bid < nq) {
-      int i = 0;
-      while (i + 1 < qcs.n && bid >= qcs.first[i + 1]) ++i;
-      colsum_reduce_block<true, true>(qcs.part[i], qcs.parts[i], qcs.colsum[i], qcs.N[i], qcs.wo[i],
-                                      bid - qcs.first[i]);
-      return;
-    }
-    bid -= nq;
-    nb -= nq;
-  }
+template <bool UPD, int SK>
+__device__ __forceinline__ void splitk_reduce_wire4_run(const float* __restrict__ ws, int split_k,
+                                                        float* __restrict__ C, int64_t ldc, int M, int N,
+                                                        float* __restrict__ colsum, const WireOut& wo, int bid,
+                                                        int nb) {
   if constexpr (SK > 0) split_k = SK;
   const int64_t slab = (int64_t)M * N, quads = slab / 4;
   const int64_t t0 = bid * (int64_t)blockDim.x + threadIdx.x, step = (int64_t)nb * blockDim.x;
@@ -1554,6 +1542,53 @@
   }
 }
 
+__device__ __forceinline__ bool queued_colsum_block(const ColsumGroup& qcs, int bid) {
+  if (bid >= qcs.first[qcs.n]) return false;
+  int i = 0;
+  while (i + 1 < qcs.n && bid >= qcs.first[i + 1]) ++i;
+  colsum_reduce_block<true, true>(qcs.part[i], qcs.parts[i], qcs.colsum[i], qcs.N[i], qcs.wo[i], bid - qcs.first[i]);
+  return true;
+}
+
+template <bool UPD, int SK = 0, bool QCS = false>
+__global__ void __launch_bounds__(256)
+    splitk_reduce_wire4_kernel(const float* __restrict__ ws, int split_k, float* __restrict__ C, int64_t ldc, int M,
+                               int N, float* __restrict__ colsum, WireOut wo, ColsumGroup qcs) {
+  int bid = (int)blockIdx.x, nb = (int)gridDim.x;
+  if constexpr (QCS) {
+    if (queued_colsum_block(qcs, bid)) return;
+    bid -= qcs.first[qcs.n];
+    nb -= qcs.first[qcs.n];
+  }
+  splitk_reduce_wire4_run<UPD, SK>(ws, split_k, C, ldc, M, N, colsum, wo, bid, nb);
+}
+
+struct SlabGroup {
+  const float* ws[kMaxGroup];
+  float* C[kMaxGroup];
+  float* colsum[kMaxGroup];
+  int64_t ldc[kMaxGroup];
+  WireOut wo[kMaxGroup];
+  int M[kMaxGroup];
+  int N[kMaxGroup];
+  int first[kMaxGroup + 1];
+  int n;
+};
+
+template <bool UPD, int SK, bool QCS = false>
+__global__ void __launch_bounds__(256) splitk_reduce_wire4_group_kernel(SlabGroup g, ColsumGroup qcs) {
+  static_assert(SK > 0, "grouped slab reduce: compile-time split count");
+  int bid = (int)blockIdx.x;
+  if constexpr (QCS) {
+    if (queued_colsum_block(qcs, bid)) return;
+    bid -= qcs.first[qcs.n];
+  }
+  int i = 0;
+  while (i + 1 < g.n && bid >= g.first[i + 1]) ++i;
+  splitk_reduce_wire4_run<UPD, SK>(g.ws[i], SK, g.C[i], g.ldc[i], g.M[i], g.N[i], g.colsum[i], g.wo[i],
+                                   bid - g.first[i], g.first[i + 1] - g.first[i]);
+}
+
 template <bool WIRE, bool UPD>
 __device__ __forceinline__ void colsum_reduce_block(const float* __restrict__ part, int parts,
                                                     float* __restrict__ colsum, int N, const WireOut& wo, int blk) {
diff --git a/csrc/gemm/gemm_bf16_plan.hip b/csrc/gemm/gemm_bf16_plan.hip
--- a/csrc/gemm/gemm_bf16_plan.hip
+++ b/csrc/gemm/gemm_bf16_plan.hip
@@ -278,6 +278,14 @@
   return p;
 }
 
+bool gemm_bf16_plan_overridden(int M, int N, int K) {
+  for (const TunedPlan& t : env_plans().plans)
+    if (t.M == M && t.N == N && t.K == K) return true;
+  for (const TunedPlan& t : kTuned)
+    if (t.M == M && t.N == N && t.K == K) return true;
+  return false;
+}
+
 bool gemm_bf16_supported(const GemmArgs& a) {
   const GemmPlan p = gemm_bf16_plan(a.M, a.N, a.K, a.split_k, a.tile_bm, a.tile_bn, a.tile_waves);
   if (p.bm == 0) return false;
diff --git a/csrc/gemm/gemm_group.h b/csrc/gemm/gemm_group.h
--- a/csrc/gemm/gemm_group.h
+++ b/csrc/gemm/gemm_group.h
@@ -8,4 +8,8 @@
 int64_t gemm_wgrad_group_ws(const GemmArgs& a);
 void launch_gemm_wgrad_group(const GemmArgs* a, int n, hipStream_t stream);
 
+bool gemm_wgrad_splitk_group_supported(const GemmArgs* a, int n, int split);
+int64_t gemm_wgrad_splitk_group_ws(const GemmArgs& a, int split);
+void launch_gemm_wgrad_splitk_group(const GemmArgs* a, int n, int split, hipStream_t stream);
+
 }
diff --git a/csrc/gemm/gemm_group.hip b/csrc/gemm/gemm_group.hip
--- a/csrc/gemm/gemm_group.hip
+++ b/csrc/gemm/gemm_group.hip
@@ -1,4 +1,4 @@
-#include "gemm/gemm_bf16_kernel.h"
+#include "gemm/gemm_bf16_launch.h"
 #include "gemm/gemm_group.h"
 
 namespace fan {
@@ -60,6 +60,89 @@
   FAN_HIP_CHECK(hipGetLastError());
 }
 
+WireOut wire_upd_of(const GemmArgs& a) {
+  WireOut wo = wire_of(a);
+  wo.um = a.upd_master;
+  wo.ulp = a.upd_lp;
+  wo.umom = a.upd_mom;
+  wo.up = a.upd;
+  return wo;
+}
+
+int slab_reduce_blocks(const GemmArgs& a) { return stream_grid((size_t)a.M * a.N / 4); }
+
+template <int SK>
+void launch_wgrad_splitk_group(const GemmArgs* a, int n, hipStream_t s) {
+  using P = PlCfg<false, false, kEpiWire, float, false, true, true, 256, 256>;
+  PlGroup<float> g{};
+  SlabGroup sg{};
+  g.n = sg.n = n;
+  int wg = 0, rb = 0;
+  for (int i = 0; i < n; ++i) {
+    const WireOut wo = wire_upd_of(a[i]);
+    g.p[i] = problem_of<float>(a[i], wo);
+    g.p[i].split_k = SK;
+    g.first[i] = wg;
+    const int units = (a[i].M / 256) * (a[i].N / 256) * SK;
+    wg += (units + kNumXCD - 1) / kNumXCD * kNumXCD;
+    sg.ws[i] = (const float*)a[i].workspace;
+    sg.C[i] = (float*)a[i].C;
+    sg.colsum[i] = a[i].colsum;
+    sg.ldc[i] = a[i].ldc;
+    sg.wo[i] = wo;
+    sg.M[i] = a[i].M;
+    sg.N[i] = a[i].N;
+    sg.first[i] = rb;
+    rb += slab_reduce_blocks(a[i]);
+  }
+  g.first[n] = wg;
+  sg.first[n] = rb;
+  auto k = gemm_groupn_kernel<P>;
+  FAN_HIP_CHECK(hipFuncSetAttribute((const void*)k, hipFuncAttributeMaxDynamicSharedMemorySize, P::kLds));
+  hipLaunchKernelGGL(k, wg, 256, P::kLds, s, g);
+  FAN_HIP_CHECK(hipGetLastError());
+  const bool upd = a[0].upd_master != nullptr;
+  const ColsumGroup q = take_pending_colsum(s);
+  const int qb = q.n > 0 ? q.first[q.n] : 0;
+  auto reduce = [&](auto kr) { hipLaunchKernelGGL(kr, qb + rb, 256, 0, s, sg, q); };
+  if (upd && q.n > 0) reduce(splitk_reduce_wire4_group_kernel<true, SK, true>);
+  else if (upd) reduce(splitk_reduce_wire4_group_kernel<true, SK, false>);
+  else if (q.n > 0) reduce(splitk_reduce_wire4_group_kernel<false, SK, true>);
+  else reduce(splitk_reduce_wire4_group_kernel<false, SK, false>);
+  FAN_HIP_CHECK(hipGetLastError());
+}
+
+}
+
+int64_t gemm_wgrad_splitk_group_ws(const GemmArgs& a, int split) { return (int64_t)split * ((int64_t)a.M * a.N + a.N); }
+
+bool gemm_wgrad_splitk_group_supported(const GemmArgs* a, int n, int split) {
+  if (n < 1 || n > kGroupMax || (split != 2 && split != 4)) return false;
+  int64_t wg = 0;
+  for (int i = 0; i < n; ++i) {
+    const GemmArgs& g = a[i];
+    if (g.a_kcontig || g.b_kcontig || g.c_bf16 || g.accumulate || !g.colsum || !g.workspace) return false;
+    if (g.epilogue != kEpiWire || !g.wire || g.defer_colsum || g.defer_reduce) return false;
+    if (g.M <= 0 || g.N <= 0 || g.M % 256 || g.N % 256 || g.K <= 0 || g.K % (64 * split) || g.ldc < g.N) return false;
+    if (g.lda % 8 || g.ldb % 8 || g.ldc % 16) return false;
+    if ((((uintptr_t)g.A | (uintptr_t)g.B | (uintptr_t)g.C | (uintptr_t)g.colsum | (uintptr_t)g.workspace) & 15))
+      return false;
+    if (g.wire_shard <= 0 || g.wire_shard % 256 || g.wire_off < 0 || g.wire_off % 16) return false;
+    if (g.wire_codec != kBfpTrunc && g.wire_codec != kBfpRne) return false;
+    if (g.wire_off + (int64_t)g.M * g.ldc + g.N >= (1ll << 31)) return false;
+    if ((g.upd_master != nullptr) != (a[0].upd_master != nullptr)) return false;
+    if (g.upd_master && (g.wire_codec != kBfpRne || g.wire_own != -1)) return false;
+    if (!g.upd_master && (g.upd_lp || g.upd_mom)) return false;
+    wg += ((int64_t)(g.M / 256) * (g.N / 256) * split + kNumXCD - 1) / kNumXCD * kNumXCD;
+  }
+  return wg <= 64 * kNumCU;
+}
+
+void launch_gemm_wgrad_splitk_group(const GemmArgs* a, int n, int split, hipStream_t s) {
+  FAN_CHECK(gemm_wgrad_splitk_group_supported(a, n, split),
+            "gemm_wgrad_splitk_group: unsupported shapes / layouts / wire or update fields");
+  if (split == 2) launch_wgrad_splitk_group<2>(a, n, s);
+  else launch_wgrad_splitk_group<4>(a, n, s);
 }
 
 int64_t gemm_wgrad_group_ws(const GemmArgs& a) { return (int64_t)(a.M / 256) * a.N; }
diff --git a/fpga_ai_nic_amd/models/mlp.py b/fpga_ai_nic_amd/models/mlp.py
--- a/fpga_ai_nic_amd/models/mlp.py
+++ b/fpga_ai_nic_amd/models/mlp.py
@@ -181,11 +181,11 @@
         if self._relu_at(self.L - 1):
             self.dz[self.L].mul_(self.logits > 0)
 
-    def backward_weight(self, i: int, wire=None, update=None, defer_colsum=False):
+    def backward_weight(self, i: int, wire=None, update=None, defer_colsum=False, split_k=None, tile=None):
         l = self.layers[i]
         if wire is not None:
             G.linear_bwd_weight(self.act[i], self.dz[i + 1], l.gw, bias_grad=l.gb if self.bias else None, wire=wire,
-                                update=update, defer_colsum=defer_colsum)
+                                update=update, defer_colsum=defer_colsum, split_k=split_k, tile=tile)
         elif not self.bias:
             G.linear_bwd_weight(self.act[i], self.dz[i + 1], l.gw)
         elif l.gw.is_cuda and self.dtype == torch.bfloat16:
@@ -194,6 +194,13 @@
             G.linear_bwd_weight(self.act[i], self.dz[i + 1], l.gw)
             NN.col_sum(self.dz[i + 1], l.gb)
 
+    def wgrad_problem(self, i: int):
+        return self.act[i], self.dz[i + 1]
+
+    def backward_weight_group(self, items, split: int):
+        G.gemm_wgrad_splitk_group([(self.act[i], self.dz[i + 1], self.layers[i].gw, self.layers[i].gb, wire, update)
+                                   for i, wire, update in items], split)
+
     def backward_data(self, i: int):
         if i == 0:
             return
diff --git a/fpga_ai_nic_amd/ops/gemm.py b/fpga_ai_nic_amd/ops/gemm.py
--- a/fpga_ai_nic_amd/ops/gemm.py
+++ b/fpga_ai_nic_amd/ops/gemm.py
@@ -121,6 +121,62 @@
         Cx.gemm_wgrad_group(Xs, dYs, Cs, css, offs, ws, buf, int(shard), int(own), int(codec), int(period))
 
 
+def wgrad_static_split(x, dz) -> int:
+    if not (x.is_cuda and x.dtype == torch.bfloat16 and dz.dtype == torch.bfloat16):
+        return 0
+    Cx = _ext.require()
+    K, M, N = x.shape[0], x.shape[1], dz.shape[1]
+    static = tuple(Cx.gemm_plan(M, N, K, 0, 0, 0, 0))
+    if static[:2] != (256, 256) or static[2] <= 1 or Cx.gemm_plan_overridden(M, N, K):
+        return 0
+    from . import gemm_tune
+
+    T = gemm_tune.tuner()
+    if T.enabled:
+        plan = T.lookup(T.key(M, N, K, True, False, EPI_WIRE, True, 1, x.device))
+        if plan is None:
+            if T.worth_tuning(M, N, static, x.device):
+                return 0
+        elif tuple(plan) != static[:3]:
+            return 0
+    return int(static[2])
+
+
+def wgrad_group_split(problems, cus: int = 256) -> int:
+    if not 2 <= len(problems) <= 8:
+        return 0
+    tiles = sum((p[0].shape[1] // 256) * (p[1].shape[1] // 256) for p in problems)
+    s = 1
+    while s * tiles < cus:
+        s *= 2
+    if s not in (2, 4) or any(p[0].shape[0] % (64 * s) or p[0].shape[0] // s < 1024 for p in problems):
+        return 0
+    mnk = [(p[0].shape[1], p[1].shape[1], p[0].shape[0]) for p in problems]
+    return s if _ext.require().gemm_wgrad_splitk_group_supported(mnk, s) else 0
+
+
+def gemm_wgrad_splitk_group(problems, split: int):
+    Cx = _ext.require()
+    Xs, dYs, Cs, css = ([p[i] for p in problems] for i in range(4))
+    wires = [tuple(p[4]) + (0, 0)[len(p[4]) - 4:] for p in problems]
+    upds = [p[5] if len(p) > 5 else None for p in problems]
+    if len({int(w[3]) for w in wires}) != 1:
+        raise ValueError("gemm_wgrad_splitk_group: one wire codec for the group")
+    u0 = upds[0]
+    hyper = lambda u: (u.lr, u.grad_scale, u.weight_decay, u.momentum, u.nesterov)
+    if any((u is None) != (u0 is None) or (u is not None and hyper(u) != hyper(u0)) for u in upds):
+        raise ValueError("gemm_wgrad_splitk_group: the fused update on every problem (same hyper-parameters) or none")
+    ws = _workspace(Cs[0].device, Cx.gemm_wgrad_splitk_group_ws([(x.shape[1], y.shape[1]) for x, y in zip(Xs, dYs)],
+                                                                int(split)))
+    kw = {} if u0 is None else dict(upd_lr=u0.lr, upd_grad_scale=u0.grad_scale, upd_weight_decay=u0.weight_decay,
+                                    upd_momentum=u0.momentum, upd_nesterov=u0.nesterov)
+    Cx.gemm_wgrad_splitk_group(Xs, dYs, Cs, css, int(split), ws, [w[0] for w in wires], [int(w[1]) for w in wires],
+                               [int(w[2]) for w in wires], [int(w[4]) for w in wires], [int(w[5]) for w in wires],
+                               int(wires[0][3]), [None if u is None else u.master for u in upds],
+                               [None if u is None else u.lp for u in upds],
+                               [None if u is None else u.mom for u in upds], **kw)
+
+
 def _aligned16(C, bias, aux) -> bool:
     ok = C.data_ptr() % 16 == 0 and C.stride(0) % 8 == 0
     if bias is not None:
@@ -297,8 +353,10 @@
     return gemm(dz, False, w, True, out, EPI_NONE)
 
 
-def linear_bwd_weight(x, dz, out, accumulate=False, bias_grad=None, wire=None, update=None, defer_colsum=False):
+def linear_bwd_weight(x, dz, out, accumulate=False, bias_grad=None, wire=None, update=None, defer_colsum=False,
+                      split_k=None, tile=None):
     if wire is not None:
         return gemm(x, True, dz, False, out, EPI_WIRE, colsum=bias_grad, wire=wire, update=update,
-                    defer_colsum=defer_colsum)
-    return gemm(x, True, dz, False, out, EPI_NONE, accumulate=accumulate, colsum=bias_grad)
+                    defer_colsum=defer_colsum, split_k=split_k, tile=tile)
+    return gemm(x, True, dz, False, out, EPI_NONE, accumulate=accumulate, colsum=bias_grad, split_k=split_k,
+                tile=tile)
diff --git a/fpga_ai_nic_amd/parallel/dp.py b/fpga_ai_nic_amd/parallel/dp.py
--- a/fpga_ai_nic_amd/parallel/dp.py
+++ b/fpga_ai_nic_amd/parallel/dp.py
@@ -7,7 +7,7 @@
 
 from ..models.mlp import MLP
 from ..ops import gemm as G
-from ..ops import wire
+from ..ops import gemm_tune, wire
 from ..utils import tracing
 from .allreduce import CompressedAllReduce, Handle, _round_up
 from .transport import Transport
@@ -61,7 +61,7 @@
                  weight_decay: float = 0.0, momentum: float = 0.0, nesterov: bool = False,
                  loss_scale: float = 1.0, average: bool = True, profile: bool = False, prepack: bool = True,
                  commit_at_end: bool | None = None, fused_update: bool | None = None,
-                 gemm_inflight: str | None = None):
+                 gemm_inflight: str | None = None, wgrad_pair: bool | str | None = None):
         self.m = model
         self.engine = engine
         self.world = engine.world if engine is not None else 1
@@ -84,6 +84,12 @@
         self.fused_updates = 0
         self.defer_colsum = os.environ.get("FAN_DEFER_COLSUM", "1") != "0"
         self.fold_logits = os.environ.get("FAN_FOLD_LOGITS", "1") != "0"
+        wp = os.environ.get("FAN_WGRAD_PAIR", "1") != "0" if wgrad_pair is None else wgrad_pair
+        if wp not in (True, False, "single"):
+            raise ValueError(f"wgrad_pair must be True|False|'single', got {wgrad_pair!r}")
+        self.wgrad_pair = wp
+        self.wgrad_groups = 0
+        self._wgrad_plan = (None, [], 0)
         self.chain_fwd = G.chain_enabled()
         self.chain_bwd = G.chain_enabled()
         gi = os.environ.get("FAN_GEMM_INFLIGHT", "persistent") if gemm_inflight is None else gemm_inflight
@@ -162,6 +168,8 @@
                  if self.prepack and l.cout % 16 == 0 else None) for l in m.layers]
         chained = (self.fused_update and self.chain_bwd and all(t is not None for t in tgts)
                    and m.backward_data_chain())
+        post, split = self._wgrad_postponed(tgts)
+        late = []
         try:
             for i in reversed(range(m.L)):
                 l = m.layers[i]
@@ -172,7 +180,10 @@
                             m.backward_data(i)
                         upd = G.LocalUpdate(l.master, l.lp, l.mom, lr=self.lr, grad_scale=self.grad_scale,
                                             weight_decay=self.wd, momentum=self.momentum, nesterov=self.nesterov)
-                        m.backward_weight(i, wire=tgt, update=upd, defer_colsum=self.defer_colsum)
+                        if i in post:
+                            late.append((i, tgt, upd))
+                        else:
+                            m.backward_weight(i, wire=tgt, update=upd, defer_colsum=self.defer_colsum)
                         self.fused_updates += 1
                     else:
                         m.backward_weight(i, wire=tgt)
@@ -199,6 +210,13 @@
                     self.times["bwd_first"] += t1 - t0
                     self.times["bwd"] += t1 - t0
                     t0 = t1
+            if late and self.wgrad_pair == "single":
+                for i, tgt, upd in late:
+                    m.backward_weight(i, wire=tgt, update=upd, split_k=split, tile=(256, 256))
+            elif late:
+                with tracing.range("bwd_wgrad_group"):
+                    m.backward_weight_group(late, split)
+                self.wgrad_groups += 1
         finally:
             if self.fused_updates and self.defer_colsum and self.cuda:
                 G.flush_colsum()
@@ -215,6 +233,18 @@
             self._sync()
             self.times["bwd"] += time.perf_counter() - t0
 
+    def _wgrad_postponed(self, tgts):
+        m = self.m
+        if not (self.wgrad_pair and self.fused_update and self.cuda and m.bias):
+            return [], 0
+        T = gemm_tune.tuner()
+        key = (m.act[0].shape[0], tuple(t is not None for t in tgts), id(T), T.enabled, len(T.plans))
+        if self._wgrad_plan[0] != key:
+            post = [i for i in range(m.L) if tgts[i] is not None and G.wgrad_static_split(*m.wgrad_problem(i)) > 1]
+            split = G.wgrad_group_split([m.wgrad_problem(i) for i in post])
+            self._wgrad_plan = (key, post if split else [], split)
+        return self._wgrad_plan[1:]
+
     def _gemm_grid(self, on: bool):
         if self.gemm_inflight != "grid":
             return
```

New measurement: 8.517 million samples/s (median of 6 runs). 1.02x the previous value.
